# MILAB-IIT-CV/ATDN_vSLAM

Measured on AMD Instinct MI355X. Metric: frame-pairs/sec, KITTI 1241x376 odometry inference at 1/2/4/8 MI355X, higher is better.
Workload: dtype f32 via 3xf16 split MFMA (fp32 accumulate); 1 GPU; KITTI seq-03-shaped 376x1241 uint8 frames (resident in HBM) resized to 376x1232, GMA flow 12 GRU iters + CLVO head -> 6-DoF trajectory (BASELINE configs[1]); streams_per_gpu=2, gru_iters=12, parallelism=pairs sharded x1, one all-gather of 512-d features, replicated LSTM scan

## Files before the change

atdn_vslam_amd/_lib.py:

```python
import ctypes as C
import os

_HERE = os.path.dirname(os.path.abspath(__file__))
LIB_PATH = os.environ.get("ATDN_LIB_PATH") or os.path.join(_HERE, "libatdn_hip.so")

_f32p = C.POINTER(C.c_float)
_i64p = C.POINTER(C.c_int64)
_vp = C.c_void_p

SIGNATURES = {
    "atdn_version": (C.c_int, []),
    "atdn_last_error": (C.c_char_p, []),
    "atdn_gma_create": (C.c_int, [C.POINTER(_vp), C.c_int, C.c_int, C.c_int, C.c_int]),
    "atdn_gma_set_low_latency": (C.c_int, [_vp, C.c_int]),
    "atdn_gma_load": (C.c_int, [_vp, C.c_char_p, _vp, _i64p, C.c_int]),
    "atdn_gma_finalize": (C.c_int, [_vp]),
    "atdn_gma_forward": (C.c_int, [_vp, _vp, _vp, C.c_int, C.c_int, _vp, _vp, _vp, _vp]),
    "atdn_gma_forward_predictions": (C.c_int, [_vp, _vp, _vp, C.c_int, C.c_int, _vp, _vp, _vp]),
    "atdn_gma_forward_sequence": (C.c_int, [_vp, _vp, C.c_int, C.c_int, _vp, _vp, _vp, _vp]),
    "atdn_gma_forward_sequence_continued": (C.c_int, [_vp, _vp, C.c_int, C.c_int, _vp, _vp, _vp, _vp]),
    "atdn_gma_debug_read": (C.c_long, [_vp, C.c_char_p, _vp, C.c_long, _vp]),
    "atdn_gma_profile": (C.c_int, [_vp, C.c_int, C.c_int, C.c_int, _f32p, _vp]),
    "atdn_gma_profile_mode": (C.c_int, [_vp, C.c_int, C.c_int, C.c_int, C.c_int, _f32p, _vp]),
    "atdn_gma_set_range_probe": (C.c_int, [_vp, C.c_int]),
    "atdn_gma_range_rows": (C.c_long, [_vp]),
    "atdn_gma_range_row": (C.c_int, [_vp, C.c_long, C.c_char_p, C.c_int, C.POINTER(C.c_int), C.POINTER(C.c_int), _f32p, _i64p, _i64p]),
    "atdn_range_probe": (C.c_int, [_vp, C.c_int64, C.c_int64, C.c_int64, _f32p, _i64p, _i64p, _vp]),
    "atdn_range_probe_launch": (C.c_int, [_vp, C.c_int64, C.c_int64, C.c_int64, _vp, _vp]),
    "atdn_gma_workspace_bytes": (C.c_size_t, [_vp]),
    "atdn_gma_destroy": (None, [_vp]),
    "atdn_device_bytes_live": (C.c_int64, []),
    "atdn_clvo_create": (C.c_int, [C.POINTER(_vp), C.c_int, C.c_int, C.c_int]),
    "atdn_clvo_load": (C.c_int, [_vp, C.c_char_p, _vp, _i64p, C.c_int]),
    "atdn_clvo_finalize": (C.c_int, [_vp]),
    "atdn_clvo_encode": (C.c_int, [_vp, _vp, C.c_int, _vp, _vp]),
    "atdn_clvo_step": (C.c_int, [_vp, _vp, C.c_int, C.c_int, _vp, _vp, _vp, _vp]),
    "atdn_clvo_last_scan_path": (C.c_int, [_vp]),
    "atdn_clvo_destroy": (None, [_vp]),
    "atdn_vae_create": (C.c_int, [C.POINTER(_vp), C.c_int, C.c_int, C.c_int]),
    "atdn_vae_load": (C.c_int, [_vp, C.c_char_p, _vp, _i64p, C.c_int]),
    "atdn_vae_finalize": (C.c_int, [_vp]),
    "atdn_vae_embedding_shape": (C.c_int, [_vp, C.POINTER(C.c_int), C.POINTER(C.c_int)]),
    "atdn_vae_encode": (C.c_int, [_vp, _vp, C.c_int, _vp, _vp]),
    "atdn_vae_scratch_floats": (C.c_int, [C.c_int, C.c_int, C.POINTER(C.c_long), C.POINTER(C.c_int)]),
    "atdn_vae_debug_stage": (C.c_int, [_vp, _vp, C.c_int, C.c_int, _vp, C.c_long, _vp]),
    "atdn_vae_destroy": (None, [_vp]),
    "atdn_clvo_trainer_create": (C.c_int, [C.POINTER(_vp), C.c_int, C.c_int, C.c_int, C.c_int]),
    "atdn_clvo_trainer_load": (C.c_int, [_vp, C.c_char_p, _vp, _i64p, C.c_int]),
    "atdn_clvo_trainer_finalize": (C.c_int, [_vp]),
    "atdn_clvo_trainer_forward_backward": (C.c_int, [_vp, _vp, _vp, _vp, _vp, _vp, _f32p, _vp]),
    "atdn_clvo_trainer_gradients": (C.c_int, [_vp, C.POINTER(_vp), C.POINTER(C.c_long)]),
    "atdn_clvo_trainer_adamw_step": (C.c_int, [_vp, C.c_float, C.c_float, C.c_float, C.c_int, _vp]),
    "atdn_clvo_trainer_set_loss": (C.c_int, [_vp, C.c_float, C.c_int, C.c_int]),
    "atdn_clvo_trainer_loss_terms": (C.c_int, [_vp, _f32p]),
    "atdn_clvo_loss": (C.c_int, [_vp, _vp, _vp, _vp, C.c_int, C.c_int, C.c_float, C.c_int, C.c_int, _f32p, _vp, _vp, _vp]),
    "atdn_clvo_trainer_read": (C.c_long, [_vp, C.c_char_p, C.c_int, _vp, C.c_long, _vp]),
    "atdn_clvo_trainer_destroy": (None, [_vp]),
    "atdn_pose_transform_f32": (C.c_int, [_vp, _vp, _vp]),
    "atdn_pose_rel2abs": (C.c_int, [_vp, _vp, C.c_int, _vp]),
    "atdn_pose_accumulate_f32": (C.c_int, [_vp, _vp, _vp]),
    "atdn_resize_frames": (C.c_int, [_vp, C.c_int, C.c_int, C.c_int, C.c_int, C.c_int, _vp, _vp]),
    "atdn_resize_frames_mode": (C.c_int, [_vp, C.c_int, C.c_int, C.c_int, C.c_int, C.c_int, C.c_int, _vp, _vp]),
    "atdn_resize_frames_u8": (C.c_int, [_vp, C.c_int, C.c_int, C.c_int, C.c_int, C.c_int, C.c_int, _vp, _vp]),
    "atdn_pad_frames": (C.c_int, [_vp, C.c_int, C.c_int, C.c_int, C.c_int, C.c_int, C.c_int, C.c_int, _vp, _vp]),
    "atdn_ingest_create": (C.c_int, [C.POINTER(_vp), C.c_int, C.c_int, C.c_int, C.c_int, C.c_int, C.c_int]),
    "atdn_ingest_frames_u8": (C.c_int, [_vp, _vp, C.c_int, _vp, _vp]),
    "atdn_ingest_destroy": (None, [_vp]),
    "atdn_flow_pack_f16": (C.c_int, [_vp, C.c_int, C.c_int, C.c_int, C.c_int, C.c_int, _vp, _vp]),
    "atdn_flow_gather_clips": (C.c_int, [_vp, C.c_int, C.c_int, C.c_int, _vp, _vp, C.c_int, C.c_int, _vp, _vp]),
    "atdn_flow_forward_interpolate": (C.c_int, [_vp, C.c_int, C.c_int, C.c_int, _vp, _vp]),
    "atdn_flow_forward_interpolate_host": (C.c_int, [_vp, C.c_int, C.c_int, C.c_int, _vp]),
    "atdn_flow_consistency": (C.c_int, [_vp, _vp, C.c_int, C.c_int, C.c_int, C.c_double, C.c_double, _vp, _vp, _vp]),
    "atdn_flow_consistency_host": (C.c_int, [_vp, _vp, C.c_int, C.c_int, C.c_int, C.c_double, C.c_double, _vp, _vp]),
    "atdn_flow_two_view_depth": (C.c_int, [_vp, _vp, _vp, C.c_int, C.c_int, C.c_int, C.c_double, C.c_double, C.c_double, C.c_double,
                                           C.c_double, C.c_double, C.c_double, _vp, _vp, _vp]),
    "atdn_flow_two_view_depth_host": (C.c_int, [_vp, _vp, _vp, C.c_int, C.c_int, C.c_int, C.c_double, C.c_double, C.c_double,
                                                C.c_double, C.c_double, C.c_double, C.c_double, _vp, _vp]),
    "atdn_depth_backproject": (C.c_int, [_vp, C.c_int, C.c_int, C.c_int, C.c_double, C.c_double, C.c_double, C.c_double, _vp, _vp]),
    "atdn_flow_track_step": (C.c_int, [_vp, _vp, _vp, _vp, C.c_int, C.c_int, C.c_int, _vp, _vp, _vp, C.c_double, C.c_double, C.c_double,
                                       C.c_double, C.c_double, C.c_double, C.c_double, _vp, _vp, _vp]),
    "atdn_flow_track_step_host": (C.c_int, [_vp, _vp, _vp, _vp, C.c_int, C.c_int, C.c_int, _vp, _vp, _vp, C.c_double, C.c_double,
                                            C.c_double, C.c_double, C.c_double, C.c_double, C.c_double, _vp, _vp]),
    "atdn_depth_fuse": (C.c_int, [_vp, _vp, _vp, _vp, C.c_int, C.c_int, C.c_int, C.c_int, C.c_int, C.c_double, C.c_double, C.c_double,
                                  C.c_double, C.c_double, C.c_double, C.c_int, C.c_double, C.c_int, _vp, _vp, _vp, _vp]),
    "atdn_depth_fuse_host": (C.c_int, [_vp, _vp, _vp, _vp, C.c_int, C.c_int, C.c_int, C.c_int, C.c_int, C.c_double, C.c_double,
                                       C.c_double, C.c_double, C.c_double, C.c_double, C.c_int, C.c_double, C.c_int, _vp, _vp, _vp]),
    "atdn_multiview_depth": (C.c_int, [_vp, _vp, _vp, _vp, _vp, C.c_int, C.c_int, C.c_int, C.c_int, C.c_int, C.c_double, C.c_double,
                                       C.c_double, C.c_double, C.c_double, C.c_double, C.c_double, C.c_int, C.c_double, C.c_double,
                                       C.c_int, _vp, _vp, _vp, _vp, _vp]),
    "atdn_multiview_depth_host": (C.c_int, [_vp, _vp, _vp, _vp, _vp, C.c_int, C.c_int, C.c_int, C.c_int, C.c_int, C.c_double,
                                            C.c_double, C.c_double, C.c_double, C.c_double, C.c_double, C.c_double, C.c_int,
                                            C.c_double, C.c_double, C.c_int, _vp, _vp, _vp, _vp]),
    "atdn_bundle_workspace_bytes": (C.c_long, [C.c_int, C.c_int, C.c_int, C.c_int, C.c_int]),
    "atdn_bundle_terms": (C.c_int, [_vp] * 6 + [C.c_int] * 5 + [C.c_double] * 4 + [C.c_int] + [C.c_double] * 3 + [C.c_int] + [_vp] * 4),
    "atdn_bundle_terms_host": (C.c_int, [_vp] * 6 + [C.c_int] * 5 + [C.c_double] * 4 + [C.c_int] + [C.c_double] * 3 + [C.c_int] +
                               [_vp] * 2),
    "atdn_bundle_adjust": (C.c_int, [_vp] * 6 + [C.c_int] * 5 + [C.c_double] * 4 + [C.c_int] * 2 + [C.c_double] * 3 + [C.c_int] +
                           [_vp] * 6),
    "atdn_bundle_adjust_host": (C.c_int, [_vp] * 6 + [C.c_int] * 5 + [C.c_double] * 4 + [C.c_int] * 2 + [C.c_double] * 3 + [C.c_int] +
                                [_vp] * 4),
    "atdn_pnp_workspace_bytes":(C.c_long, [C.c_int, C.c_int, C.c_int]),
    "atdn_pnp_terms": (C.c_int, [_vp, _vp, _vp, _vp, C.c_int, C.c_int, C.c_int, C.c_double, C.c_double, C.c_double, C.c_double,
                                 C.c_double, C.c_double, C.c_double, _vp, _vp, _vp, _vp]),
    "atdn_pnp_terms_host": (C.c_int, [_vp, _vp, _vp, _vp, C.c_int, C.c_int, C.c_int, C.c_double, C.c_double, C.c_double, C.c_double,
                                      C.c_double, C.c_double, C.c_double, _vp, _vp]),
    "atdn_pnp_solve": (C.c_int, [_vp, _vp, _vp, _vp, C.c_int, C.c_int, C.c_int, C.c_double, C.c_double, C.c_double, C.c_double,
                                 C.c_double, C.c_double, C.c_double, C.c_int, _vp, _vp, _vp, _vp, _vp]),
    "atdn_pnp_solve_host": (C.c_int, [_vp, _vp, _vp, _vp, C.c_int, C.c_int, C.c_int, C.c_double, C.c_double, C.c_double, C.c_double,
                                      C.c_double, C.c_double, C.c_double, C.c_int, _vp, _vp, _vp]),
    "atdn_epipolar_workspace_bytes": (C.c_long, [C.c_int, C.c_int, C.c_int]),
    "atdn_epipolar_terms": (C.c_int, [_vp, _vp, _vp, C.c_int, C.c_int, C.c_int, C.c_double, C.c_double, C.c_double, C.c_double,
                                      C.c_double, C.c_double, _vp, _vp, _vp, _vp]),
    "atdn_epipolar_terms_host": (C.c_int, [_vp, _vp, _vp, C.c_int, C.c_int, C.c_int, C.c_double, C.c_double, C.c_double, C.c_double,
                                           C.c_double, C.c_double, _vp, _vp]),
    "atdn_epipolar_solve": (C.c_int, [_vp, _vp, _vp, C.c_int, C.c_int, C.c_int, C.c_double, C.c_double, C.c_double, C.c_double,
                                      C.c_double, C.c_double, C.c_int, _vp, _vp, _vp, _vp, _vp]),
    "atdn_epipolar_solve_host": (C.c_int, [_vp, _vp, _vp, C.c_int, C.c_int, C.c_int, C.c_double, C.c_double, C.c_double, C.c_double,
                                           C.c_double, C.c_double, C.c_int, _vp, _vp, _vp]),
    "atdn_ground_workspace_bytes": (C.c_long, [C.c_int, C.c_int, C.c_int]),
    "atdn_ground_terms": (C.c_int, [_vp] * 3 + [C.c_int] * 5 + [C.c_double] * 8 + [_vp] * 4),
    "atdn_ground_terms_host": (C.c_int, [_vp] * 3 + [C.c_int] * 5 + [C.c_double] * 8 + [_vp] * 2),
    "atdn_ground_solve": (C.c_int, [_vp] * 3 + [C.c_int] * 5 + [C.c_double] * 11 + [C.c_int] * 2 + [_vp] * 5),
    "atdn_ground_solve_host": (C.c_int, [_vp] * 3 + [C.c_int] * 5 + [C.c_double] * 11 + [C.c_int] * 2 + [_vp] * 3),
    "atdn_ground_classify": (C.c_int, [_vp] * 3 + [C.c_int] * 5 + [C.c_double] * 7 + [_vp] * 3),
    "atdn_ground_classify_host": (C.c_int, [_vp] * 3 + [C.c_int] * 5 + [C.c_double] * 7 + [_vp] * 2),
    "atdn_pose_graph_workspace_bytes": (C.c_long, [C.c_int, C.c_int, C.c_int]),
    "atdn_pose_graph_terms": (C.c_int, [_vp, _vp, _vp, _vp, _vp, C.c_int, C.c_int, C.c_int, C.c_double, _vp, _vp, _vp, _vp, _vp]),
    "atdn_pose_graph_terms_host": (C.c_int, [_vp, _vp, _vp, _vp, _vp, C.c_int, C.c_int, C.c_int, C.c_double, _vp, _vp, _vp]),
    "atdn_pose_graph_solve": (C.c_int, [_vp, _vp, _vp, _vp, _vp, _vp, C.c_int, C.c_int, C.c_int, C.c_double, C.c_int, C.c_int,
                                        C.c_double, _vp, _vp, _vp, _vp, _vp, _vp]),
    "atdn_pose_graph_solve_host": (C.c_int, [_vp, _vp, _vp, _vp, _vp, _vp, C.c_int, C.c_int, C.c_int, C.c_double, C.c_int, C.c_int,
                                             C.c_double, _vp, _vp, _vp, _vp]),
    "atdn_map_search": (C.c_int, [_vp, C.c_int, C.c_int, _vp, C.c_int, C.c_int, _vp, _vp, _vp]),
    "atdn_map_gather_images_u8": (C.c_int, [_vp, C.c_int, C.c_long, _vp, C.c_int, _vp, _vp]),
    "atdn_corr_lookup": (C.c_int, [_vp, _vp, _vp, _vp, C.c_int, C.c_int, C.c_int, _vp, _vp, C.c_int, _vp]),
    "atdn_corr_pyramid": (C.c_int, [_vp, _vp, C.c_int, C.c_int, C.c_int, C.c_int, _vp, _vp, _vp, _vp, _vp]),
    "atdn_corr_lookup_bricks": (C.c_int, [_vp, _vp, C.c_int, C.c_int, C.c_int, C.c_int, _vp, _vp, _vp, _vp, _vp, _vp, _vp, _vp,
                                          _vp, _vp]),
    "atdn_conv2d_nhwc": (C.c_int, [_vp, C.c_int, C.c_int, C.c_int, C.c_int, _vp, _vp, C.c_int, C.c_int, C.c_int,
                                   C.c_int, C.c_int, C.c_int, C.c_int, _vp, _vp]),
    "atdn_conv2d_nhwc_sf": (C.c_int, [_vp, C.c_int, C.c_int, C.c_int, C.c_int, _vp, _vp, C.c_int, C.c_int, C.c_int,
                                      C.c_int, C.c_int, C.c_int, _vp, _vp]),
    "atdn_conv2d_nhwc_sf_epi": (C.c_int, [_vp, C.c_int, C.c_int, C.c_int, C.c_int, _vp, _vp, C.c_int, C.c_int, C.c_int,
                                      C.c_int, C.c_int, C.c_int, C.c_int, _vp, _vp]),
}

GMA_STAGES = ("fnet", "corr", "pool", "cnet", "attention", "lookup", "motion_encoder", "aggregate", "gru_zr", "gru_q",
              "flow_head", "mask", "gru_ctx", "attn_logits", "agg_vt", "convc1", "gru_zr_v", "gru_q_v")

_lib = None


def lib():
    global _lib
    if _lib is None:
        if not os.path.exists(LIB_PATH):
            raise RuntimeError(
                "%s is missing: the HIP extension has not been built (python -m atdn_vslam_amd.build). "
                "There is no CPU fallback for the product path." % LIB_PATH)
        import torch
        handle = C.CDLL(LIB_PATH)
        for name, (res, args) in SIGNATURES.items():
            fn = getattr(handle, name)
            fn.restype = res
            fn.argtypes = args
        _lib = handle
    return _lib


def check(rc):
    if rc != 0:
        raise RuntimeError("libatdn_hip: " + lib().atdn_last_error().decode("utf-8", "replace"))


def load_state(load_fn, handle, state):
    import numpy as np
    import torch
    for key, val in state.items():
        if isinstance(val, torch.Tensor):
            if not val.dtype.is_floating_point:
                continue
            arr = val.detach().to("cpu", torch.float32).contiguous().numpy()
        else:
            arr = np.asarray(val)
            if arr.dtype.kind != "f":
                continue
            arr = np.ascontiguousarray(arr, dtype=np.float32)
        shape = (C.c_int64 * max(arr.ndim, 1))(*arr.shape) if arr.ndim else (C.c_int64 * 1)(1)
        check(load_fn(handle, key.encode(), arr.ctypes.data_as(_vp), shape, arr.ndim))
```

atdn_vslam_amd/csrc/capi.hip:

```cpp
#include "../../include/atdn_hip.h"

#include <cmath>
#include <cstring>

#include "clvo.h"
#include "gma.h"
#include "vae.h"
#include "clvo_train.h"
#include "train_kernels.h"
#include "frontend.h"
#include "conv_sf.h"
#include "depth_fusion_host.h"
#include "epilogues_sf.h"
#include "epipolar_host.h"
#include "flow_args.h"
#include "flow_consistency_host.h"
#include "flow_track_host.h"
#include "bundle_host.h"
#include "ground_host.h"
#include "multiview_depth_host.h"
#include "pnp_host.h"
#include "two_view_host.h"
#include "warm_start_host.h"

namespace atdn {
extern template TileChoice conv_dispatch<MODE_TAP, EpiBias<ACT_NONE>>(const ConvShape&, EpiBias<ACT_NONE>, hipStream_t);
extern template TileChoice conv_dispatch<MODE_TAP, EpiBias<ACT_RELU>>(const ConvShape&, EpiBias<ACT_RELU>, hipStream_t);
extern template TileChoice conv_dispatch<MODE_ROW, EpiBias<ACT_NONE>>(const ConvShape&, EpiBias<ACT_NONE>, hipStream_t);
extern template TileChoice conv_dispatch<MODE_ROW, EpiBias<ACT_RELU>>(const ConvShape&, EpiBias<ACT_RELU>, hipStream_t);
extern template TileChoice conv_dispatch<MODE_TAP, EpiScale>(const ConvShape&, EpiScale, hipStream_t);

extern template TileChoice conv_sf_dispatch<EpiBias<ACT_NONE>>(const ConvShape&, float, EpiBias<ACT_NONE>, hipStream_t);
extern template TileChoice conv_sf_dispatch<SfBias<ACT_NONE>>(const ConvShape&, float, SfBias<ACT_NONE>, hipStream_t);

static thread_local std::string g_last_error;
void set_last_error(const std::string& msg) { g_last_error = msg; }
}

using namespace atdn;

struct atdn_gma { GmaNet net; atdn_gma(int H, int W, int B, int prec) : net(H, W, B, prec) {} };
struct atdn_clvo { ClvoNet net; atdn_clvo(int H, int W, int B) : net(H, W, B) {} };
struct atdn_vae { VaeEncoder net; atdn_vae(int H, int W, int B) : net(H, W, B) {} };
struct atdn_ingest { FrameIngest in; atdn_ingest(int a, int b, int c, int d, int n, int aa) : in(a, b, c, d, n, aa) {} };
struct atdn_clvo_trainer { ClvoTrainer net; atdn_clvo_trainer(int H, int W, int B, int T) : net(H, W, B, T) {} };

template <class T>
static void euler_yxz(const T* r, T* R) {
  const T c1 = std::cos(r[0]), c2 = std::cos(r[1]), c3 = std::cos(r[2]);
  const T s1 = std::sin(r[0]), s2 = std::sin(r[1]), s3 = std::sin(r[2]);
  R[0] = c1 * c3 + s1 * s2 * s3; R[1] = c3 * s1 * s2 - c1 * s3; R[2] = c2 * s1;
  R[3] = c2 * s3;                R[4] = c2 * c3;                R[5] = -s2;
  R[6] = c1 * s2 * s3 - c3 * s1; R[7] = c1 * c3 * s2 + s1 * s3; R[8] = c1 * c2;
}
template <class T>
static void make_transform(const T* rot, const T* tr, T* m) {
  T R[9];
  euler_yxz(rot, R);
  for (int i = 0; i < 3; ++i) { for (int j = 0; j < 3; ++j) m[i * 4 + j] = R[i * 3 + j]; m[i * 4 + 3] = tr[i]; }
  m[12] = 0; m[13] = 0; m[14] = 0; m[15] = 1;
}
template <class T>
static void matmul4(const T* a, const T* b, T* c) {
  for (int i = 0; i < 4; ++i)
    for (int j = 0; j < 4; ++j) {
      T s = 0;
      for (int k = 0; k < 4; ++k) s += a[i * 4 + k] * b[k * 4 + j];
      c[i * 4 + j] = s;
    }
}

extern "C" {

int atdn_version(void) { return 100; }
const char* atdn_last_error(void) { return g_last_error.c_str(); }

int atdn_gma_create(atdn_gma** out, int H, int W, int max_batch, int precision) {
  ATDN_API_BEGIN
  ATDN_CHECK(out, "null out pointer");
  *out = new atdn_gma(H, W, max_batch, precision);
  ATDN_API_END
}
int atdn_gma_set_low_latency(atdn_gma* h, int on) {
  ATDN_API_BEGIN
  ATDN_CHECK(h, "null handle");
  h->net.set_low_latency(on != 0);
  ATDN_API_END
}
int atdn_gma_load(atdn_gma* h, const char* key, const float* data, const int64_t* shape, int rank) {
  ATDN_API_BEGIN
  ATDN_CHECK(h && key && data && rank >= 0 && rank <= 4, "bad state-dict entry");
  h->net.state().put(key, data, shape, rank);
  ATDN_API_END
}
int atdn_gma_finalize(atdn_gma* h) {
  ATDN_API_BEGIN
  ATDN_CHECK(h, "null handle");
  h->net.finalize();
  ATDN_API_END
}
int atdn_gma_forward(atdn_gma* h, const float* im1, const float* im2, int B, int iters, const float* flow_init,
                     float* flow_low, float* flow_up, void* stream) {
  ATDN_API_BEGIN
  ATDN_CHECK(h, "null handle");
  h->net.forward(im1, im2, B, iters, flow_init, flow_low, flow_up, (hipStream_t)stream);
  ATDN_API_END
}
int atdn_gma_forward_predictions(atdn_gma* h, const float* im1, const float* im2, int B, int iters, const float* flow_init,
                                 float* flow_predictions, void* stream) {
  ATDN_API_BEGIN
  ATDN_CHECK(h, "null handle");
  h->net.forward_predictions(im1, im2, B, iters, flow_init, flow_predictions, (hipStream_t)stream);
  ATDN_API_END
}
int atdn_gma_forward_sequence(atdn_gma* h, const float* frames, int B, int iters, const float* flow_init,
                              float* flow_low, float* flow_up, void* stream) {
  ATDN_API_BEGIN
  ATDN_CHECK(h, "null handle");
  h->net.forward_sequence(frames, B, iters, flow_init, flow_low, flow_up, (hipStream_t)stream);
  ATDN_API_END
}
int atdn_gma_forward_sequence_continued(atdn_gma* h, const float* frames, int B, int iters, const float* flow_init,
                                        float* flow_low, float* flow_up, void* stream) {
  ATDN_API_BEGIN
  ATDN_CHECK(h, "null handle");
  h->net.forward_sequence(frames, B, iters, flow_init, flow_low, flow_up, (hipStream_t)stream, true);
  ATDN_API_END
}
long atdn_gma_debug_read(atdn_gma* h, const char* name, float* host, long capacity, void* stream) {
  try {
    if (!h || !name || !host) throw Error("null argument");
    const long n = h->net.debug_read(name, host, capacity, (hipStream_t)stream);
    if (n < 0) throw Error(std::string("unknown tensor name: ") + name);
    return n;
  } catch (const std::exception& e) {
    set_last_error(e.what());
    return -1;
  }
}
int atdn_gma_profile(atdn_gma* h, int B, int iters, int reps, float* ms_out, void* stream) {
  ATDN_API_BEGIN
  ATDN_CHECK(h && ms_out, "null argument");
  static_assert(GmaNet::ST_COUNT == ATDN_GMA_STAGES, "stage table out of sync with the header");
  h->net.profile(B, iters, reps, ms_out, (hipStream_t)stream, 0);
  ATDN_API_END
}
int atdn_gma_profile_mode(atdn_gma* h, int B, int iters, int reps, int mode, float* ms_out, void* stream) {
  ATDN_API_BEGIN
  ATDN_CHECK(h && ms_out, "null argument");
  ATDN_CHECK(mode >= 0 && mode <= 2, "mode must be 0 (pair), 1 (sequence) or 2 (continued sequence)");
  h->net.profile(B, iters, reps, ms_out, (hipStream_t)stream, mode);
  ATDN_API_END
}
int atdn_gma_set_range_probe(atdn_gma* h, int on) {
  ATDN_API_BEGIN
  ATDN_CHECK(h, "null handle");
  h->net.set_probe(on != 0);
  ATDN_API_END
}
long atdn_gma_range_rows(atdn_gma* h) {
  if (!h) { set_last_error("null handle"); return -1; }
  return (long)h->net.probe_rows().size();
}
int atdn_gma_range_row(atdn_gma* h, long index, char* name, int name_capacity, int* iteration, int* limited, float* max_abs,
                       int64_t* over, int64_t* nonfinite) {
  ATDN_API_BEGIN
  ATDN_CHECK(h && name && iteration && limited && max_abs && over && nonfinite, "null argument");
  const auto& rows = h->net.probe_rows();
  ATDN_CHECK(index >= 0 && index < (long)rows.size(), "row index out of range");
  const GmaNet::ProbeRow& r = rows[(size_t)index];
  ATDN_CHECK(name_capacity > (int)r.name.size(), "name buffer too small");
  memcpy(name, r.name.c_str(), r.name.size() + 1);
  *iteration = r.iter; *limited = r.limited ? 1 : 0; *max_abs = r.max_abs;
  *over = (int64_t)r.over; *nonfinite = (int64_t)r.nonfinite;
  ATDN_API_END
}
int atdn_range_probe_launch(const float* x, int64_t rows, int64_t cols, int64_t ld, void* slot, void* stream) {
  ATDN_API_BEGIN
  launch_range_probe(x, (long)rows, (long)cols, (long)ld, static_cast<RangeSlot*>(slot), (hipStream_t)stream);
  ATDN_API_END
}
int atdn_range_probe(const float* x, int64_t rows, int64_t cols, int64_t ld, float* max_abs, int64_t* over, int64_t* nonfinite,
                     void* stream) {
  ATDN_API_BEGIN
  ATDN_CHECK(x && max_abs && over && nonfinite, "null argument");
  hipStream_t st = (hipStream_t)stream;
// ... 451 lines not shown
    }
    fbrick[l].alloc((long)B * bp.NB[l] * 256);
    launch_brick_rows(src, src_sb, B, pH[l], pW[l], 256, 256, fbrick[l].p, (long)bp.NB[l] * 256, st);
    pyr[l].alloc((long)B * bp.NPB * kBrickPixelBlock * bp.NB[l]);
    launch_corr_bricks(f1.p, (long)N * 256, fbrick[l].p, (long)bp.NB[l] * 256, B, N, bp.NB[l], 256, 1.0f / sqrtf(256.0f), pyr[l].p, false, st);
    bp.base[l] = pyr[l].p;
    if (rowmajor[l]) launch_unbrick(pyr[l].p, bp.NB[l], N, pH[l], pW[l], n8, rowmajor[l], st);
  }
  if (samples) {
    outsf.alloc(n8 * 352);
    launch_lookup_bricks(bp, coords, n8, outsf.p, st);
    scratch.alloc(n8 * 352);
    launch_from_sf(outsf.p, scratch.p, n8, 352, st);
    ATDN_HIP(hipMemcpy2DAsync(samples, 324 * sizeof(float), scratch.p, 352 * sizeof(float), 324 * sizeof(float), (size_t)n8,
                              hipMemcpyDeviceToDevice, st));
  }
  if (cor1) {
    StateDict sd;
    const int64_t ws[4] = {256, 324, 1, 1}, bs[1] = {256};
    sd.put("c.weight", convc1_weight_host, ws, 4);
    sd.put("c.bias", convc1_bias_host, bs, 1);
    PackedConv L = pack_conv_sf(A, sd, {"c"});
    pack_fragment_major16(A, L);
    A.upload();
    resolve(A, L);
    csf.alloc(n8 * 256);
    launch_lookup_conv(bp, coords, n8, nullptr, L.wf16, L.wscale, L.b, csf.p, false, st);
    launch_from_sf(csf.p, cor1, n8, 256, st);
    ATDN_HIP(hipStreamSynchronize(st));
  }
  ATDN_HIP(hipStreamSynchronize(st));
  ATDN_API_END
}

int atdn_conv2d_nhwc(const float* src, int nimg, int H, int W, int Cin, const float* weight_host,
                     const float* bias_host, int Cout, int KH, int KW, int stride, int padH, int padW, int relu,
                     float* dst, void* stream) {
  ATDN_API_BEGIN
  ATDN_CHECK(src && weight_host && dst && nimg >= 1, "null argument");
  const bool row = (Cin == 4 || Cin == 16);
  ATDN_CHECK(row || Cin % 32 == 0, "Cin must be 4, 16 or a multiple of 32");
  StateDict sd;
  const int64_t ws[4] = {Cout, Cin, KH, KW};
  sd.put("c.weight", weight_host, ws, 4);
  std::vector<float> zb(Cout, 0.f);
  const int64_t bs[1] = {Cout};
  sd.put("c.bias", bias_host ? bias_host : zb.data(), bs, 1);
  WeightArena A;
  PackedConv L = pack_conv(A, sd, {"c"}, row ? MODE_ROW : MODE_TAP, Cin);
  A.upload();
  resolve(A, L);
  ConvShape s;
  s.src0 = src; s.ld0 = Cin; s.sb0 = (long)H * W * Cin; s.C0 = L.C; s.H = H; s.W = W;
  s.KH = KH; s.KW = KW; s.stride = stride; s.padH = padH; s.padW = padW;
  s.w = L.w; s.ldw = L.ldw; s.N = Cout; s.nimg = nimg;
  const int Ho = conv_out(H, KH, stride, padH), Wo = conv_out(W, KW, stride, padW);
  hipStream_t st = (hipStream_t)stream;
  if (row) {
    if (relu) conv_dispatch<MODE_ROW>(s, EpiBias<ACT_RELU>{L.b, dst, (long)Ho * Wo * Cout, Cout, 1.f}, st);
    else conv_dispatch<MODE_ROW>(s, EpiBias<ACT_NONE>{L.b, dst, (long)Ho * Wo * Cout, Cout, 1.f}, st);
  } else {
    if (relu) conv_dispatch<MODE_TAP>(s, EpiBias<ACT_RELU>{L.b, dst, (long)Ho * Wo * Cout, Cout, 1.f}, st);
    else conv_dispatch<MODE_TAP>(s, EpiBias<ACT_NONE>{L.b, dst, (long)Ho * Wo * Cout, Cout, 1.f}, st);
  }
  ATDN_HIP(hipStreamSynchronize(st));
  ATDN_API_END
}

int atdn_resize_frames(const float* src, int planes, int Hin, int Win, int Hout, int Wout, float* dst, void* stream) {
  return atdn_resize_frames_mode(src, planes, Hin, Win, Hout, Wout, ATDN_RESIZE_ANTIALIAS, dst, stream);
}
int atdn_resize_frames_mode(const float* src, int planes, int Hin, int Win, int Hout, int Wout, int antialias, float* dst,
                            void* stream) {
  ATDN_API_BEGIN
  ATDN_CHECK(src && dst && planes >= 1 && Hin >= 1 && Win >= 1 && Hout >= 1 && Wout >= 1, "bad argument");
  ATDN_CHECK(antialias == 0 || antialias == 1, "antialias must be ATDN_RESIZE_BILINEAR or ATDN_RESIZE_ANTIALIAS");
  launch_resize<float>(src, planes, Hin, Win, Hout, Wout, antialias, dst, (hipStream_t)stream);
  ATDN_API_END
}
int atdn_resize_frames_u8(const uint8_t* src, int planes, int Hin, int Win, int Hout, int Wout, int antialias, float* dst,
                          void* stream) {
  ATDN_API_BEGIN
  ATDN_CHECK(src && dst && planes >= 1 && Hin >= 1 && Win >= 1 && Hout >= 1 && Wout >= 1, "bad argument");
  ATDN_CHECK(antialias == 0 || antialias == 1, "antialias must be ATDN_RESIZE_BILINEAR or ATDN_RESIZE_ANTIALIAS");
  launch_resize<unsigned char>(src, planes, Hin, Win, Hout, Wout, antialias, dst, (hipStream_t)stream);
  ATDN_API_END
}
int atdn_pad_frames(const float* src, int planes, int H, int W, int left, int right, int top, int bottom, float* dst,
                    void* stream) {
  ATDN_API_BEGIN
  ATDN_CHECK(src && dst && planes >= 1 && H >= 1 && W >= 1 && left >= 0 && right >= 0 && top >= 0 && bottom >= 0, "bad argument");
  launch_pad_replicate(src, planes, H, W, left, right, top, bottom, dst, (hipStream_t)stream);
  ATDN_API_END
}
int atdn_ingest_create(atdn_ingest** out, int Hin, int Win, int Hout, int Wout, int max_frames, int antialias) {
  ATDN_API_BEGIN
  ATDN_CHECK(out, "null out pointer");
  ATDN_CHECK(antialias == 0 || antialias == 1, "antialias must be ATDN_RESIZE_BILINEAR or ATDN_RESIZE_ANTIALIAS");
  *out = new atdn_ingest(Hin, Win, Hout, Wout, max_frames, antialias);
  ATDN_API_END
}
int atdn_ingest_frames_u8(atdn_ingest* h, const uint8_t* host_frames, int n_frames, float* dst, void* stream) {
  ATDN_API_BEGIN
  ATDN_CHECK(h, "null handle");
  h->in.ingest(host_frames, n_frames, dst, (hipStream_t)stream);
  ATDN_API_END
}
void atdn_ingest_destroy(atdn_ingest* h) { delete h; }

int atdn_conv2d_nhwc_sf_epi(const float* src, int nimg, int H, int W, int Cin, const float* weight_host,
                            const float* bias_host, int Cout, int KH, int KW, int stride, int padH, int padW, int sf_store,
                            float* dst, void* stream) {
  ATDN_API_BEGIN
  ATDN_CHECK(src && weight_host && dst && nimg >= 1 && Cin % 32 == 0, "bad argument (Cin must be a multiple of 32)");
  ATDN_CHECK(sf_store >= 0 && sf_store <= 7 && (sf_store & 6) != 6, "sf_store: bit 0 names the epilogue, bit 1 or bit 2 the tile form");
  const int tile_form = (sf_store & 2) ? 1 : (sf_store & 4) ? 2 : 0;
  sf_store &= 1;
  ATDN_CHECK(!sf_store || Cout % 32 == 0, "the split-f16 store needs Cout % 32 == 0");
  StateDict sd;
  const int64_t ws[4] = {Cout, Cin, KH, KW};
  sd.put("c.weight", weight_host, ws, 4);
  std::vector<float> zb(Cout, 0.f);
  const int64_t bs[1] = {Cout};
  sd.put("c.bias", bias_host ? bias_host : zb.data(), bs, 1);
  WeightArena A;
  PackedConv L = pack_conv_sf(A, sd, {"c"});
  A.upload();
  resolve(A, L);
  hipStream_t st = (hipStream_t)stream;
  DeviceBuf tmp, osf;
  const long rows = (long)nimg * H * W;
  tmp.alloc(rows * Cin);
  launch_to_sf(src, tmp.p, rows, Cin, st);
  ConvShape s;
  s.src0 = tmp.p; s.ld0 = Cin; s.sb0 = (long)H * W * Cin; s.C0 = L.C; s.H = H; s.W = W;
  s.KH = KH; s.KW = KW; s.stride = stride; s.padH = padH; s.padW = padW;
  s.w = L.w; s.ldw = L.ldw; s.N = Cout; s.nimg = nimg;
  const int Ho = conv_out(H, KH, stride, padH), Wo = conv_out(W, KW, stride, padW);
  s.wfrag16 = L.wf16;
  s.tile_form = tile_form;
  if (sf_store) {
    const long orows = (long)nimg * Ho * Wo;
    osf.alloc(orows * Cout);
    conv_sf_dispatch(s, L.wscale, SfBias<ACT_NONE>{L.b, osf.p, (long)Ho * Wo * Cout, Cout}, st);
    launch_from_sf(osf.p, dst, orows, Cout, st);
    ATDN_HIP(hipStreamSynchronize(st));
  } else {
    conv_sf_dispatch(s, L.wscale, EpiBias<ACT_NONE>{L.b, dst, (long)Ho * Wo * Cout, Cout, 1.f}, st);
    ATDN_HIP(hipStreamSynchronize(st));
  }
  ATDN_API_END
}

int atdn_conv2d_nhwc_sf(const float* src, int nimg, int H, int W, int Cin, const float* weight_host,
                        const float* bias_host, int Cout, int KH, int KW, int stride, int padH, int padW, float* dst,
                        void* stream) {
  return atdn_conv2d_nhwc_sf_epi(src, nimg, H, W, Cin, weight_host, bias_host, Cout, KH, KW, stride, padH, padW, 0, dst, stream);
}

}
```

atdn_vslam_amd/csrc/conv_mfma.h:

```cpp
#pragma once
#include "common.h"

namespace atdn {

typedef float f32x16 __attribute__((ext_vector_type(16)));

enum { MODE_TAP = 0, MODE_ROW = 1 };

struct ConvGeom {
  const float* src0;
  const float* src1;
  long sb0, sb1;
  int ld0, ld1;
  int C0, C1;
  int H, W, Ho, Wo;
  int KH, KW, stride, padH, padW;
  int cpk;
  int nchunks;
  int log2C;
  const float* w;
  long wb;
  int ldw;
  int N;
  int tiles_per_img, nimg, ntile_n;
// ... 62 lines not shown
        const float4 v = *reinterpret_cast<const float4*>(sp + (long)(ok ? iy * g.W + ix : 0) * ld + co + 4 * s);
        ra[i] = v;
        aok[i] = ok;
      }
      cc += 32;
      if (cc == ctot) { cc = 0; if (++kx == g.KW) { kx = 0; ++ky; } }
    } else {
      const int f = kx * 32 + 4 * s;
      const int dx = f >> g.log2C, c = f & (g.C0 - 1);
#pragma unroll
      for (int i = 0; i < RA; ++i) {
        const int iy = iy0[i] + ky, ix = ix0[i] + dx;
        const bool ok = ((unsigned)iy < (unsigned)g.H) & ((unsigned)ix < (unsigned)g.W);
        const float4 v = *reinterpret_cast<const float4*>(s0 + (long)(ok ? iy * g.W + ix : 0) * g.ld0 + c);
        ra[i] = v;
        aok[i] = ok;
      }
      if (++kx == g.cpk) { kx = 0; ++ky; }
    }
#pragma unroll
    for (int j = 0; j < RB; ++j) {
      const float4 v = *reinterpret_cast<const float4*>(wrow[j] + q * 32);
      rb[j] = v;
    }
  };

  const int lane = tid & 63, wave = tid >> 6;
  const int wm = wave / WGN, wn = wave % WGN;
  const int r = lane & 31, h = lane >> 5;
  f32x16 acc[TM][TN];
#pragma unroll
  for (int i = 0; i < TM; ++i)
#pragma unroll
    for (int j = 0; j < TN; ++j)
#pragma unroll
      for (int e = 0; e < 16; ++e) acc[i][j][e] = 0.f;

  const float* a_rd = As + (wm * TM * 32 + r) * LDS_LD + 4 * h;
  const float* b_rd = Bs + (wn * TN * 32 + r) * LDS_LD + 4 * h;

  fetch(0);
  for (int q = 0; q < g.nchunks; ++q) {
    __syncthreads();
#pragma unroll
    for (int i = 0; i < RA; ++i)
      *reinterpret_cast<float4*>(As + (r0 + 32 * i) * LDS_LD + 4 * s) = keep_if(aok[i], ra[i]);
#pragma unroll
    for (int j = 0; j < RB; ++j)
      *reinterpret_cast<float4*>(Bs + (r0 + 32 * j) * LDS_LD + 4 * s) = keep_if(wok[j], rb[j]);
    __syncthreads();
    if (q + 1 < g.nchunks) fetch(q + 1);
#pragma unroll
    for (int kc = 0; kc < 4; ++kc) {
      float4 a[TM], b[TN];
#pragma unroll
      for (int i = 0; i < TM; ++i) a[i] = *reinterpret_cast<const float4*>(a_rd + i * 32 * LDS_LD + kc * 8);
#pragma unroll
      for (int j = 0; j < TN; ++j) b[j] = *reinterpret_cast<const float4*>(b_rd + j * 32 * LDS_LD + kc * 8);
#pragma unroll
      for (int i = 0; i < TM; ++i)
#pragma unroll
        for (int j = 0; j < TN; ++j) {
          acc[i][j] = __builtin_amdgcn_mfma_f32_32x32x2f32(a[i].x, b[j].x, acc[i][j], 0, 0, 0);
          acc[i][j] = __builtin_amdgcn_mfma_f32_32x32x2f32(a[i].y, b[j].y, acc[i][j], 0, 0, 0);
          acc[i][j] = __builtin_amdgcn_mfma_f32_32x32x2f32(a[i].z, b[j].z, acc[i][j], 0, 0, 0);
          acc[i][j] = __builtin_amdgcn_mfma_f32_32x32x2f32(a[i].w, b[j].w, acc[i][j], 0, 0, 0);
        }
    }
  }

  typename EpiCol<Epi>::type colj[TN];
  float biasj[TN];
#pragma unroll
  for (int j = 0; j < TN; ++j) {
    const int n = min(n0 + (wn * TN + j) * 32 + r, g.N - 1);
    biasj[j] = 0.f;
    if constexpr (Epi::kStats) biasj[j] = ep.bias[n];
    if constexpr (epi_bias_arg<Epi>::value) colj[j] = ep.col(n);
  }
#pragma unroll
  for (int i = 0; i < TM; ++i) {
    const int mbase = pix0 + (wm * TM + i) * 32;
#pragma unroll
    for (int j = 0; j < TN; ++j) {
      const int n = n0 + (wn * TN + j) * 32 + r;
      const bool nok = n < g.N;
      if constexpr (Epi::kStats) {
        const float bias = nok ? biasj[j] : 0.f;
        float v[16];
        float sum = 0.f;
        int cnt = 0;
#pragma unroll
        for (int e = 0; e < 16; ++e) {
          const int m = mbase + (e & 3) + 8 * (e >> 2) + 4 * h;
          v[e] = acc[i][j][e] + bias;
          if (m < HoWo) { sum += v[e]; ++cnt; }
        }
        sum += __shfl_xor(sum, 32);
        cnt += __shfl_xor(cnt, 32);
        const float mean = sum / (float)(cnt > 0 ? cnt : 1);
        float m2 = 0.f;
#pragma unroll
        for (int e = 0; e < 16; ++e) {
          const int m = mbase + (e & 3) + 8 * (e >> 2) + 4 * h;
          if (m < HoWo) { const float d = v[e] - mean; m2 += d * d; }
        }
        m2 += __shfl_xor(m2, 32);
        if (h == 0 && nok) {
          const int grp = mbase >> 5;
          const long o = ((long)img * ep.groups_per_img + grp) * g.N + n;
          ep.part_sum[o] = sum;
          ep.part_m2[o] = m2;
        }
      }
      if (nok) {
        if constexpr (Epi::kPrefetch) {
          typename Epi::Aux aux[16];
#pragma unroll
          for (int e = 0; e < 16; ++e) aux[e] = ep.load(img, min(mbase + (e & 3) + 8 * (e >> 2) + 4 * h, HoWo - 1), n);
#pragma unroll
          for (int e = 0; e < 16; ++e) {
            const int m = mbase + (e & 3) + 8 * (e >> 2) + 4 * h;
            if (m < HoWo) ep.apply(img, m, n, acc[i][j][e], aux[e]);
          }
        } else if constexpr (epi_bias_arg<Epi>::value) {
#pragma unroll
          for (int e = 0; e < 16; ++e) {
            const int m = mbase + (e & 3) + 8 * (e >> 2) + 4 * h;
            if (m < HoWo) ep.store_c(img, m, n, acc[i][j][e], colj[j]);
          }
        } else {
#pragma unroll
          for (int e = 0; e < 16; ++e) {
            const int m = mbase + (e & 3) + 8 * (e >> 2) + 4 * h;
            if (m < HoWo) ep(img, m, n, acc[i][j][e]);
          }
        }
      }
    }
  }
}

struct ConvShape {
  const float* src0 = nullptr; const float* src1 = nullptr;
  long sb0 = 0, sb1 = 0;
  int ld0 = 0, ld1 = 0, C0 = 0, C1 = 0;
  int H = 1, W = 1;
  int KH = 1, KW = 1, stride = 1, padH = 0, padW = 0;
  const float* w = nullptr; long wb = 0; int ldw = 0;
  const float* wfrag16 = nullptr;
  int N = 0;
  int nimg = 1;
  const float* in_mean = nullptr; const float* in_rstd = nullptr;
  int tile_form = 0;
};

inline int conv_out(int in, int k, int stride, int pad) { return (in + 2 * pad - k) / stride + 1; }

template <int MODE>
inline ConvGeom make_geom(const ConvShape& s, int BM, int BN) {
  ConvGeom g{};
  g.src0 = s.src0; g.src1 = s.src1; g.sb0 = s.sb0; g.sb1 = s.sb1; g.ld0 = s.ld0; g.ld1 = s.ld1;
  g.C0 = s.C0; g.C1 = s.C1; g.H = s.H; g.W = s.W;
  g.KH = s.KH; g.KW = s.KW; g.stride = s.stride; g.padH = s.padH; g.padW = s.padW;
  g.Ho = conv_out(s.H, s.KH, s.stride, s.padH);
  g.Wo = conv_out(s.W, s.KW, s.stride, s.padW);
  if (MODE == MODE_TAP) {
    ATDN_CHECK(s.C0 % 32 == 0 && s.C1 % 32 == 0 && s.C0 > 0, "TAP mode needs channel counts that are multiples of 32");
    ATDN_CHECK(s.ld0 % 4 == 0 && (s.C1 == 0 || (s.src1 && s.ld1 % 4 == 0)), "TAP mode needs 16-byte aligned pixels");
    g.cpk = s.KW * ((s.C0 + s.C1) / 32);
    g.log2C = 0;
  } else {
    ATDN_CHECK(s.C1 == 0 && s.src1 == nullptr, "ROW mode takes one source");
    ATDN_CHECK(s.C0 >= 4 && (s.C0 & (s.C0 - 1)) == 0 && s.ld0 == s.C0, "ROW mode needs dense power-of-two channels");
    g.cpk = cdiv(s.KW * s.C0, 32);
    int l = 0; while ((1 << l) < s.C0) ++l;
    g.log2C = l;
  }
  g.nchunks = s.KH * g.cpk;
  g.w = s.w; g.wb = s.wb; g.ldw = s.ldw; g.N = s.N;
  ATDN_CHECK(s.ldw % 4 == 0 && s.ldw >= g.nchunks * 32, "weight rows must hold the padded K and be 16-byte aligned");
  ATDN_CHECK(((uintptr_t)s.src0 % 16) == 0 && ((uintptr_t)s.w % 16) == 0 && s.sb0 % 4 == 0 && s.wb % 4 == 0,
             "operands must be 16-byte aligned");
  ATDN_CHECK(g.Ho > 0 && g.Wo > 0 && s.N > 0 && s.nimg > 0, "empty convolution");
  g.nimg = s.nimg;
  g.tiles_per_img = cdiv(g.Ho * g.Wo, BM);
  g.ntile_n = cdiv(s.N, BN);
  return g;
}

inline int packed_k(int mode, int KH, int KW, int C) {
  return mode == MODE_TAP ? KH * KW * C : KH * round_up(KW * C, 32);
}

template <int MODE, int TM, int TN, int WGM, int WGN, class Epi>
inline void launch_conv(const ConvShape& s, const Epi& ep, hipStream_t st) {
  constexpr int BM = 32 * TM * WGM, BN = 32 * TN * WGN;
  ConvGeom g = make_geom<MODE>(s, BM, BN);
  const int nblk = g.nimg * g.tiles_per_img * g.ntile_n;
  hipLaunchKernelGGL((conv_mfma_kernel<MODE, TM, TN, WGM, WGN, Epi>), dim3(nblk), dim3(256), 0, st, g, ep);
  ATDN_HIP(hipGetLastError());
}

}
```

atdn_vslam_amd/csrc/conv_sf.h:

```cpp
#pragma once
#include <type_traits>
#include "conv_dispatch.h"
#include "sf.h"

namespace atdn {

template <int TM, int TN, int WGM, int WGN, class Epi, bool FAST = false>
__global__ __launch_bounds__(256) void conv_sf_kernel(const ConvGeom g, const float wscale, const Epi ep) {
  constexpr int BM = 32 * TM * WGM, BN = 32 * TN * WGN;
  constexpr int RA = BM / 32, RB = BN / 32;
  constexpr int LDS_LD = 40;
  __shared__ __attribute__((aligned(16))) float lds[(BM + BN) * LDS_LD];
  float* As = lds;
  float* Bs = lds + BM * LDS_LD;

  const int tid = threadIdx.x;
  const int nblk = g.nimg * g.tiles_per_img * g.ntile_n;
  const int id = xcd_remap(blockIdx.x, nblk);
  const int tile_n = id % g.ntile_n;
  const int tmg = id / g.ntile_n;
  const int img = tmg / g.tiles_per_img;
  const int pix0 = (tmg % g.tiles_per_img) * BM;
  const int n0 = tile_n * BN;
  const int HoWo = g.Ho * g.Wo;
// ... 74 lines not shown
  for (int d = 0; d < PF; ++d) fetch(min(d, last), d);
  const int nq = (g.nchunks + PF - 1) / PF * PF;
  for (int q0 = 0; q0 < nq; q0 += PF) {
#pragma unroll
   for (int d = 0; d < PF; ++d) {
    const int q = q0 + d;
    const bool live = PF == 1 || q <= last;
    __syncthreads();
#pragma unroll
    for (int i = 0; i < RA; ++i)
      *reinterpret_cast<float4*>(As + (r0 + 32 * i) * LDS_LD + 4 * s) = keep_if(aok[d][i] && live, ra[d][i]);
#pragma unroll
    for (int j = 0; j < RB; ++j)
      *reinterpret_cast<float4*>(Bs + (r0 + 32 * j) * LDS_LD + 4 * s) = keep_if(wok[j], rb[d][j]);
    __syncthreads();
    fetch(min(q + PF, last), d);
    f16x8 ah[TM][2], al[TM][2], bh[TN][2], bl[TN][2];
#pragma unroll
    for (int i = 0; i < TM; ++i)
#pragma unroll
      for (int hb = 0; hb < 2; ++hb) {
        ah[i][hb] = *reinterpret_cast<const f16x8*>(a_rd + (i * 32 + 16 * hb) * ROWB);
        if constexpr (!FAST) al[i][hb] = *reinterpret_cast<const f16x8*>(a_rd + (i * 32 + 16 * hb) * ROWB + 64);
      }
#pragma unroll
    for (int j = 0; j < TN; ++j)
#pragma unroll
      for (int cb = 0; cb < 2; ++cb) {
        bh[j][cb] = *reinterpret_cast<const f16x8*>(b_rd + (j * 32 + 16 * cb) * ROWB);
        if constexpr (!FAST) bl[j][cb] = *reinterpret_cast<const f16x8*>(b_rd + (j * 32 + 16 * cb) * ROWB + 64);
      }
#pragma unroll
    for (int i = 0; i < TM; ++i)
#pragma unroll
      for (int j = 0; j < TN; ++j)
#pragma unroll
        for (int hb = 0; hb < 2; ++hb)
#pragma unroll
          for (int cb = 0; cb < 2; ++cb) {
            f32x4v c = acc[i][j].b[hb][cb];
            if constexpr (!FAST) {
              c = __builtin_amdgcn_mfma_f32_16x16x32_f16(al[i][hb], bh[j][cb], c, 0, 0, 0);
              c = __builtin_amdgcn_mfma_f32_16x16x32_f16(ah[i][hb], bl[j][cb], c, 0, 0, 0);
            }
            c = __builtin_amdgcn_mfma_f32_16x16x32_f16(ah[i][hb], bh[j][cb], c, 0, 0, 0);
            acc[i][j].b[hb][cb] = c;
          }
   }
  }

  constexpr int NSET = 2, NPX = 8;
  auto col_of = [&](int cs) { return 16 * cs + (lane & 15); };
  auto row_of = [&](int e) { return 16 * (e >> 2) + 4 * (lane >> 4) + (e & 3); };
  auto val_of = [&](int i, int j, int cs, int e) __attribute__((always_inline)) { return acc[i][j].b[e >> 2][cs][e & 3]; };
  typename EpiCol<Epi>::type colj[TN][NSET];
  float biasj[TN][NSET];
#pragma unroll
  for (int j = 0; j < TN; ++j)
#pragma unroll
    for (int cs = 0; cs < NSET; ++cs) {
      const int n = min(n0 + (wn * TN + j) * 32 + col_of(cs), g.N - 1);
      biasj[j][cs] = 0.f;
      if constexpr (Epi::kStats) biasj[j][cs] = ep.bias[n];
      if constexpr (epi_bias_arg<Epi>::value) colj[j][cs] = ep.col(n);
    }
#pragma unroll
  for (int i = 0; i < TM; ++i) {
    const int mbase = pix0 + (wm * TM + i) * 32;
#pragma unroll
    for (int j = 0; j < TN; ++j)
#pragma unroll
      for (int cs = 0; cs < NSET; ++cs) {
        const int n = n0 + (wn * TN + j) * 32 + col_of(cs);
        const bool nok = n < g.N;
        if constexpr (Epi::kStats) {
          const float bias = nok ? biasj[j][cs] : 0.f;
          float v[NPX];
          float sum = 0.f;
          int cnt = 0;
#pragma unroll
          for (int e = 0; e < NPX; ++e) {
            const int m = mbase + row_of(e);
            v[e] = val_of(i, j, cs, e) * wscale + bias;
            if (m < HoWo) { sum += v[e]; ++cnt; }
          }
          sum += __shfl_xor(sum, 16);
          cnt += __shfl_xor(cnt, 16);
          sum += __shfl_xor(sum, 32);
          cnt += __shfl_xor(cnt, 32);
          const float mean = sum / (float)(cnt > 0 ? cnt : 1);
          float m2 = 0.f;
#pragma unroll
          for (int e = 0; e < NPX; ++e) {
            const int m = mbase + row_of(e);
            if (m < HoWo) { const float d = v[e] - mean; m2 += d * d; }
          }
          m2 += __shfl_xor(m2, 16);
          m2 += __shfl_xor(m2, 32);
          if ((lane >> 4) == 0 && nok) {
            const int grp = mbase >> 5;
            const long o = ((long)img * ep.groups_per_img + grp) * g.N + n;
            ep.part_sum[o] = sum;
            ep.part_m2[o] = m2;
          }
        }
        if (nok) {
          if constexpr (Epi::kPrefetch) {
            typename Epi::Aux aux[NPX];
#pragma unroll
            for (int e = 0; e < NPX; ++e) aux[e] = ep.load(img, min(mbase + row_of(e), HoWo - 1), n);
#pragma unroll
            for (int e = 0; e < NPX; ++e) {
              const int m = mbase + row_of(e);
              if (m < HoWo) ep.apply(img, m, n, val_of(i, j, cs, e) * wscale, aux[e]);
            }
          } else if constexpr (epi_bias_arg<Epi>::value) {
#pragma unroll
            for (int e = 0; e < NPX; ++e) {
              const int m = mbase + row_of(e);
              if (m < HoWo) ep.store_c(img, m, n, val_of(i, j, cs, e) * wscale, colj[j][cs]);
            }
          } else {
#pragma unroll
            for (int e = 0; e < NPX; ++e) {
              const int m = mbase + row_of(e);
              if (m < HoWo) ep(img, m, n, val_of(i, j, cs, e) * wscale);
            }
          }
        }
      }
  }
}

template <int TM, int TN, int WGM, int WGN, class Epi, bool FAST = false>
inline void launch_conv_sf(const ConvShape& s, float wscale, const Epi& ep, hipStream_t st) {
  constexpr int BM = 32 * TM * WGM, BN = 32 * TN * WGN;
  ConvGeom g = make_geom<MODE_TAP>(s, BM, BN);
  const int nblk = g.nimg * g.tiles_per_img * g.ntile_n;
  hipLaunchKernelGGL((conv_sf_kernel<TM, TN, WGM, WGN, Epi, FAST>), dim3(nblk), dim3(256), 0, st, g, wscale, ep);
  ATDN_HIP(hipGetLastError());
}

bool& sf_fast_mode();

template <class F>
inline auto with_fast(bool fast, F&& f) {
  return fast ? f(std::true_type{}) : f(std::false_type{});
}

template <class Epi>
TileChoice conv_sf_dispatch(const ConvShape& s, float wscale, Epi ep, hipStream_t st);
template <class Epi>
void conv_sf_dispatch_pair(const ConvShape& s0, float wscale0, Epi ep0, const ConvShape& s1, float wscale1, Epi ep1, hipStream_t st);

}
```

atdn_vslam_amd/csrc/conv_sf6.h:

```cpp
#pragma once
#include <type_traits>
#include "conv_sf.h"

namespace atdn {

struct Conv2Geom {
  const float* src0; const float* src1;
  long sb0, sb1;
  int ld0, ld1, C0, C1;
  int H, W, Ho, Wo;
  int padH, padW;
  int tiles_x, tiles_y;
  int nimg, ntile_n;
  const float* w; int N;
  float wscale;
  const float* in_mean; const float* in_rstd;
};

inline bool conv_halo_eligible(const ConvShape& s) {
  if (s.stride != 1 || s.wb != 0) return false;
  return (s.KH == 3 && s.KW == 3) || (s.KH == 1 && s.KW == 5) || (s.KH == 5 && s.KW == 1);
}

template <class E, class = void> struct epi_gen6 : std::integral_constant<int, 0> {};
template <class E> struct epi_gen6<E, std::void_t<decltype(E::kGen6)>> : std::integral_constant<int, E::kGen6> {};
template <class E, class = void> struct EpiAux4 { struct type {}; };
template <class E> struct EpiAux4<E, std::void_t<typename E::Aux4>> { using type = typename E::Aux4; };
template <class E, class = void> struct epi_flowhead : std::false_type {};
template <class E> struct epi_flowhead<E, std::void_t<decltype(E::kFlowHead)>> : std::bool_constant<E::kFlowHead> {};
template <class E, class = void> struct epi_ring3 : std::false_type {};
template <class E> struct epi_ring3<E, std::void_t<decltype(E::kRing3)>> : std::bool_constant<E::kRing3> {};
template <class E, class = void> struct epi_rawacc : std::false_type {};
template <class E> struct epi_rawacc<E, std::void_t<decltype(E::kRawAcc)>> : std::bool_constant<E::kRawAcc> {};
template <class E, class = void> struct epi_vec4 : std::false_type {};
template <class E> struct epi_vec4<E, std::void_t<decltype(E::kVec4)>> : std::bool_constant<E::kVec4> {};

typedef float f32x4v __attribute__((ext_vector_type(4)));
struct SfAcc { f32x4v b[2][2]; };

#ifdef ATDN_CONV_STAMP
#define ATDN_CONV_STAMP_SLOTS 4096
extern __device__ unsigned long long atdn_conv_stamps_dev[4][ATDN_CONV_STAMP_SLOTS][12];
template <class E> struct conv_stamp_kind : std::integral_constant<int, -1> {};
#endif

template <int TH, int TW, int BN, int WM, int WN, int KH, int KW, class Epi, bool FAST = false, bool NORM = false, int ABL = 0,
          bool RUN = false>
__device__ __forceinline__ void conv_sf6_body(const Conv2Geom& g, const Epi& ep, const int bidx) {
  static_assert(ABL == 0 || !NORM, "ablation builds exist for the plain patch loader");
  static_assert(!RUN || (((KH == 1 && KW == 5) || (KH == 5 && KW == 1)) && TH == 8 && BN == 128 && WM == 1 && WN == 4 && !NORM &&
                         ABL == 0 && !Epi::kStats && !epi_flowhead<Epi>::value),
                "run tiles: separable passes on the 8 x 16 x 128 block, plain loader, epilogues without statistics");
  static_assert(TW == 16, "the 16x16x32 loop is built for 16-pixel tile rows");
  constexpr int NIMG = 2;
  constexpr int NW = WM * WN, NT = NW * 64;
  constexpr int TM = TH * TW / 32 / WM, TN = BN / 32 / WN;
  static_assert(TM * WM * 32 == TH * TW && TN * WN * 32 == BN, "wave grid must tile the block");
  static_assert(32 % TW == 0 || TW % 32 == 0, "a 32-pixel MFMA row tile must cover whole tile rows");
  constexpr int NTAP = KH * KW;
  constexpr int RSTEP = NT / 8;
  constexpr int RSLOTS = 160;
  constexpr int PROWS = RUN ? RSLOTS : (TH + KH - 1) * (TW + KW - 1);
  constexpr int PW = TW + KW - 1;
  constexpr int NP = (PROWS + RSTEP - 1) / RSTEP;
  constexpr int ROWB = 160;
  constexpr int RS = PW * ROWB;
  constexpr bool SWAP = epi_vec4<Epi>::value;
  constexpr int PSZ = RUN ? RSLOTS * ROWB : (TH + KH - 1) * RS;
  __shared__ __attribute__((aligned(256))) char Pbytes[NIMG * PSZ];

  const int tid = threadIdx.x;
  const int tiles_img = g.tiles_x * g.tiles_y;
  const int nblk = g.nimg * tiles_img * g.ntile_n;
  const int id = xcd_remap(bidx, nblk);
  const int tile_n = id % g.ntile_n;
  const int tmg = id / g.ntile_n;
  const int img = tmg / tiles_img;
  const int tloc = tmg - img * tiles_img;
  const int ty0 = (tloc / g.tiles_x) * TH, tx0 = (tloc % g.tiles_x) * TW;
  const int n0 = tile_n * BN;
  const int lane = tid & 63, wave = tid >> 6;
  const int rL = KH == 1 ? g.W : g.H, rHW = g.H * g.W;
  const int rm0 = tloc * (TH * TW);
  const int rrun0 = RUN ? rm0 / rL : 0, rpos0 = rm0 - rrun0 * rL;
  const int rb1 = rL - rpos0, rb2 = rb1 + rL, rb3 = rb2 + rL;
  auto out_pixel = [&](int p) {
    if constexpr (RUN) {
      const int k = (p >= rb1 ? 1 : 0) + (p >= rb2 ? 1 : 0) + (p >= rb3 ? 1 : 0);
      const int m = rm0 + p;
      if (m >= rHW) return -1;
      return KH == 1 ? m : (rpos0 + p - k * rL) * g.W + rrun0 + k;
    } else {
      const int oy = ty0 + p / TW, ox = tx0 + p % TW;
      return (oy < g.Ho && ox < g.Wo) ? oy * g.Wo + ox : -1;
    }
  };
#ifdef ATDN_CONV_STAMP
  constexpr int kStamp = conv_stamp_kind<Epi>::value;
  unsigned long long st_r0 = 0, st_t0 = 0, st_t1 = 0, st_t2 = 0, st_bar = 0;
  unsigned long long st_e_slab = 0, st_e_wait = 0, st_e_apply = 0;
  if constexpr (kStamp >= 0) { st_r0 = __builtin_amdgcn_s_memrealtime(); st_t0 = __builtin_amdgcn_s_memtime(); }
#endif

  const int jrow = (tid >> 3) & 7;
  const int s = tid & 7, r0 = !NORM ? tid >> 3 : ((tid >> 6) << 3) + 2 * (jrow & 1) + ((jrow >> 1) & 1) + 4 * (jrow >> 2);
  static_assert(PSZ / 16 <= 4096, "LDS offset field");
  unsigned pmeta[NP];
#pragma unroll
  for (int k = 0; k < NP; ++k) {
    const int prow = r0 + RSTEP * k;
    unsigned off = 0;
    if constexpr (RUN) {
      static_assert(PROWS == NP * RSTEP, "every loader step writes slots of the image");
      const int kk = (prow >= 2 + rb1 ? 1 : 0) + (prow >= 10 + rb2 ? 1 : 0) + (prow >= 18 + rb3 ? 1 : 0);
      const bool gap = kk > 0 && prow < 2 + rb1 + (kk - 1) * rL + 8 * kk;
      const int p = prow - 2 - 8 * kk;
      const int pos = rpos0 + p - kk * rL;
      if (!gap && p < 130 && (unsigned)pos < (unsigned)rL && rm0 + p < rHW) off = (unsigned)(KH == 1 ? rm0 + p : pos * g.W + rrun0 + kk) + 1u;
      pmeta[k] = (off << 12) | (unsigned)((prow * ROWB + 16 * s) >> 4);
      continue;
    }
    const int py = prow / PW, px = prow - py * PW;
    if (prow < PROWS) {
      const int iy = ty0 - g.padH + py, ix = tx0 - g.padW + px;
      if ((unsigned)iy < (unsigned)g.H && (unsigned)ix < (unsigned)g.W) off = (unsigned)(iy * g.W + ix) + 1u;
    }
    pmeta[k] = (off << 12) | (unsigned)((py * RS + px * ROWB + 16 * s) >> 4);
    if (prow >= PROWS) pmeta[k] = pmeta[0];
  }
  const float* s0 = g.src0 + (long)img * g.sb0;
  const float* s1 = g.src1 ? g.src1 + (long)img * g.sb1 : nullptr;
  const int nck = (g.C0 + g.C1) >> 5;

  float4 pr[NP];
  auto fetch_patch = [&](int c) {
    const int cc = c << 5;
    const float* sp; int ld, co;
    if (cc < g.C0) { sp = s0; ld = g.ld0; co = cc; } else { sp = s1; ld = g.ld1; co = cc - g.C0; }
#pragma unroll
    for (int k = 0; k < NP; ++k)
      pr[k] = *reinterpret_cast<const float4*>(sp + (long)((pmeta[k] >> 12) ? (pmeta[k] >> 12) - 1 : 0) * ld + co + 4 * s);
  };
  auto store_patch = [&](int buf) {
#pragma unroll
    for (int k = 0; k < NP; ++k)
      *reinterpret_cast<float4*>(Pbytes + buf * PSZ + ((pmeta[k] & 0xFFFu) << 4)) = keep_if((pmeta[k] >> 12) != 0, pr[k]);
  };
  float4 nmu = make_float4(0.f, 0.f, 0.f, 0.f), nrs = make_float4(1.f, 1.f, 1.f, 1.f);
  auto fetch_norm = [&](int c) {
    nmu = *reinterpret_cast<const float4*>(g.in_mean + (long)img * g.C0 + (c << 5) + 4 * s);
    nrs = *reinterpret_cast<const float4*>(g.in_rstd + (long)img * g.C0 + (c << 5) + 4 * s);
  };
  bool norm_sat = false;
  auto store_row_norm = [&](int buf, int k, float4 mu, float4 rs) {
    const float hi = (pmeta[k] >> 12) != 0 ? 65504.f : 0.f;
    float4 v = pr[k];
    v.x = (v.x - mu.x) * rs.x; v.y = (v.y - mu.y) * rs.y; v.z = (v.z - mu.z) * rs.z; v.w = (v.w - mu.w) * rs.w;
    const float m = fmaxf(fmaxf(v.x, v.y), fmaxf(v.z, v.w));
    norm_sat |= !(m <= 65504.f);
    v.x = __builtin_amdgcn_fmed3f(v.x, 0.f, hi); v.y = __builtin_amdgcn_fmed3f(v.y, 0.f, hi);
    v.z = __builtin_amdgcn_fmed3f(v.z, 0.f, hi); v.w = __builtin_amdgcn_fmed3f(v.w, 0.f, hi);
    const unsigned h0 = sf_cvt_pk_(v.x, v.y), h1 = sf_cvt_pk_(v.z, v.w);
    const unsigned l0 = sf_residual_pk_(h0, v.x, v.y), l1 = sf_residual_pk_(h1, v.z, v.w);
    char* px = Pbytes + buf * PSZ + (((pmeta[k] & 0xFFFu) - (unsigned)s) << 4);
    *reinterpret_cast<uint2*>(px + 8 * s) = make_uint2(h0, h1);
    *reinterpret_cast<uint2*>(px + 64 + 8 * s) = make_uint2(l0, l1);
  };

  const int wm = wave / WN, wn = wave % WN;
  SfAcc acc[TM][TN];
#pragma unroll
  for (int i = 0; i < TM; ++i)
#pragma unroll
    for (int j = 0; j < TN; ++j) {
#pragma unroll
      for (int e = 0; e < 16; ++e) acc[i][j].b[e >> 3][(e >> 2) & 1][e & 3] = 0.f;
    }
  {
    const int n16 = lane & 15, g16 = lane >> 4;
    int a_off[RUN ? 2 * TM : TM];
#pragma unroll
    for (int i = 0; i < TM; ++i) {
      if constexpr (RUN) {
#pragma unroll
        for (int hh = 0; hh < 2; ++hh) {
          const int p = ((wm * TM + i) * 2 + hh) * 16 + n16;
          const int k = (p >= rb1 ? 1 : 0) + (p >= rb2 ? 1 : 0) + (p >= rb3 ? 1 : 0);
          a_off[hh * TM + i] = (p + 8 * k) * ROWB + 16 * g16;
        }
      } else {
        a_off[i] = ((wm * TM + i) * 2) * RS + n16 * ROWB + 16 * g16;
      }
    }
    const char* Pb = Pbytes;
    const int nblk16 = (g.N + 15) >> 4;
    const float* wrow[TN][2];
#pragma unroll
    for (int j = 0; j < TN; ++j)
#pragma unroll
      for (int cb = 0; cb < 2; ++cb)
        wrow[j][cb] = g.w + (long)min(((n0 >> 4) + (wn * TN + j) * 2 + cb), nblk16 - 1) * (NTAP * nck) * 512 + lane * 4;
    constexpr int RT = (NTAP % 3 == 0 || epi_ring3<Epi>::value) ? 3 : 2;
    constexpr int CU = (NTAP % RT == 0) ? 1 : RT;
    constexpr int NS = CU * NTAP;
    static_assert(NS % RT == 0, "ring size must divide the K steps of an unrolled iteration");
    struct WFrag { f16x8 hi[TN][2], lo[TN][2]; };
    WFrag wr[RT];
    auto load_w = [&](WFrag& f, int c0, int st, int cb) __attribute__((always_inline)) {
      const int cc = min(c0 + st / NTAP, nck - 1);
      const int q = (st % NTAP) * nck + cc;
#pragma unroll
      for (int j = 0; j < TN; ++j) {
        f.hi[j][cb] = *reinterpret_cast<const f16x8*>(wrow[j][cb] + (long)q * 512);
        if constexpr (!FAST) f.lo[j][cb] = *reinterpret_cast<const f16x8*>(wrow[j][cb] + (long)q * 512 + 256);
      }
    };
    fetch_patch(0);
    if constexpr (NORM) fetch_norm(0);
#pragma unroll
    for (int st = 0; st < RT - 1; ++st) { load_w(wr[st], 0, st, 0); load_w(wr[st], 0, st, 1); }
    if constexpr ((ABL & 1) != 0) { load_w(wr[RT - 1], 0, RT - 1, 0); load_w(wr[RT - 1], 0, RT - 1, 1); }
    if constexpr (NORM) {
#pragma unroll
      for (int k = 0; k < NP; ++k) store_row_norm(0, k, nmu, nrs);
    } else {
      store_patch(0);
    }
    __syncthreads();
#ifdef ATDN_CONV_STAMP
    if constexpr (kStamp >= 0) st_t1 = __builtin_amdgcn_s_memtime();
#endif
    f16x8 ah[2][TM], al[2][TM];
    auto read_a = [&](int half, int tap) __attribute__((always_inline)) {
      const char* arow = RUN ? Pb + tap * ROWB : Pb + (tap / KW + half) * RS + (tap % KW) * ROWB;
#pragma unroll
      for (int i = 0; i < TM; ++i) {
        const int ao = a_off[RUN ? half * TM + i : i];
        ah[half][i] = *reinterpret_cast<const f16x8*>(arow + ao);
        if constexpr (!FAST) al[half][i] = *reinterpret_cast<const f16x8*>(arow + ao + 64);
      }
    };
    auto mfma_half = [&](int half, const WFrag& w) __attribute__((always_inline)) {
#pragma unroll
      for (int i = 0; i < TM; ++i)
#pragma unroll
        for (int j = 0; j < TN; ++j)
#pragma unroll
          for (int cb = 0; cb < 2; ++cb) {
            f32x4v c = acc[i][j].b[half][cb];
            if constexpr (SWAP) {
              if constexpr (!FAST) {
                c = __builtin_amdgcn_mfma_f32_16x16x32_f16(w.hi[j][cb], al[half][i], c, 0, 0, 0);
                c = __builtin_amdgcn_mfma_f32_16x16x32_f16(w.lo[j][cb], ah[half][i], c, 0, 0, 0);
              }
              c = __builtin_amdgcn_mfma_f32_16x16x32_f16(w.hi[j][cb], ah[half][i], c, 0, 0, 0);
            } else {
              if constexpr (!FAST) {
                c = __builtin_amdgcn_mfma_f32_16x16x32_f16(al[half][i], w.hi[j][cb], c, 0, 0, 0);
                c = __builtin_amdgcn_mfma_f32_16x16x32_f16(ah[half][i], w.lo[j][cb], c, 0, 0, 0);
              }
              c = __builtin_amdgcn_mfma_f32_16x16x32_f16(ah[half][i], w.hi[j][cb], c, 0, 0, 0);
            }
            acc[i][j].b[half][cb] = c;
          }
    };
    constexpr int NMF = (FAST ? 1 : 3) * TM * TN * 2;
    constexpr int NH = 2 * NTAP;
    static_assert(!NORM || NH - 1 - NP >= 1, "normalise-on-load spreads its NP patch rows over the half-steps of a chunk");
    read_a(0, 0);
    if constexpr (KH != 3 || !Epi::kStats) __builtin_amdgcn_s_setprio(2);
    for (int c0 = 0; c0 < nck; c0 += CU) {
#pragma unroll
      for (int cu = 0; cu < CU; ++cu) {
        const int c = c0 + cu;
        const bool live = CU == 1 || c < nck;
        const int cn = min(c + 1, nck - 1);
#pragma unroll
        for (int hs = 0; hs < NH; ++hs) {
          const int tap = hs >> 1, half = hs & 1;
          const int st = cu * NTAP + tap;
          __builtin_amdgcn_sched_barrier(0);
          if (!(ABL & 2) && hs == 0) { fetch_patch(cn); if constexpr (NORM) fetch_norm(cn); }
          if (!(ABL & 1)) {
            if (RT == 2) { if (half == 0) { load_w(wr[(st + 1) % RT], c0, st + 1, 0); load_w(wr[(st + 1) % RT], c0, st + 1, 1); } }
            else load_w(wr[(st + RT - 1) % RT], c0, st + RT - 1, half);
          }
          if (!(ABL & 4) && hs + 1 < NH) read_a((hs + 1) & 1, (hs + 1) >> 1);
          if constexpr (NORM) {
            if (hs >= NH - 1 - NP && hs <= NH - 2) store_row_norm((c + 1) & 1, hs - (NH - 1 - NP), nmu, nrs);
          } else {
            if (!(ABL & 2) && hs == NH - 2) store_patch((c + 1) & 1);
          }
          if (live) mfma_half(half, wr[st % RT]);
          {
            constexpr int nds = 2 * TM;
            const int nvm = (RT == 2 ? (half == 0 ? 4 * TN : 0) : 2 * TN) + (hs == 0 ? NP : 0);
            const int ndw = NORM ? ((hs >= NH - 1 - NP && hs <= NH - 2) ? 2 : 0) : ((hs == NH - 2) ? NP : 0);
#pragma unroll
            for (int k = 0; k < NMF; ++k) {
              __builtin_amdgcn_sched_group_barrier(0x008, 1, 0);
              if (hs + 1 < NH && k < nds) __builtin_amdgcn_sched_group_barrier(0x100, 1, 0);
              else if (k - ((hs + 1 < NH) ? nds : 0) < nvm) __builtin_amdgcn_sched_group_barrier(0x020, 1, 0);
              else if (k - ((hs + 1 < NH) ? nds : 0) - nvm < ndw) __builtin_amdgcn_sched_group_barrier(0x200, 1, 0);
            }
          }
        }
        if (!(ABL & 2)) {
#ifdef ATDN_CONV_STAMP
          unsigned long long st_b0 = 0;
          if constexpr (kStamp >= 0) { asm volatile("s_waitcnt lgkmcnt(0)" ::: "memory"); st_b0 = __builtin_amdgcn_s_memtime(); }
#endif
          asm volatile("s_waitcnt lgkmcnt(0)\n\ts_barrier" ::: "memory");
#ifdef ATDN_CONV_STAMP
          if constexpr (kStamp >= 0) st_bar += __builtin_amdgcn_s_memtime() - st_b0;
#endif
          Pb = Pbytes + ((c + 1) & 1) * PSZ;
        }
        if (!(ABL & 4)) read_a(0, 0);
      }
    }
  }

#ifdef ATDN_CONV_STAMP
  if constexpr (kStamp >= 0) st_t2 = __builtin_amdgcn_s_memtime();
  auto stamp_out = [&]() __attribute__((always_inline)) {
    if constexpr (kStamp >= 0) {
      asm volatile("s_waitcnt vmcnt(0) lgkmcnt(0)" ::: "memory");
      const unsigned long long t3 = __builtin_amdgcn_s_memtime(), r1 = __builtin_amdgcn_s_memrealtime();
      const unsigned hw = __builtin_amdgcn_s_getreg((31 << 11) | 4), xcc = __builtin_amdgcn_s_getreg((31 << 11) | 20);
      if (wave == 0 && lane == 0 && bidx < ATDN_CONV_STAMP_SLOTS) {
        unsigned long long* o = atdn_conv_stamps_dev[kStamp * 2 + (KH == 5 ? 1 : 0)][bidx];
        o[0] = st_r0; o[1] = r1; o[2] = st_t1 - st_t0; o[3] = st_t2 - st_t1; o[4] = st_bar; o[5] = t3 - st_t2;
        o[6] = ((unsigned long long)xcc << 32) | hw; o[7] = t3 - st_t0;
        o[8] = st_e_slab; o[9] = st_e_wait; o[10] = st_e_apply; o[11] = 0;
      }
    }
  };
#endif
  if constexpr (KH != 3 || !Epi::kStats) __builtin_amdgcn_s_setprio(0);
  if constexpr (NORM) sf_report(norm_sat);
  if constexpr ((ABL & 8) != 0) {
    float tot = 0.f;
#pragma unroll
    for (int i = 0; i < TM; ++i)
#pragma unroll
      for (int j = 0; j < TN; ++j)
#pragma unroll
        for (int e = 0; e < 16; ++e) tot += acc[i][j].b[e >> 3][(e >> 2) & 1][e & 3];
    if (tot == 1.2345e-30f) ep(img, 0, 0, tot);
    return;
  }
  if constexpr (SWAP) {
    static_assert(NW * 32 * LDS_LD * 4 <= NIMG * PSZ, "transpose slabs must fit in the patch images");
    __syncthreads();
    float* tb = reinterpret_cast<float*>(Pbytes) + wave * (32 * LDS_LD);
    const int trow = lane >> 3, tcol = (lane & 7) * 4;
    auto tile_pixel = [&](int i, int q) {
      const int p = (wm * TM + i) * 32 + 8 * q + trow;
      if constexpr ((ABL & 16) != 0) return p;
      return out_pixel(p);
    };
    constexpr bool RAW = epi_rawacc<Epi>::value && !epi_flowhead<Epi>::value;
    auto slab_write = [&](const SfAcc& a) __attribute__((always_inline)) {
      const float sc = RAW ? 1.0f : g.wscale;
#pragma unroll
      for (int hh = 0; hh < 2; ++hh)
#pragma unroll
        for (int cb = 0; cb < 2; ++cb)
          *reinterpret_cast<float4*>(tb + (16 * hh + (lane & 15)) * LDS_LD + 16 * cb + 4 * (lane >> 4)) =
              RAW ? make_float4(a.b[hh][cb][0], a.b[hh][cb][1], a.b[hh][cb][2], a.b[hh][cb][3])
                  : make_float4(a.b[hh][cb][0] * sc, a.b[hh][cb][1] * sc, a.b[hh][cb][2] * sc, a.b[hh][cb][3] * sc);
    };
    if constexpr (epi_flowhead<Epi>::value) {
      static_assert(!epi_flowhead<Epi>::value || (WM == 1 && TN == 1 && TW == 16), "one block holds all output channels of its pixels");
      constexpr int RP = 20;
      static_assert(32 * RP <= 32 * LDS_LD, "the exchange rows live inside the wave's slab");
      {
        const int n16 = lane & 15, g16 = lane >> 4;
        const int c8 = n0 + wn * 32 + 8 * g16;
        const float4 bq0 = *reinterpret_cast<const float4*>(ep.bias + c8), bq1 = *reinterpret_cast<const float4*>(ep.bias + c8 + 4);
        const float b8[8] = {bq0.x, bq0.y, bq0.z, bq0.w, bq1.x, bq1.y, bq1.z, bq1.w};
        f16x8 w2h[2], w2l[2];
#pragma unroll
        for (int rbk = 0; rbk < 2; ++rbk) {
          const int u = 16 * rbk + n16;
          const float* wr = ep.w2 + (long)min(u, 17) * g.N + c8;
          const float4 wa = *reinterpret_cast<const float4*>(wr), wb = *reinterpret_cast<const float4*>(wr + 4);
          const float w8[8] = {wa.x, wa.y, wa.z, wa.w, wb.x, wb.y, wb.z, wb.w};
#pragma unroll
          for (int e = 0; e < 8; ++e) {
            const float w = u < 18 ? w8[e] * ep.w2mul : 0.f;
            w2h[rbk][e] = (_Float16)w;
            w2l[rbk][e] = (_Float16)(w - (float)w2h[rbk][e]);
          }
        }
        bool sat = false;
#pragma unroll
        for (int i = 0; i < TM; ++i) {
          slab_write(acc[i][0]);
          asm volatile("s_waitcnt lgkmcnt(0)" ::: "memory");
          __builtin_amdgcn_wave_barrier();
          f16x8 xh[2], xl[2];
#pragma unroll
          for (int pb = 0; pb < 2; ++pb) {
            const float* src = tb + (16 * pb + n16) * LDS_LD + 8 * g16;
            const float4 xa = *reinterpret_cast<const float4*>(src), xb = *reinterpret_cast<const float4*>(src + 4);
            const float x8[8] = {xa.x, xa.y, xa.z, xa.w, xb.x, xb.y, xb.z, xb.w};
#pragma unroll
            for (int e = 0; e < 8; ++e) {
              const SfPair sp = sf_split_flag(fmaxf(x8[e] + b8[e], 0.f), sat);
              xh[pb][e] = sp.hi; xl[pb][e] = sp.lo;
            }
          }
          asm volatile("s_waitcnt lgkmcnt(0)" ::: "memory");
          __builtin_amdgcn_wave_barrier();
#pragma unroll
          for (int pb = 0; pb < 2; ++pb) {
            f32x4v d0 = {0.f, 0.f, 0.f, 0.f}, d1 = {0.f, 0.f, 0.f, 0.f};
            if constexpr (!FAST) {
              d0 = __builtin_amdgcn_mfma_f32_16x16x32_f16(w2h[0], xl[pb], d0, 0, 0, 0);
              d0 = __builtin_amdgcn_mfma_f32_16x16x32_f16(w2l[0], xh[pb], d0, 0, 0, 0);
              d1 = __builtin_amdgcn_mfma_f32_16x16x32_f16(w2h[1], xl[pb], d1, 0, 0, 0);
              d1 = __builtin_amdgcn_mfma_f32_16x16x32_f16(w2l[1], xh[pb], d1, 0, 0, 0);
            }
            d0 = __builtin_amdgcn_mfma_f32_16x16x32_f16(w2h[0], xh[pb], d0, 0, 0, 0);
            d1 = __builtin_amdgcn_mfma_f32_16x16x32_f16(w2h[1], xh[pb], d1, 0, 0, 0);
            float* rp = tb + (16 * pb + n16) * RP;
            *reinterpret_cast<float4*>(rp + 4 * g16) = make_float4(d0[0] * ep.w2inv, d0[1] * ep.w2inv, d0[2] * ep.w2inv, d0[3] * ep.w2inv);
            if (g16 == 0) *reinterpret_cast<float2*>(rp + 16) = make_float2(d1[0] * ep.w2inv, d1[1] * ep.w2inv);
          }
          __syncthreads();
          for (int idx = tid; idx < 32 * 18; idx += NT) {
            const int px = idx / 18, u = idx - px * 18;
            const float* rq = reinterpret_cast<const float*>(Pbytes) + px * RP + u;
            float sum = 0.f;
#pragma unroll
            for (int w = 0; w < NW; ++w) sum += rq[w * (32 * LDS_LD)];
            const int p = i * 32 + px;
            const int oy = ty0 + p / TW, ox = tx0 + p % TW;
            if (oy < g.Ho && ox < g.Wo)
              ep.G[(long)(n0 / (NW * 32)) * ep.gstride + ((long)img * ep.npix + (long)oy * g.Wo + ox) * 18 + u] = sum;
          }
          __syncthreads();
        }
        sf_report(sat);
        return;
      }
    }
    struct NoAux {};
    using AuxT = typename std::conditional<Epi::kPrefetch, typename EpiAux4<Epi>::type, NoAux>::type;
    constexpr bool PIPE = Epi::kPrefetch && sizeof(AuxT) <= 2 * sizeof(float4);
    AuxT aux_next[PIPE ? 4 : 1];
    bool clamped = false;
    if constexpr (PIPE) {
      const int nb0 = n0 + (wn * TN) * 32 + tcol;
#pragma unroll
// ... 49 lines not shown
            asm volatile("s_waitcnt lgkmcnt(0)" ::: "memory");
            st_e_wait += st_c - st_b; st_b = st_c;
          }
#endif
#endif
#pragma unroll
          for (int q = 0; q < 4; ++q)
            if (mq[q] >= 0 && nb < g.N) {
              if constexpr (RAW) ep.apply4(img, mq[q], nb, v[q], aux[q], bj, clamped, g.wscale);
              else ep.apply4(img, mq[q], nb, v[q], aux[q], bj, clamped);
            }
#ifdef ATDN_CONV_STAMP
          if constexpr (kStamp >= 0) { asm volatile("s_waitcnt lgkmcnt(0)" ::: "memory"); st_e_apply += __builtin_amdgcn_s_memtime() - st_b; }
#endif
        } else {
#pragma unroll
          for (int q = 0; q < 4; ++q) {
            if (mq[q] < 0) continue;
            if (nb + 4 <= g.N) {
              if constexpr (RAW) ep.store4((ABL & 16) ? 0 : img, mq[q], nb, v[q], bj, clamped, g.wscale);
              else ep.store4((ABL & 16) ? 0 : img, mq[q], nb, v[q], bj, clamped);
            } else {
              const float sc = RAW ? g.wscale : 1.0f;
              const float e4[4] = {v[q].x * sc, v[q].y * sc, v[q].z * sc, v[q].w * sc};
#pragma unroll
              for (int e = 0; e < 4; ++e)
                if (nb + e < g.N) ep(img, mq[q], nb + e, e4[e]);
            }
          }
        }
      }
    }
    sf_report(clamped);
#ifdef ATDN_CONV_STAMP
    stamp_out();
#endif
    return;
  }
  constexpr int NSET = 2, NPX = 8;
  auto col_of = [&](int cs) { return 16 * cs + (lane & 15); };
  auto pix_of = [&](int e) { return 16 * (e >> 2) + 4 * (lane >> 4) + (e & 3); };
  auto val_of = [&](const SfAcc& a, int cs, int e) __attribute__((always_inline)) { return a.b[e >> 2][cs][e & 3]; };
  typename EpiCol<Epi>::type colj[TN][NSET];
  float biasj[TN][NSET];
#pragma unroll
  for (int j = 0; j < TN; ++j)
#pragma unroll
    for (int cs = 0; cs < NSET; ++cs) {
      const int n = min(n0 + (wn * TN + j) * 32 + col_of(cs), g.N - 1);
      biasj[j][cs] = 0.f;
      if constexpr (Epi::kStats) biasj[j][cs] = ep.bias[n];
      if constexpr (epi_bias_arg<Epi>::value) colj[j][cs] = ep.col(n);
    }
#pragma unroll
  for (int i = 0; i < TM; ++i) {
    const int pbase = (wm * TM + i) * 32;
    int mm[NPX];
#pragma unroll
    for (int e = 0; e < NPX; ++e) {
      mm[e] = out_pixel(pbase + pix_of(e));
    }
    int cnt = 0;
    unsigned mo[NPX];
    if constexpr (Epi::kStats) {
#pragma unroll
      for (int e = 0; e < NPX; ++e) {
        cnt += mm[e] >= 0 ? 1 : 0;
        mo[e] = (unsigned)max(mm[e], 0) * (unsigned)ep.ld;
      }
      cnt += __shfl_xor(cnt, 16);
      cnt += __shfl_xor(cnt, 32);
      cnt = __builtin_amdgcn_readfirstlane(cnt);
    }
    const bool full = cnt == 32;
    const float inv_cnt = 1.0f / (float)(cnt > 0 ? cnt : 1);
#pragma unroll
    for (int j = 0; j < TN; ++j)
#pragma unroll
      for (int cs = 0; cs < NSET; ++cs) {
        const int n = n0 + (wn * TN + j) * 32 + col_of(cs);
        const bool nok = n < g.N;
        if constexpr (Epi::kStats) {
          const float bias = nok ? biasj[j][cs] : 0.f;
          float v[NPX];
#pragma unroll
          for (int e = 0; e < NPX; ++e) v[e] = __builtin_fmaf(val_of(acc[i][j], cs, e), g.wscale, bias);
          float sum, m2;
          if (full) {
            sum = ((v[0] + v[1]) + (v[2] + v[3])) + ((v[4] + v[5]) + (v[6] + v[7]));
          } else {
            sum = 0.f;
#pragma unroll
            for (int e = 0; e < NPX; ++e) sum += mm[e] >= 0 ? v[e] : 0.f;
          }
          sum += __shfl_xor(sum, 16);
          sum += __shfl_xor(sum, 32);
          const float mean = sum * inv_cnt;
          if (full) {
            float d[NPX];
#pragma unroll
            for (int e = 0; e < NPX; ++e) d[e] = v[e] - mean;
            m2 = __builtin_fmaf(d[1], d[1], d[0] * d[0]);
#pragma unroll
            for (int e = 2; e < NPX; ++e) m2 = __builtin_fmaf(d[e], d[e], m2);
          } else {
            m2 = 0.f;
#pragma unroll
            for (int e = 0; e < NPX; ++e) { const float dd = mm[e] >= 0 ? v[e] - mean : 0.f; m2 = __builtin_fmaf(dd, dd, m2); }
          }
          m2 += __shfl_xor(m2, 16);
          m2 += __shfl_xor(m2, 32);
          const int grp = tloc * (TH * TW / 32) + wm * TM + i;
          if ((lane >> 4) == 0 && nok) {
            const long o = ((long)img * ep.groups_per_img + grp) * g.N + n;
            ep.part_sum[o] = sum;
            ep.part_m2[o] = m2;
          }
          if (lane == 0 && n == 0) ep.part_cnt[(long)img * ep.groups_per_img + grp] = (float)cnt;
          if (nok) {
            char* ob = reinterpret_cast<char*>(ep.dst + (long)img * ep.ob);
#pragma unroll
            for (int e = 0; e < NPX; ++e)
              if (full || mm[e] >= 0) *reinterpret_cast<float*>(ob + 4u * (mo[e] + (unsigned)n)) = v[e];
          }
          continue;
        }
        if (nok) {
          if constexpr (Epi::kPrefetch) {
            typename Epi::Aux aux[NPX];
#pragma unroll
            for (int e = 0; e < NPX; ++e) aux[e] = ep.load(img, max(mm[e], 0), n);
#pragma unroll
            for (int e = 0; e < NPX; ++e)
              if (mm[e] >= 0) ep.apply(img, mm[e], n, val_of(acc[i][j], cs, e) * g.wscale, aux[e]);
          } else if constexpr (epi_bias_arg<Epi>::value) {
#pragma unroll
            for (int e = 0; e < NPX; ++e)
              if (mm[e] >= 0) ep.store_c(img, mm[e], n, val_of(acc[i][j], cs, e) * g.wscale, colj[j][cs]);
          } else {
#pragma unroll
            for (int e = 0; e < NPX; ++e)
              if (mm[e] >= 0) ep(img, mm[e], n, val_of(acc[i][j], cs, e) * g.wscale);
          }
        }
      }
  }
}

template <int TH, int TW, int BN, int WM, int WN, int KH, int KW, class Epi, bool FAST = false, bool NORM = false, int ABL = 0>
__global__ __launch_bounds__(WM * WN * 64, 1) void conv_sf6_kernel(const Conv2Geom g, const Epi ep) {
  conv_sf6_body<TH, TW, BN, WM, WN, KH, KW, Epi, FAST, NORM, ABL>(g, ep, (int)blockIdx.x);
}

template <int KH, int KW, class Epi, bool FAST = false>
__global__ __launch_bounds__(256, 1) void conv_sf6_run_kernel(const Conv2Geom g, const Epi ep) {
  conv_sf6_body<8, 16, 128, 1, 4, KH, KW, Epi, FAST, false, 0, true>(g, ep, (int)blockIdx.x);
}

__device__ __forceinline__ Conv2Geom conv2_geom_pick(const Conv2Geom& a, const Conv2Geom& b, bool s) {
  Conv2Geom g;
  g.src0 = s ? b.src0 : a.src0; g.src1 = s ? b.src1 : a.src1; g.sb0 = s ? b.sb0 : a.sb0; g.sb1 = s ? b.sb1 : a.sb1;
  g.ld0 = s ? b.ld0 : a.ld0; g.ld1 = s ? b.ld1 : a.ld1; g.C0 = s ? b.C0 : a.C0; g.C1 = s ? b.C1 : a.C1;
  g.H = s ? b.H : a.H; g.W = s ? b.W : a.W; g.Ho = s ? b.Ho : a.Ho; g.Wo = s ? b.Wo : a.Wo;
  g.padH = s ? b.padH : a.padH; g.padW = s ? b.padW : a.padW; g.tiles_x = s ? b.tiles_x : a.tiles_x; g.tiles_y = s ? b.tiles_y : a.tiles_y;
  g.nimg = s ? b.nimg : a.nimg; g.ntile_n = s ? b.ntile_n : a.ntile_n;
  g.w = s ? b.w : a.w; g.N = s ? b.N : a.N; g.wscale = s ? b.wscale : a.wscale;
  g.in_mean = nullptr; g.in_rstd = nullptr;
  return g;
}
template <int TH, int TW, int BN, int WM, int WN, int KH, int KW, class Epi, bool FAST = false>
__global__ __launch_bounds__(WM * WN * 64, 1) void conv_sf6_pair_kernel(const Conv2Geom g0, const Conv2Geom g1, const Epi ep0,
                                                                        const Epi ep1, const int nblk0, const int start1) {
  const int b = (int)blockIdx.x;
  if (b >= nblk0 && b < start1) return;
  const bool second = b >= start1;
  const Conv2Geom g = conv2_geom_pick(g0, g1, second);
  const Epi ep = Epi::pick(ep0, ep1, second);
  conv_sf6_body<TH, TW, BN, WM, WN, KH, KW, Epi, FAST, false, 0>(g, ep, second ? b - start1 : b);
}

template <int TH, int BN, int WM, int WN, int KH, int KW, class Epi, bool FAST = false, bool NORM = false, int ABL = 0>
inline Conv2Geom conv_sf6_geom(const ConvShape& s, float wscale) {
  constexpr int TW = 16;
  ATDN_CHECK(s.KH == KH && s.KW == KW && s.stride == 1, "kernel shape does not match the instantiation");
  Conv2Geom g{};
  g.src0 = s.src0; g.src1 = s.src1; g.sb0 = s.sb0; g.sb1 = s.sb1; g.ld0 = s.ld0; g.ld1 = s.ld1;
  g.C0 = s.C0; g.C1 = s.C1; g.H = s.H; g.W = s.W;
  g.padH = s.padH; g.padW = s.padW;
  g.Ho = conv_out(s.H, s.KH, 1, s.padH); g.Wo = conv_out(s.W, s.KW, 1, s.padW);
  ATDN_CHECK(s.C0 % 32 == 0 && s.C1 % 32 == 0 && s.C0 > 0 && s.ld0 % 4 == 0, "TAP-mode channel constraints");
  ATDN_CHECK(s.ldw % 4 == 0 && s.ldw >= s.KH * s.KW * (s.C0 + s.C1), "weight rows too short");
  ATDN_CHECK(!epi_vec4<Epi>::value || !Epi::kPrefetch || s.N % 4 == 0, "channel-vector epilogue with operand loads needs N % 4 == 0");
  ATDN_CHECK((long)s.H * s.W < (1L << 20) - 1, "image too large for the packed patch descriptor");
  ATDN_CHECK((long)g.Ho * g.Wo * 1024L * 4L <= (1L << 32) && s.ld0 <= 1024 && s.ld1 <= 1024 && s.N <= 1024,
             "per-image slice of 4 GB or more: the 32-bit epilogue offsets would wrap");
  g.tiles_x = cdiv(g.Wo, TW); g.tiles_y = cdiv(g.Ho, TH);
  g.nimg = s.nimg; g.ntile_n = cdiv(s.N, BN);
  g.w = s.wfrag16; g.N = s.N; g.wscale = wscale;
  g.in_mean = s.in_mean; g.in_rstd = s.in_rstd;
  ATDN_CHECK(NORM == (s.in_mean != nullptr) && (!NORM || (s.in_rstd && s.C1 == 0 && s.ld0 == s.C0)),
             "normalise-on-load: one dense fp32 source with its mean / rstd");
  ATDN_CHECK(g.w != nullptr, "missing weight copy for this kernel");
  return g;
}

template <int TH, int BN, int WM, int WN, int KH, int KW, class Epi, bool FAST = false, bool NORM = false, int ABL = 0>
inline void launch_conv_sf6(const ConvShape& s, float wscale, Epi ep, hipStream_t st) {
  constexpr int TW = 16;
  const Conv2Geom g = conv_sf6_geom<TH, BN, WM, WN, KH, KW, Epi, FAST, NORM, ABL>(s, wscale);
  set_groups(ep, g.tiles_x * g.tiles_y * (TH * TW / 32));
  const int nblk = g.nimg * g.tiles_x * g.tiles_y * g.ntile_n;
  hipLaunchKernelGGL((conv_sf6_kernel<TH, TW, BN, WM, WN, KH, KW, Epi, FAST, NORM, ABL>), dim3(nblk), dim3(WM * WN * 64), 0, st, g, ep);
  ATDN_HIP(hipGetLastError());
}

template <int KH, int KW>
inline bool conv_sf6_run_eligible(const ConvShape& s) {
  if (KH * KW != 5 || s.KH != KH || s.KW != KW || s.stride != 1 || s.in_mean) return false;
  if (s.padH != KH / 2 || s.padW != KW / 2) return false;
  const int L = KH == 1 ? s.W : s.H;
  return (L + 126) / L <= 3;
}

template <int KH, int KW, class Epi, bool FAST>
inline void launch_conv_sf6_run(const ConvShape& s, float wscale, Epi ep, hipStream_t st) {
  Conv2Geom g = conv_sf6_geom<8, 128, 1, 4, KH, KW, Epi, FAST, false, 0>(s, wscale);
  ATDN_CHECK((conv_sf6_run_eligible<KH, KW>(s)) && g.Ho == g.H && g.Wo == g.W, "shape not served by the run-tile kernel");
  g.tiles_x = cdiv(g.H * g.W, 128); g.tiles_y = 1;
  const int nblk = g.nimg * g.tiles_x * g.ntile_n;
  hipLaunchKernelGGL((conv_sf6_run_kernel<KH, KW, Epi, FAST>), dim3(nblk), dim3(256), 0, st, g, ep);
  ATDN_HIP(hipGetLastError());
}

template <int TH, int BN, int WM, int WN, int KH, int KW, class Epi, bool FAST>
inline void launch_conv_sf6_pair(const ConvShape& s0, float wscale0, Epi ep0, const ConvShape& s1, float wscale1, Epi ep1,
                                 hipStream_t st) {
  constexpr int TW = 16;
  static_assert(!Epi::kStats, "the pair launch serves plain-store epilogues");
  const Conv2Geom g0 = conv_sf6_geom<TH, BN, WM, WN, KH, KW, Epi, FAST, false, 0>(s0, wscale0);
  const Conv2Geom g1 = conv_sf6_geom<TH, BN, WM, WN, KH, KW, Epi, FAST, false, 0>(s1, wscale1);
  const int nblk0 = g0.nimg * g0.tiles_x * g0.tiles_y * g0.ntile_n;
  const int start1 = (nblk0 + 7) / 8 * 8;
  const int nblk1 = g1.nimg * g1.tiles_x * g1.tiles_y * g1.ntile_n;
  hipLaunchKernelGGL((conv_sf6_pair_kernel<TH, TW, BN, WM, WN, KH, KW, Epi, FAST>), dim3(start1 + nblk1), dim3(WM * WN * 64), 0, st,
                     g0, g1, ep0, ep1, nblk0, start1);
  ATDN_HIP(hipGetLastError());
}


inline bool conv_sf6_operands_ok(const ConvShape& s) {
  return s.wfrag16 && s.stride == 1 && s.C0 % 32 == 0 && s.C1 % 32 == 0 && s.C0 > 0 && s.ld0 % 4 == 0;
}

struct Sf6Plan { int th, bn; bool run; };

template <int KH, int KW, class Epi>
inline Sf6Plan conv_sf6_plan(const ConvShape& s, bool fast) {
  constexpr bool k3 = KH == 3;
  constexpr bool plain = !Epi::kStats && !epi_flowhead<Epi>::value;
  constexpr Sf6Plan none{0, 0, false};
  const int Ho = conv_out(s.H, s.KH, 1, s.padH), Wo = conv_out(s.W, s.KW, 1, s.padW);
  const long tiles = (long)s.nimg * cdiv(Wo, 16) * cdiv(Ho, 8);
  int bn = 64;
  if (s.N <= 32 && k3) bn = 32;
  else if (s.N == 96 && k3) bn = 96;
  else {
    int best = cdiv(s.N, 64) * 64;
    for (int c : {128, 256})
      if (cdiv(s.N, c) * c <= best) { best = cdiv(s.N, c) * c; bn = c; }
  }
  while (bn > 64 && bn != 96 && tiles * cdiv(s.N, bn) < 300) bn /= 2;
  if (!k3) bn = std::min(bn, 128);
  const bool fits12 = k3 && (bn == 64 || bn == 96) && cdiv(Ho, 12) * 12 * 100 <= cdiv(Ho, 8) * 8 * 103;
  if (s.in_mean) {
    if (!Epi::kStats || !k3 || fast || bn == 32 || bn == 256) return none;
    return {fits12 ? 12 : 8, bn, false};
  }
  const bool run_ok = !k3 && plain && conv_sf6_run_eligible<KH, KW>(s);
  if (!k3 && plain && s.tile_form == 1) return {8, 128, false};
  if (run_ok && s.tile_form == 2) return {8, 128, true};
  if (plain && bn == 64 && tiles * cdiv(s.N, 64) < 300) return {4, 64, false};
  const long tiles12 = (long)s.nimg * cdiv(Wo, 16) * cdiv(Ho, 12);
  if (fits12 && (Epi::kStats || tiles12 * cdiv(s.N, bn) >= 512)) return {12, bn, false};
  if (run_ok && bn == 128) return {8, 128, true};
  return {8, bn, false};
}

template <int TH, int BN, int WM, int WN, int KH, int KW, class Epi, bool FAST>
inline void conv_sf6_launch_tile(const ConvShape& s, float wscale, const Epi& ep, hipStream_t st) {
  if (s.in_mean) {
    if constexpr (Epi::kStats && KH == 3 && !FAST && TH >= 8 && (BN == 64 || BN == 96 || BN == 128))
      return launch_conv_sf6<TH, BN, WM, WN, KH, KW, Epi, false, true>(s, wscale, ep, st);
    ATDN_CHECK(false, "no normalise-on-load kernel for this tile");
  }
  launch_conv_sf6<TH, BN, WM, WN, KH, KW, Epi, FAST, false>(s, wscale, ep, st);
}

template <int KH, int KW, class Epi, bool FAST>
inline void conv_sf6_launch(const Sf6Plan& p, const ConvShape& s, float wscale, const Epi& ep, hipStream_t st) {
  constexpr bool k3 = KH == 3;
  constexpr bool plain = !Epi::kStats && !epi_flowhead<Epi>::value;
  const int th = p.th, bn = p.bn;
  if (p.run) {
    if constexpr (!k3 && plain) return launch_conv_sf6_run<KH, KW, Epi, FAST>(s, wscale, ep, st);
  } else if (th == 4 && bn == 64) {
    if constexpr (plain) return conv_sf6_launch_tile<4, 64, 2, 2, KH, KW, Epi, FAST>(s, wscale, ep, st);
  } else if (th == 8 && bn == 64) {
    return conv_sf6_launch_tile<8, 64, 2, 2, KH, KW, Epi, FAST>(s, wscale, ep, st);
  } else if (th == 8 && bn == 128) {
    return conv_sf6_launch_tile<8, 128, 1, 4, KH, KW, Epi, FAST>(s, wscale, ep, st);
  } else if constexpr (k3) {
    if (th == 8 && bn == 32) return conv_sf6_launch_tile<8, 32, 4, 1, KH, KW, Epi, FAST>(s, wscale, ep, st);
    if (th == 8 && bn == 96) return conv_sf6_launch_tile<8, 96, 2, 3, KH, KW, Epi, FAST>(s, wscale, ep, st);
    if (th == 8 && bn == 256) return conv_sf6_launch_tile<8, 256, 1, 8, KH, KW, Epi, FAST>(s, wscale, ep, st);
    if (th == 12 && bn == 64) return conv_sf6_launch_tile<12, 64, 2, 2, KH, KW, Epi, FAST>(s, wscale, ep, st);
    if (th == 12 && bn == 96) return conv_sf6_launch_tile<12, 96, 2, 3, KH, KW, Epi, FAST>(s, wscale, ep, st);
  }
  ATDN_CHECK(false, "tile plan without a kernel for this epilogue");
}

template <class Epi>
inline bool conv_sf6_try_pair(const ConvShape& s0, float wscale0, const Epi& ep0, const ConvShape& s1, float wscale1, const Epi& ep1,
                              hipStream_t st, bool fast) {
  if constexpr ((epi_gen6<Epi>::value & 1) == 0 || Epi::kStats || epi_flowhead<Epi>::value) {
    return false;
  } else {
    auto picks_12x64 = [&](const ConvShape& s) {
      if (!conv_halo_eligible(s) || s.KH != 3 || s.KW != 3 || !conv_sf6_operands_ok(s) || s.in_mean) return false;
      if (epi_vec4<Epi>::value && (s.N % 4) != 0) return false;
      const Sf6Plan p = conv_sf6_plan<3, 3, Epi>(s, fast);
      return p.th == 12 && p.bn == 64 && !p.run;
    };
    if (!picks_12x64(s0) || !picks_12x64(s1)) return false;
    with_fast(fast, [&](auto f) {
      launch_conv_sf6_pair<12, 64, 2, 2, 3, 3, Epi, decltype(f)::value>(s0, wscale0, ep0, s1, wscale1, ep1, st);
    });
    return true;
  }
}

template <int KH, int KW, class Epi>
inline bool conv_sf6_try_taps(const ConvShape& s, float wscale, const Epi& ep, hipStream_t st, int* bn_out, int* th_out, bool fast) {
  const Sf6Plan p = conv_sf6_plan<KH, KW, Epi>(s, fast);
  if (p.th == 0) return false;
  *bn_out = p.bn; *th_out = p.th;
  with_fast(fast, [&](auto f) { conv_sf6_launch<KH, KW, Epi, decltype(f)::value>(p, s, wscale, ep, st); });
  return true;
}

template <class Epi>
inline bool conv_sf6_try(const ConvShape& s, float wscale, const Epi& ep, hipStream_t st, int* bn_out, int* th_out, bool fast) {
  constexpr int kinds = epi_gen6<Epi>::value;
  if (kinds == 0 || !conv_sf6_operands_ok(s)) return false;
  if (epi_vec4<Epi>::value && Epi::kPrefetch && (s.N % 4) != 0) return false;
  if (epi_vec4<Epi>::value && s.N < 4) return false;
  if constexpr ((kinds & 1) != 0) {
    if (s.KH == 3 && s.KW == 3) return conv_sf6_try_taps<3, 3>(s, wscale, ep, st, bn_out, th_out, fast);
  }
  if constexpr ((kinds & 2) != 0) {
    if (s.KH == 1 && s.KW == 5) return conv_sf6_try_taps<1, 5>(s, wscale, ep, st, bn_out, th_out, fast);
    if (s.KH == 5 && s.KW == 1) return conv_sf6_try_taps<5, 1>(s, wscale, ep, st, bn_out, th_out, fast);
  }
  return false;
}

}
```

atdn_vslam_amd/csrc/conv_sf_dispatch_impl.h:

```cpp
#pragma once
#include "conv_dispatch_impl.h"
#include "conv_sf.h"
#include "conv_sf6.h"
#include "epilogues_sf.h"

namespace atdn {

template <class Epi>
TileChoice conv_sf_dispatch(const ConvShape& s, float wscale, Epi ep, hipStream_t st) {
  const int Ho = conv_out(s.H, s.KH, s.stride, s.padH), Wo = conv_out(s.W, s.KW, s.stride, s.padW);
  if (conv_halo_eligible(s)) {
    int bn = 0, th = 8;
    if (conv_sf6_try(s, wscale, ep, st, &bn, &th, sf_fast_mode())) return TileChoice{th * 16, bn, cdiv(Wo, 16) * cdiv(Ho, th) * (th / 2), true};
  }
  ATDN_CHECK(s.in_mean == nullptr, "normalise-on-load is served by the halo-patch statistics kernels only");
  TileChoice t = choose_tile(s.nimg, Ho * Wo, s.N);
  t.groups_per_img = cdiv(Ho * Wo, t.BM) * (t.BM / 32);
  set_groups(ep, t.groups_per_img);
  with_fast(sf_fast_mode(), [&](auto f) {
    constexpr bool FAST = decltype(f)::value;
    if (t.BM == 128 && t.BN == 128) launch_conv_sf<2, 2, 2, 2, Epi, FAST>(s, wscale, ep, st);
    else if (t.BM == 128 && t.BN == 64) launch_conv_sf<2, 1, 2, 2, Epi, FAST>(s, wscale, ep, st);
    else if (t.BM == 128 && t.BN == 96) launch_conv_sf<1, 3, 4, 1, Epi, FAST>(s, wscale, ep, st);
    else if (t.BM == 128 && t.BN == 32) launch_conv_sf<1, 1, 4, 1, Epi, FAST>(s, wscale, ep, st);
    else launch_conv_sf<1, 1, 2, 2, Epi, FAST>(s, wscale, ep, st);
  });
  return t;
}

template <class Epi>
void conv_sf_dispatch_pair(const ConvShape& s0, float wscale0, Epi ep0, const ConvShape& s1, float wscale1, Epi ep1, hipStream_t st) {
  if (conv_sf6_try_pair(s0, wscale0, ep0, s1, wscale1, ep1, st, sf_fast_mode())) return;
  conv_sf_dispatch(s0, wscale0, ep0, st);
  conv_sf_dispatch(s1, wscale1, ep1, st);
}

#define ATDN_INSTANTIATE_CONV_SF(EPI) \
  template TileChoice conv_sf_dispatch<EPI>(const ConvShape&, float, EPI, hipStream_t);
#define ATDN_INSTANTIATE_CONV_SF_PAIR(EPI) \
  template void conv_sf_dispatch_pair<EPI>(const ConvShape&, float, EPI, const ConvShape&, float, EPI, hipStream_t);

}
```

atdn_vslam_amd/csrc/conv_sf_inst_b.hip:

```cpp
#include "conv_sf_dispatch_impl.h"
namespace atdn {
ATDN_INSTANTIATE_CONV_SF(EpiBiasStats)
ATDN_INSTANTIATE_CONV_SF(SfBiasReluAddRelu)
ATDN_INSTANTIATE_CONV_SF(SfContextSplit)
}
```

atdn_vslam_amd/csrc/gma.hip:

```cpp
#include "gma.h"
#include "small_convs.h"
#include "conv_sf.h"
#include "epilogues_sf.h"

namespace atdn { const float* zero_line(); }

namespace atdn {

extern template TileChoice conv_dispatch<MODE_TAP, EpiBias<ACT_NONE>>(const ConvShape&, EpiBias<ACT_NONE>, hipStream_t);
extern template TileChoice conv_dispatch<MODE_TAP, EpiBias<ACT_RELU>>(const ConvShape&, EpiBias<ACT_RELU>, hipStream_t);
extern template TileChoice conv_dispatch<MODE_ROW, EpiBias<ACT_RELU>>(const ConvShape&, EpiBias<ACT_RELU>, hipStream_t);
extern template TileChoice conv_dispatch<MODE_TAP, EpiBiasStats>(const ConvShape&, EpiBiasStats, hipStream_t);
extern template TileChoice conv_dispatch<MODE_ROW, EpiBiasStats>(const ConvShape&, EpiBiasStats, hipStream_t);
extern template TileChoice conv_dispatch<MODE_TAP, EpiBiasReluAddRelu>(const ConvShape&, EpiBiasReluAddRelu, hipStream_t);
extern template TileChoice conv_dispatch<MODE_TAP, EpiContextSplit>(const ConvShape&, EpiContextSplit, hipStream_t);
extern template TileChoice conv_dispatch<MODE_TAP, EpiScale>(const ConvShape&, EpiScale, hipStream_t);
extern template TileChoice conv_dispatch<MODE_TAP, EpiQK>(const ConvShape&, EpiQK, hipStream_t);
extern template TileChoice conv_dispatch<MODE_TAP, EpiStoreT>(const ConvShape&, EpiStoreT, hipStream_t);
extern template TileChoice conv_dispatch<MODE_TAP, EpiAggregate>(const ConvShape&, EpiAggregate, hipStream_t);
extern template TileChoice conv_dispatch<MODE_TAP, EpiGruZR>(const ConvShape&, EpiGruZR, hipStream_t);
extern template TileChoice conv_dispatch<MODE_TAP, EpiGruQ>(const ConvShape&, EpiGruQ, hipStream_t);
extern template TileChoice conv_dispatch<MODE_TAP, EpiFlowDelta>(const ConvShape&, EpiFlowDelta, hipStream_t);

extern template TileChoice conv_dispatch<MODE_ROW, SfBias<ACT_RELU>>(const ConvShape&, SfBias<ACT_RELU>, hipStream_t);
// ... 390 lines not shown
        pr(bi, ".downsample.out", true, R, ohw, co);
        conv_dispatch<MODE_TAP>(s2, EpiBiasReluAddRelu{Bk.c2.b, R, ohw * co, co, P, ohw * co, co}, st);
      } else {
        conv_dispatch<MODE_TAP>(s2, EpiBiasReluAddRelu{Bk.c2.b, P, ohw * co, co, R, ohw * co, co}, st);
        std::swap(P, R);
      }
    }
    pr(bi, "", true, P, ohw, co);
    h = oh; w = ow; c = co;
  }
  *out_buf = P; *outH = h; *outW = w;
}

void GmaNet::iteration(int B, hipStream_t st) {
  const long n8 = (long)B * N;
  PyramidLevels pl;
  for (int l = 0; l < 4; ++l) { pl.base[l] = pyr_[l].p; pl.H[l] = pyrH_[l]; pl.W[l] = pyrW_[l]; }
  launch_lookup(pl, coords1_.p, n8, corrfeat_.p, CORR_LD, st);
  mark(ST_LOOKUP, st);
  auto pr = [&](const char* name, bool limited, const float* p, long rows, long cols, long ld) {
    if (probe_) probe(name, limited, p, rows, cols, ld, st);
  };
  pr("corr_lookup", true, corrfeat_.p, n8, 324, CORR_LD);

  ConvShape s = conv_shape(convc1_, corrfeat_.p, CORR_LD, (long)N * CORR_LD, B, H8, W8, 1, 0, 0);
  conv_dispatch<MODE_TAP>(s, EpiBias<ACT_RELU>{convc1_.b, cor1_.p, (long)N * 256, 256, 1.f}, st);
  mark(ST_CONVC1, st);
  pr("encoder.convc1", true, cor1_.p, n8, 256, 256);
  s = conv_shape(convc2_, cor1_.p, 256, (long)N * 256, B, H8, W8, 1, 1, 1);
  conv_dispatch<MODE_TAP>(s, EpiBias<ACT_RELU>{convc2_.b, corflo_.p, (long)N * 256, 256, 1.f}, st);
  pr("encoder.convc2", true, corflo_.p, n8, convc2_.N, 256);
  s = conv_shape(convf1_, flow4_.p, 4, (long)N * 4, B, H8, W8, 1, 3, 3);
  conv_dispatch<MODE_ROW>(s, EpiBias<ACT_RELU>{convf1_.b, flo1_.p, (long)N * 128, 128, 1.f}, st);
  pr("encoder.convf1", true, flo1_.p, n8, 128, 128);
  s = conv_shape(convf2_, flo1_.p, 128, (long)N * 128, B, H8, W8, 1, 1, 1);
  conv_dispatch<MODE_TAP>(s, EpiBias<ACT_RELU>{convf2_.b, corflo_.p + 192, (long)N * 256, 256, 1.f}, st);
  pr("encoder.convf2", true, corflo_.p + 192, n8, convf2_.N, 256);
  s = conv_shape(convm_, corflo_.p, 256, (long)N * 256, B, H8, W8, 1, 1, 1);
  float* mf = x_.p + 128;
  conv_dispatch<MODE_TAP>(s, EpiBias<ACT_RELU>{convm_.b, mf, (long)N * XLD, XLD, 1.f}, st);
  mark(ST_MOTION, st);
  pr("encoder.conv", true, mf, n8, convm_.N, XLD);

  s = conv_shape(to_v_, mf, XLD, (long)N * XLD, B, H8, W8, 1, 0, 0);
  conv_dispatch<MODE_TAP>(s, EpiStoreT{vT_.p, (long)128 * ldN, ldN}, st);
  mark(ST_AGG_VT, st);
  pr("aggregator.to_v", true, vT_.p, (long)B * 128, N, ldN);
  ConvShape a;
  a.src0 = attn_.p; a.ld0 = ldN; a.sb0 = (long)N * ldN; a.C0 = ldN; a.H = 1; a.W = N;
  a.w = vT_.p; a.wb = (long)128 * ldN; a.ldw = ldN; a.N = 128; a.nimg = B;
  conv_dispatch<MODE_TAP>(a, EpiAggregate{gamma_, mf, (long)N * XLD, XLD, x_.p + 256, (long)N * XLD, XLD}, st);
  mark(ST_AGG, st);
  pr("aggregator.out", true, x_.p + 256, n8, 128, XLD);

  for (int p = 0; p < 2; ++p) {
    const float* hin = h_[p].p;
    float* hout = h_[p ^ 1].p;
    const int ph = p ? 2 : 0, pw = p ? 0 : 2;
    ConvShape g = conv_shape(gru_zr_[p], hin, 128, (long)N * 128, B, H8, W8, 1, ph, pw);
    g.C0 = 128; g.src1 = x_.p; g.ld1 = XLD; g.sb1 = (long)N * XLD; g.C1 = XLD;
    conv_dispatch<MODE_TAP>(g, EpiGruZR{gru_zr_[p].b, hin, z_.p, rh_.p, (long)N * 128}, st);
    mark(p ? ST_GRU_ZR_V : ST_GRU_ZR, st);
    pr(p ? "gru.z2" : "gru.z1", false, z_.p, n8, 128, 128);
    pr(p ? "gru.rh2" : "gru.rh1", true, rh_.p, n8, 128, 128);
    g.src0 = rh_.p; g.w = gru_q_[p].w; g.ldw = gru_q_[p].ldw; g.N = gru_q_[p].N;
    conv_dispatch<MODE_TAP>(g, EpiGruQ{gru_q_[p].b, hin, z_.p, hout, (long)N * 128}, st);
    mark(p ? ST_GRU_Q_V : ST_GRU_Q, st);
    pr(p ? "gru.h2" : "gru.h1", true, hout, n8, 128, 128);
  }

  s = conv_shape(fh1_, h_[0].p, 128, (long)N * 128, B, H8, W8, 1, 1, 1);
  conv_dispatch<MODE_TAP>(s, EpiBias<ACT_RELU>{fh1_.b, fh_.p, (long)N * 256, 256, 1.f}, st);
  pr("flow_head.conv1", true, fh_.p, n8, 256, 256);
  s = conv_shape(fh2_, fh_.p, 256, (long)N * 256, B, H8, W8, 1, 1, 1);
  conv_dispatch<MODE_TAP>(s, EpiFlowDelta{fh2_.b, coords1_.p, flow4_.p, x_.p + 254, XLD, (long)N * XLD, W8, (long)N}, st);
  mark(ST_FLOWHEAD, st);
  pr("flow", true, flow4_.p, n8, 2, 4);
  pr("coords1", false, coords1_.p, n8, 2, 2);
}

void GmaNet::run_body(int B, int iters, hipStream_t st) {
  float* f; int fh, fw;
  run_encoder(fnet_, true, 2 * B, st, &f, &fh, &fw);
  ATDN_CHECK(fh == H8 && fw == W8, "encoder geometry mismatch");
  ConvShape s = conv_shape(fnet_.head, f, 128, (long)N * 128, 2 * B, H8, W8, 1, 0, 0);
  conv_dispatch<MODE_TAP>(s, EpiBias<ACT_NONE>{fnet_.head.b, fmap_.p, (long)N * 256, 256, 1.f}, st);
  mark(ST_FNET, st);
  auto pr = [&](const char* name, bool limited, const float* p, long rows, long cols, long ld) {
    if (probe_) probe(name, limited, p, rows, cols, ld, st);
  };
  pr("fnet.conv2", true, fmap_.p, 2L * B * N, 256, 256);

  ConvShape c;
  c.src0 = fmap_.p; c.ld0 = 256; c.sb0 = (long)N * 256; c.C0 = 256; c.H = 1; c.W = N;
  c.w = fmap_.p + (long)B * N * 256; c.wb = (long)N * 256; c.ldw = 256; c.N = N; c.nimg = B;
  conv_dispatch<MODE_TAP>(c, EpiScale{1.0f / sqrtf(256.0f), pyr_[0].p, (long)N * N, N}, st);
  mark(ST_CORR, st);
  pr("corr.0", false, pyr_[0].p, (long)B * N, N, N);
  for (int l = 1; l < 4; ++l) {
    launch_avgpool(pyr_[l - 1].p, pyrH_[l - 1], pyrW_[l - 1], pyr_[l].p, (long)B * N, st);
    if (probe_) probe("corr." + std::to_string(l), false, pyr_[l].p, (long)B * N, (long)pyrH_[l] * pyrW_[l], (long)pyrH_[l] * pyrW_[l], st);
  }
  mark(ST_POOL, st);

  run_encoder(cnet_, false, B, st, &f, &fh, &fw);
  s = conv_shape(cnet_.head, f, 128, (long)N * 128, B, H8, W8, 1, 0, 0);
  conv_dispatch<MODE_TAP>(s, EpiContextSplit{cnet_.head.b, h_[0].p, (long)N * 128, x_.p, (long)N * XLD, XLD}, st);
  mark(ST_CNET, st);
  pr("net0", true, h_[0].p, (long)B * N, 128, 128);
  pr("inp", true, x_.p, (long)B * N, 128, XLD);

  s = conv_shape(to_qk_, x_.p, XLD, (long)N * XLD, B, H8, W8, 1, 0, 0);
  conv_dispatch<MODE_TAP>(s, EpiQK{1.0f / sqrtf(128.0f), 128, qk_.p, (long)N * 256, 256}, st);
  pr("att.qk", true, qk_.p, (long)B * N, 256, 256);
  ConvShape q;
  q.src0 = qk_.p; q.ld0 = 256; q.sb0 = (long)N * 256; q.C0 = 128; q.H = 1; q.W = N;
  q.w = qk_.p + 128; q.wb = (long)N * 256; q.ldw = 256; q.N = N; q.nimg = B;
  conv_dispatch<MODE_TAP>(q, EpiScale{1.0f, attn_.p, (long)N * ldN, ldN}, st);
  mark(ST_ATTN_LOGITS, st);
  pr("att.logits", false, attn_.p, (long)B * N, N, ldN);
  launch_softmax_rows(attn_.p, (long)B * N, N, ldN, st);
  mark(ST_ATTN, st);
  pr("att.attn", false, attn_.p, (long)B * N, N, ldN);

  for (int it = 0; it < iters; ++it) {
    probe_it_ = it;
    iteration(B, st);
    if (preds_out_) {
      mask_head(B, st);
      launch_upsample(mask_.p, flow4_.p, B, H8, W8, nullptr, preds_out_ + it * preds_stride_, st);
      pr("flow_up", false, preds_out_ + it * preds_stride_, 1, preds_stride_, preds_stride_);
    }
  }
  probe_it_ = -1;
  if (!preds_out_) mask_head(B, st);
  mark(ST_MASK, st);
}

void GmaNet::mask_head(int B, hipStream_t st) {
  ConvShape s = conv_shape(mask0_, h_[0].p, 128, (long)N * 128, B, H8, W8, 1, 1, 1);
  conv_dispatch<MODE_TAP>(s, EpiBias<ACT_RELU>{mask0_.b, fh_.p, (long)N * 256, 256, 1.f}, st);
  if (probe_) probe("mask.0", true, fh_.p, (long)B * N, 256, 256, st);
  s = conv_shape(mask2_, fh_.p, 256, (long)N * 256, B, H8, W8, 1, 0, 0);
  conv_dispatch<MODE_TAP>(s, EpiBias<ACT_NONE>{mask2_.b, mask_.p, (long)N * 576, 576, 0.25f}, st);
  if (probe_) probe("mask", false, mask_.p, (long)B * N, 576, 576, st);
}

void GmaNet::run_encoder_sf(const EncoderWeights& E, bool instance, int nimg, hipStream_t st, float** out_buf, int first_img,
                            DeviceBuf* bufs, float* final_dst) {
  const float* images = img4_.p + (long)first_img * H * W * 4;
  int h = conv_out(H, 7, 2, 3), w = conv_out(W, 7, 2, 3);
  DeviceBuf* eb = bufs ? bufs : enc_;
  float* X = eb[0].p; float* R = eb[1].p; float* Y = eb[2].p; float* O = eb[3].p;
  auto stats_sf = [&](const PackedConv& L, const float* src, int ld, int ih, int iw, int stride, int pad, float* dst,
                      int slot, int in_slot = -1) {
    ConvShape s = conv_shape(L, src, ld, (long)ih * iw * ld, nimg, ih, iw, stride, pad, pad);
    if (in_slot >= 0) { s.in_mean = mean_[in_slot].p; s.in_rstd = rstd_[in_slot].p; }
    const int oh = conv_out(ih, L.KH, stride, pad), ow = conv_out(iw, L.KW, stride, pad);
    EpiBiasStats ep{L.b, dst, (long)oh * ow * L.N, L.N, psum_.p, pm2_.p, 0, pcnt_.p};
    TileChoice t = conv_sf_dispatch(s, L.wscale, ep, st);
    const int groups = t.groups_per_img;
    ATDN_CHECK((long)nimg * groups * L.N <= psum_.n && (long)nimg * groups <= pcnt_.n, "statistics scratch too small");
    if (t.counted)
      launch_in_finalize_cnt(psum_.p, pm2_.p, pcnt_.p, nimg, groups, oh * ow, L.N, 1e-5f, mean_[slot].p,
                             rstd_[slot].p, reinterpret_cast<double*>(fin_.p), st);
    else
      launch_in_finalize_cnt(psum_.p, pm2_.p, nullptr, nimg, groups, oh * ow, L.N, 1e-5f, mean_[slot].p, rstd_[slot].p,
                             reinterpret_cast<double*>(fin_.p), st);
  };
  const bool stem_raw = instance && norm_on_load_;
  if (stem_raw) {
    const int groups = stem_sf_groups(h, w);
    ATDN_CHECK((long)nimg * groups * 64 <= psum_.n && (long)nimg * groups <= pcnt_.n, "statistics scratch too small");
    launch_stem_sf(3, images, nimg, H, W, E.stem.wf, E.stem.wscale, E.stem.b, X, psum_.p, pm2_.p, pcnt_.p, nullptr, nullptr, st);
    launch_in_finalize_cnt(psum_.p, pm2_.p, pcnt_.p, nimg, groups, h * w, 64, 1e-5f, mean_[2].p, rstd_[2].p,
                           reinterpret_cast<double*>(fin_.p), st);
  } else if (instance) {
    const int groups = stem_sf_groups(h, w);
    ATDN_CHECK((long)nimg * groups * 64 <= psum_.n && (long)nimg * groups <= pcnt_.n, "statistics scratch too small");
    launch_stem_sf(1, images, nimg, H, W, E.stem.wf, E.stem.wscale, E.stem.b, nullptr, psum_.p, pm2_.p, pcnt_.p, nullptr,
                   nullptr, st);
    launch_in_finalize_cnt(psum_.p, pm2_.p, pcnt_.p, nimg, groups, h * w, 64, 1e-5f, mean_[0].p, rstd_[0].p,
                           reinterpret_cast<double*>(fin_.p), st);
    launch_stem_sf(2, images, nimg, H, W, E.stem.wf, E.stem.wscale, E.stem.b, X, nullptr, nullptr, nullptr, mean_[0].p,
                   rstd_[0].p, st);
  } else {
    launch_stem_sf(0, images, nimg, H, W, E.stem.wf, E.stem.wscale, E.stem.b, X, nullptr, nullptr, nullptr, nullptr,
                   nullptr, st);
  }
  int c = 64;
  for (int bi = 0; bi < 6; ++bi) {
    const auto& Bk = E.blk[bi];
    const int stride = Bk.has_ds ? 2 : 1;
    const int co = Bk.c1.N;
    const int oh = conv_out(h, 3, stride, 1), ow = conv_out(w, 3, stride, 1);
    const long ohw = (long)oh * ow;
    if (bi == 5 && final_dst) O = final_dst;
    if (instance && norm_on_load_) {
      const bool raw_in = stem_raw && bi == 0;
      ATDN_CHECK(!raw_in || !Bk.has_ds, "the block behind the stem has no downsample branch");
      stats_sf(Bk.c1, X, c, h, w, stride, 1, R, 0, raw_in ? 2 : -1);
      stats_sf(Bk.c2, R, co, oh, ow, 1, 1, Y, 1, 0);
      if (Bk.has_ds) {
        stats_sf(Bk.ds, X, c, h, w, 2, 0, R, 0);
        launch_in_apply_sf(Y, O, mean_[1].p, rstd_[1].p, nullptr, R, mean_[0].p, rstd_[0].p, nimg, ohw, co, st);
      } else if (raw_in) {
        launch_in_apply_sf(Y, O, mean_[1].p, rstd_[1].p, nullptr, X, mean_[2].p, rstd_[2].p, nimg, ohw, co, st, true);
      } else {
        launch_in_apply_sf(Y, O, mean_[1].p, rstd_[1].p, X, nullptr, nullptr, nullptr, nimg, ohw, co, st);
      }
    } else if (instance) {
      stats_sf(Bk.c1, X, c, h, w, stride, 1, R, 0);
      launch_in_apply_sf(R, Y, mean_[0].p, rstd_[0].p, nullptr, nullptr, nullptr, nullptr, nimg, ohw, co, st);
      stats_sf(Bk.c2, Y, co, oh, ow, 1, 1, R, 0);
      if (Bk.has_ds) {
        stats_sf(Bk.ds, X, c, h, w, 2, 0, Y, 1);
        launch_in_apply_sf(R, O, mean_[0].p, rstd_[0].p, nullptr, Y, mean_[1].p, rstd_[1].p, nimg, ohw, co, st);
      } else {
        launch_in_apply_sf(R, O, mean_[0].p, rstd_[0].p, X, nullptr, nullptr, nullptr, nimg, ohw, co, st);
      }
    } else {
      const float* res = X;
      if (Bk.has_ds) {
        ConvShape sd = conv_shape(Bk.ds, X, c, (long)h * w * c, nimg, h, w, 2, 0, 0);
        conv_sf_dispatch(sd, Bk.ds.wscale, SfBias<ACT_NONE>{Bk.ds.b, R, ohw * co, co}, st);
        res = R;
      }
      ConvShape s1 = conv_shape(Bk.c1, X, c, (long)h * w * c, nimg, h, w, stride, 1, 1);
      conv_sf_dispatch(s1, Bk.c1.wscale, SfBias<ACT_RELU>{Bk.c1.b, Y, ohw * co, co}, st);
      ConvShape s2 = conv_shape(Bk.c2, Y, co, ohw * co, nimg, oh, ow, 1, 1, 1);
      conv_sf_dispatch(s2, Bk.c2.wscale, SfBiasReluAddRelu{Bk.c2.b, res, ohw * co, co, O, ohw * co, co}, st);
    }
    std::swap(X, O);
    h = oh; w = ow; c = co;
  }
  ATDN_CHECK(h == H8 && w == W8, "encoder geometry mismatch");
  *out_buf = X;
}

void GmaNet::iteration_sf(int B, hipStream_t st) {
  const long n8 = (long)B * N;
  ConvShape s;
  if (par_) fork(st, par_stream_);
  launch_lookup_conv(brick_pyramid(), coords1_.p, n8, coords_used_.p, convc1_.wf16, convc1_.wscale, convc1_.b, cor1_.p,
                     sf_fast_mode(), st);
  mark(ST_LOOKUP, st);
  s = conv_shape(convc2_, cor1_.p, 256, (long)N * 256, B, H8, W8, 1, 1, 1);
  const ConvShape sf2 = conv_shape(convf2_, flo1_.p, 128, (long)N * 128, B, H8, W8, 1, 1, 1);
  if (par_) {
    launch_flow_conv7_sf(flow4_.p, B, H8, W8, arena_.dev(convf1_sf_off_), convf1_wscale_, convf1_.b, flo1_.p, sf_fast_mode(), par_stream_);
    conv_sf_dispatch(sf2, convf2_.wscale, SfBias<ACT_RELU>{convf2_.b, corflo_.p + 192, (long)N * 256, 256}, par_stream_);
    conv_sf_dispatch(s, convc2_.wscale, SfBias<ACT_RELU>{convc2_.b, corflo_.p, (long)N * 256, 256}, st);
    fork(par_stream_, st);
  } else {
    launch_flow_conv7_sf(flow4_.p, B, H8, W8, arena_.dev(convf1_sf_off_), convf1_wscale_, convf1_.b, flo1_.p, sf_fast_mode(), st);
    conv_sf_dispatch_pair(s, convc2_.wscale, SfBias<ACT_RELU>{convc2_.b, corflo_.p, (long)N * 256, 256},
                          sf2, convf2_.wscale, SfBias<ACT_RELU>{convf2_.b, corflo_.p + 192, (long)N * 256, 256}, st);
  }
  s = conv_shape(convm_, corflo_.p, 256, (long)N * 256, B, H8, W8, 1, 1, 1);
  float* mf = x_.p + 128;
  conv_sf_dispatch(s, convm_.wscale, SfBias<ACT_RELU>{convm_.b, mf, (long)N * XLD, XLD}, st);
  mark(ST_MOTION, st);

  launch_attn_v(attn_.p, rinv_.p, attn_geom(B, N, ldN), nullptr, nullptr, mf, x_.p + 256, (long)N * XLD, XLD,
                sf_fast_mode(), st, attn_part_.p);
  mark(ST_AGG, st);

  for (int p = 0; p < 2; ++p) {
    const float* hin = h_[p].p;
    float* hout = h_[p ^ 1].p;
    const int ph = p ? 2 : 0, pw = p ? 0 : 2;
    ConvShape g = conv_shape(gru_zr_[p], hin, 128, (long)N * 128, B, H8, W8, 1, ph, pw);
    g.C0 = 128; g.src1 = x_.p + 128; g.ld1 = XLD; g.sb1 = (long)N * XLD; g.C1 = 256;
    conv_sf_dispatch(g, gru_zr_[p].wscale,
                     SfGruZR{gru_zr_[p].b, hin, z_.p, rh_.p, (long)N * 128, pre_zr_[p].p, (long)N * 256}, st);
    mark(p ? ST_GRU_ZR_V : ST_GRU_ZR, st);
    g.src0 = rh_.p; g.w = gru_q_[p].w; g.wfrag16 = gru_q_[p].wf16; g.ldw = gru_q_[p].ldw; g.N = gru_q_[p].N;
    conv_sf_dispatch(g, gru_q_[p].wscale, SfGruQ{gru_q_[p].b, hin, z_.p, hout, (long)N * 128, pre_q_[p].p}, st);
    mark(p ? ST_GRU_Q_V : ST_GRU_Q, st);
  }

  s = conv_shape(fh1_, h_[0].p, 128, (long)N * 128, B, H8, W8, 1, 1, 1);
  const SfFlowDelta fd{fh2_.b, coords1_.p, flow4_.p, x_.p, XLD, (long)N * XLD, 254, W8, (long)N};
  const long fh_gs = (long)maxB * N * 18;
  launch_flow_head_fused(s, fh1_.wscale, SfFlowHeadPartial{fh1_.b, arena_.dev(fh2_w32_off_), fhG_.p, (long)N, fh2_mul_, 1.0f / fh2_mul_, fh_gs}, st);
  launch_flow_gather(fhG_.p, fh_gs, B, H8, W8, fd, st);
  mark(ST_FLOWHEAD, st);
}

void GmaNet::run_body_sf(int B, int iters, hipStream_t st) {
  float* f;
  const int nfeat = seq_ == 0 ? 2 * B : seq_ == 1 ? B + 1 : B;
  hipStream_t sB = par_ ? par_stream_ : st;
  if (par_) fork(st, sB);
  run_encoder_sf(fnet_, true, nfeat, st, &f, seq_ == 2 ? 1 : 0, nullptr, fpre_.p + (seq_ == 2 ? (long)N * 128 : 0));
  ConvShape s = conv_shape(fhead_fold_, fpre_.p, 128, (long)N * 128, B, H8, W8, 1, 0, 0);
  conv_sf_dispatch(s, fhead_fold_.wscale, SfBias<ACT_NONE>{fhead_fold_.b, fsrc_.p, (long)N * 160, 160}, st);
  mark(ST_FNET, st);

  const float* target = fpre_.p + (long)(seq_ ? 1 : B) * N * 128;
  for (int l = 0; l < 4; ++l) {
    const float* plain = target;
    long plain_sb = (long)N * 128;
    if (l > 0) {
      const float* prev = l == 1 ? target : fplain_[l - 2].p;
      const long prev_sb = l == 1 ? (long)N * 128 : (long)pyrH_[l - 1] * pyrW_[l - 1] * 128;
      plain_sb = (long)pyrH_[l] * pyrW_[l] * 128;
      launch_pool_features_sf(prev, B, pyrH_[l - 1], pyrW_[l - 1], 128, prev_sb, fplain_[l - 1].p, plain_sb, st);
      plain = fplain_[l - 1].p;
    }
    launch_brick_rows(plain, plain_sb, B, pyrH_[l], pyrW_[l], 128, 160, fbrick_[l].p, (long)brickNB_[l] * 160, st);
    launch_corr_bricks(fsrc_.p, (long)N * 160, fbrick_[l].p, (long)brickNB_[l] * 160, B, N, brickNB_[l], 160,
                       corr_mul_ / sqrtf(256.0f), pyr_[l].p, sf_fast_mode(), st);
    if (l == 0) mark(ST_CORR, st);
  }
  mark(ST_POOL, st);

  run_encoder_sf(cnet_, false, B, sB, &f, 0, par_ ? enc2_ : nullptr);
  s = conv_shape(cnet_.head, f, 128, (long)N * 128, B, H8, W8, 1, 0, 0);
  conv_sf_dispatch(s, cnet_.head.wscale,
                   SfContextSplit{cnet_.head.b, h_[0].p, (long)N * 128, x_.p, (long)N * XLD, XLD}, sB);
  mark(ST_CNET, st);

  s = conv_shape(to_qk_, x_.p, XLD, (long)N * XLD, B, H8, W8, 1, 0, 0);
  conv_sf_dispatch(s, to_qk_.wscale, SfQK{1.0f / sqrtf(128.0f), 128, qk_.p, (long)N * 256, 256}, sB);
  {
    const AttnGeom ag = attn_geom(B, N, ldN);
    launch_qk_rowmax(qk_.p, ag, rowmax_.p, sB);
    mark(ST_ATTN_LOGITS, st);
    launch_qk_softmax(qk_.p, ag, rowmax_.p, attn_.p, rinv_.p, sf_fast_mode(), sB);
  }
  mark(ST_ATTN, st);

  for (int p = 0; p < 2; ++p) {
    const int ph = p ? 2 : 0, pw = p ? 0 : 2;
    ConvShape g = conv_shape(gru_zr_ctx_[p], x_.p, XLD, (long)N * XLD, B, H8, W8, 1, ph, pw);
    conv_sf_dispatch(g, gru_zr_ctx_[p].wscale, EpiBias<ACT_NONE>{nullptr, pre_zr_[p].p, (long)N * 256, 256, 1.f}, sB);
    g = conv_shape(gru_q_ctx_[p], x_.p, XLD, (long)N * XLD, B, H8, W8, 1, ph, pw);
    conv_sf_dispatch(g, gru_q_ctx_[p].wscale, EpiBias<ACT_NONE>{nullptr, pre_q_[p].p, (long)N * 128, 128, 1.f}, sB);
  }
  mark(ST_GRU_CTX, st);
  if (par_) fork(sB, st);

  for (int it = 0; it < iters; ++it) {
    iteration_sf(B, st);
    if (preds_out_) {
      mask_head_sf(B, st);
      launch_upsample(mask_.p, flow4_.p, B, H8, W8, nullptr, preds_out_ + it * preds_stride_, st);
    }
  }
  if (!preds_out_) mask_head_sf(B, st);
  mark(ST_MASK, st);
}

void GmaNet::mask_head_sf(int B, hipStream_t st) {
  ConvShape s = conv_shape(mask0_, h_[0].p, 128, (long)N * 128, B, H8, W8, 1, 1, 1);
  conv_sf_dispatch(s, mask0_.wscale, SfBias<ACT_RELU>{mask0_.b, fh_.p, (long)N * 256, 256}, st);
  s = conv_shape(mask2_, fh_.p, 256, (long)N * 256, B, H8, W8, 1, 0, 0);
  conv_sf_dispatch(s, mask2_.wscale, EpiBias<ACT_NONE>{mask2_.b, mask_.p, (long)N * 576, 576, 0.25f}, st);
}
// ... 207 lines not shown
```

atdn_vslam_amd/csrc/kernels.hip:

```cpp
#include "kernels.h"
#include "sf.h"

namespace atdn {

bool& sf_fast_mode() {
  static thread_local bool fast = false;
  return fast;
}

__device__ __forceinline__ float wave_sum(float v) {
#pragma unroll
  for (int o = 32; o > 0; o >>= 1) v += __shfl_xor(v, o);
  return v;
}
__device__ __forceinline__ float wave_max(float v) {
#pragma unroll
  for (int o = 32; o > 0; o >>= 1) v = fmaxf(v, __shfl_xor(v, o));
  return v;
}
template <bool MAX>
__device__ __forceinline__ float block_reduce(float v, float* sm) {
  v = MAX ? wave_max(v) : wave_sum(v);
  __syncthreads();
  if ((threadIdx.x & 63) == 0) sm[threadIdx.x >> 6] = v;
// ... 348 lines not shown
  for (int b = 0; b < B; ++b) {
    float acc = 0.f;
    const float4* w = reinterpret_cast<const float4*>(W0 + (long)n * K0);
    const float4* x = reinterpret_cast<const float4*>(x0 + (long)b * ldx0);
    for (int k = lane; k < K0 / 4; k += 64) {
      const float4 a = w[k], v = x[k];
      acc += a.x * v.x + a.y * v.y + a.z * v.z + a.w * v.w;
    }
    if (W1) {
      const float4* w1 = reinterpret_cast<const float4*>(W1 + (long)n * K1);
      const float4* x1v = reinterpret_cast<const float4*>(x1 + (long)b * ldx1);
      for (int k = lane; k < K1 / 4; k += 64) {
        const float4 a = w1[k], v = x1v[k];
        acc += a.x * v.x + a.y * v.y + a.z * v.z + a.w * v.w;
      }
    }
    acc = wave_sum(acc);
    if (lane == 0) {
      float v = acc + (b0 ? b0[n] : 0.f) + (b1 ? b1[n] : 0.f);
      if (act == 1) v = mishf_(v);
      y[(long)b * ldy + n] = v;
    }
  }
}
void launch_linear(const float* W0, const float* x0, int K0, int ldx0, const float* W1, const float* x1, int K1,
                   int ldx1, const float* b0, const float* b1, int act, float* y, int ldy, int N, int B,
                   hipStream_t st) {
  ATDN_CHECK(K0 % 4 == 0 && K1 % 4 == 0 && ldx0 % 4 == 0 && ldx1 % 4 == 0, "linear: K and ld must be multiples of 4");
  hipLaunchKernelGGL(linear_kernel, dim3(cdiv(N, 4)), dim3(256), 0, st, W0, x0, K0, ldx0, W1, x1, K1, ldx1, b0, b1, act,
                     y, ldy, N, B);
  ATDN_HIP(hipGetLastError());
}

__global__ __launch_bounds__(256) void lstm_pipe_kernel(const LstmPipeArgs a) {
  __shared__ float gate[4];
  const int Hd = a.Hd, lane = threadIdx.x & 63, wv = threadIdx.x >> 6;
  auto dot = [&](const float* __restrict__ wrow, const float* __restrict__ x) {
    float acc = 0.f;
    for (int k = lane; k < Hd / 4; k += 64) {
      const float4 w = reinterpret_cast<const float4*>(wrow)[k];
      const float4 v = reinterpret_cast<const float4*>(x)[k];
      acc += w.x * v.x + w.y * v.y + w.z * v.z + w.w * v.w;
    }
    return wave_sum(acc);
  };
  int blk = blockIdx.x;
  if (blk < Hd) {
    if (!a.do1) return;
    const int j = blk;
    for (int b = 0; b < a.B; ++b) {
      const float acc = dot(a.Whh1 + ((long)wv * Hd + j) * Hd, a.h1_in + (long)b * Hd);
      if (lane == 0) gate[wv] = a.pre1[(long)b * 4 * Hd + wv * Hd + j] + (acc + a.bhh1[wv * Hd + j]);
      __syncthreads();
      if (threadIdx.x == 0) {
        const float cn = sigmoidf_(gate[1]) * a.c1[(long)b * Hd + j] + sigmoidf_(gate[0]) * tanhf(gate[2]);
        a.c1[(long)b * Hd + j] = cn;
        a.h1_out[(long)b * Hd + j] = sigmoidf_(gate[3]) * tanhf(cn);
      }
      __syncthreads();
    }
    return;
  }
  blk -= Hd;
  if (blk < Hd / 4) {
    if (!a.do_lin) return;
    const int j = blk * 4 + wv;
    for (int b = 0; b < a.B; ++b) {
      const float acc = dot(a.Wlin + (long)j * Hd, a.lin_in + (long)b * Hd);
      if (lane == 0) a.lin_out[(long)b * Hd + j] = mishf_(acc + a.blin[j]);
    }
    return;
  }
  blk -= Hd / 4;
  if (!a.do2) return;
  const int j = blk;
  for (int b = 0; b < a.B; ++b) {
    const float ax = dot(a.Wih2 + ((long)wv * Hd + j) * Hd, a.x2_in + (long)b * Hd);
    const float ah = dot(a.Whh2 + ((long)wv * Hd + j) * Hd, a.h2_in + (long)b * Hd);
    if (lane == 0) gate[wv] = (ax + a.bih2[wv * Hd + j]) + (ah + a.bhh2[wv * Hd + j]);
    __syncthreads();
    if (threadIdx.x == 0) {
      const float cn = sigmoidf_(gate[1]) * a.c2[(long)b * Hd + j] + sigmoidf_(gate[0]) * tanhf(gate[2]);
      a.c2[(long)b * Hd + j] = cn;
      a.h2_out[(long)b * Hd + j] = sigmoidf_(gate[3]) * tanhf(cn);
    }
    __syncthreads();
  }
}
void launch_lstm_pipe(const LstmPipeArgs& a, hipStream_t st) {
  ATDN_CHECK(a.Hd % 16 == 0 && a.B >= 1, "lstm_pipe: bad arguments");
  hipLaunchKernelGGL(lstm_pipe_kernel, dim3(2 * a.Hd + a.Hd / 4), dim3(256), 0, st, a);
  ATDN_HIP(hipGetLastError());
}

__global__ __launch_bounds__(256) void mlp_heads_kernel(const float* __restrict__ h2, MlpHead rot, MlpHead tr,
                                                        float* __restrict__ rot_out, float* __restrict__ tr_out) {
  __shared__ float x[512];
  __shared__ float a1[2][128];
  __shared__ float a2[2][64];
  const int b = blockIdx.x, t = threadIdx.x;
  x[t] = h2[(long)b * 512 + t];
  x[t + 256] = h2[(long)b * 512 + 256 + t];
  __syncthreads();
  const int hd = t >> 7, u = t & 127;
  const MlpHead& H = hd ? tr : rot;
  {
    const float* w = H.w0 + (long)u * 512;
    float acc = 0.f;
    for (int k = 0; k < 512; ++k) acc += w[k] * x[k];
    a1[hd][u] = mishf_(acc + H.b0[u]);
  }
  __syncthreads();
  if (u < 64) {
    const float* w = H.w1 + (long)u * 128;
    float acc = 0.f;
    for (int k = 0; k < 128; ++k) acc += w[k] * a1[hd][k];
    a2[hd][u] = mishf_(acc + H.b1[u]);
  }
  __syncthreads();
  if (u < 3) {
    const float* w = H.w2 + (long)u * 64;
    float acc = 0.f;
    for (int k = 0; k < 64; ++k) acc += w[k] * a2[hd][k];
    (hd ? tr_out : rot_out)[(long)b * 3 + u] = acc;
  }
}
void launch_mlp_heads(const float* h2, int B, MlpHead rot, MlpHead tr, float* rot_out, float* tr_out, hipStream_t st) {
  hipLaunchKernelGGL(mlp_heads_kernel, dim3(B), dim3(256), 0, st, h2, rot, tr, rot_out, tr_out);
  ATDN_HIP(hipGetLastError());
}

const float* zero_line() {
  static float* z = nullptr;
  if (!z) {
    ATDN_HIP(hipMalloc(&z, 256));
    ATDN_HIP(hipMemset(z, 0, 256));
    ATDN_HIP(hipDeviceSynchronize());
  }
  return z;
}

__global__ void fill_kernel(float* p, long n, float v) {
  for (long i = (long)blockIdx.x * blockDim.x + threadIdx.x; i < n; i += (long)gridDim.x * blockDim.x) p[i] = v;
}
void launch_fill(float* p, long n, float v, hipStream_t st) {
  if (n <= 0) return;
  hipLaunchKernelGGL(fill_kernel, dim3((unsigned)std::min<long>(cdivl(n, 256), 4096)), dim3(256), 0, st, p, n, v);
  ATDN_HIP(hipGetLastError());
}

}

#include "sf.h"
#include <mutex>
#include <vector>
namespace atdn {

namespace {
std::vector<void (*)(unsigned int*)>& sf_counter_setters() { static std::vector<void (*)(unsigned int*)> v; return v; }
std::mutex g_sf_counter_mutex;
struct SfCounterDev { int dev; unsigned int* ptr; };
std::vector<SfCounterDev> g_sf_counters;
unsigned int* sf_counter_for_current_device(bool create) {
  int dev = 0;
  ATDN_HIP(hipGetDevice(&dev));
  for (auto& c : g_sf_counters) if (c.dev == dev) return c.ptr;
  if (!create) return nullptr;
  unsigned int* p = nullptr;
  ATDN_HIP(hipMalloc(&p, 2 * sizeof(unsigned int)));
  ATDN_HIP(hipMemset(p, 0, 2 * sizeof(unsigned int)));
  for (auto set : sf_counter_setters()) {
    set(p);
    ATDN_HIP(hipGetLastError());
  }
  ATDN_HIP(hipDeviceSynchronize());
  g_sf_counters.push_back({dev, p});
  return p;
}
}
void sf_counter_register(void (*setter)(unsigned int*)) { sf_counter_setters().push_back(setter); }
void sf_counter_attach() {
  std::lock_guard<std::mutex> lock(g_sf_counter_mutex);
  (void)sf_counter_for_current_device(true);
}
__global__ void sf_counter_exchange_kernel(unsigned int* counter, unsigned int* out) { *out = atomicExch(counter, 0u); }
unsigned int sf_counter_read_reset(hipStream_t st) {
  std::lock_guard<std::mutex> lock(g_sf_counter_mutex);
  unsigned int* p = sf_counter_for_current_device(true);
  unsigned int* slot = p + 1;
  unsigned int v = 0;
  hipLaunchKernelGGL(sf_counter_exchange_kernel, dim3(1), dim3(1), 0, st, p, slot);
  ATDN_HIP(hipGetLastError());
  ATDN_HIP(hipMemcpyAsync(&v, slot, sizeof(v), hipMemcpyDeviceToHost, st));
  ATDN_HIP(hipStreamSynchronize(st));
  return v;
}

__device__ __forceinline__ void sf_store4(float* dst, long i4, float4 v) {
  const long grp = i4 >> 3;
  const int sl = (int)(i4 & 7);
  _Float16* g = reinterpret_cast<_Float16*>(dst + grp * 32) + sl * 4;
  const SfPair a = sf_split(v.x), b = sf_split(v.y), c = sf_split(v.z), d = sf_split(v.w);
  typedef _Float16 h4 __attribute__((ext_vector_type(4)));
  h4 hi = {a.hi, b.hi, c.hi, d.hi};
  h4 lo = {a.lo, b.lo, c.lo, d.lo};
  *reinterpret_cast<h4*>(g) = hi;
  *reinterpret_cast<h4*>(g + 32) = lo;
}
__device__ __forceinline__ float4 sf_load4(const float* src, long i4) {
  const long grp = i4 >> 3;
  const int sl = (int)(i4 & 7);
  const _Float16* g = reinterpret_cast<const _Float16*>(src + grp * 32) + sl * 4;
  typedef _Float16 h4 __attribute__((ext_vector_type(4)));
  const h4 hi = *reinterpret_cast<const h4*>(g);
  const h4 lo = *reinterpret_cast<const h4*>(g + 32);
  return make_float4((float)hi[0] + (float)lo[0], (float)hi[1] + (float)lo[1], (float)hi[2] + (float)lo[2],
                     (float)hi[3] + (float)lo[3]);
}

__global__ void to_sf_kernel(const float4* __restrict__ src, float* __restrict__ dst, long total4) {
  for (long i = (long)blockIdx.x * blockDim.x + threadIdx.x; i < total4; i += (long)gridDim.x * blockDim.x)
    sf_store4(dst, i, src[i]);
}
void launch_to_sf(const float* src, float* dst, long rows, int C, hipStream_t st) {
  ATDN_CHECK(C % 32 == 0, "sf tensors need C % 32 == 0");
  const long total4 = rows * C / 4;
  hipLaunchKernelGGL(to_sf_kernel, dim3((unsigned)std::min<long>(cdivl(total4, 256), 4096)), dim3(256), 0, st,
                     reinterpret_cast<const float4*>(src), dst, total4);
  ATDN_HIP(hipGetLastError());
}
__global__ void from_sf_kernel(const float* __restrict__ src, float4* __restrict__ dst, long total4) {
  for (long i = (long)blockIdx.x * blockDim.x + threadIdx.x; i < total4; i += (long)gridDim.x * blockDim.x)
    dst[i] = sf_load4(src, i);
}
void launch_from_sf(const float* src, float* dst, long rows, int C, hipStream_t st) {
  ATDN_CHECK(C % 32 == 0, "sf tensors need C % 32 == 0");
  const long total4 = rows * C / 4;
  hipLaunchKernelGGL(from_sf_kernel, dim3((unsigned)std::min<long>(cdivl(total4, 256), 4096)), dim3(256), 0, st, src,
                     reinterpret_cast<float4*>(dst), total4);
  ATDN_HIP(hipGetLastError());
}

__global__ __launch_bounds__(128) void mfg_reconstruct_kernel(float* __restrict__ x, int ld, int cmf, int cagg,
                                                              const float* __restrict__ wv, const float* __restrict__ gamma,
                                                              const float* __restrict__ coords_used, int N, int W8, int cflow) {
  __shared__ float a[128];
  const long pix = blockIdx.x;
  float* row = x + pix * ld;
  const int c = threadIdx.x;
  a[c] = row[cagg + c];
  __syncthreads();
  float s = 0.f;
  for (int k = 0; k < 128; ++k) s = fmaf(wv[c * 128 + k], a[k], s);
  float m = row[cmf + c];
  const int n = cmf + c - cflow;
  if (coords_used && (n == 0 || n == 1)) {
    const int p = (int)(pix % N);
    const float f = coords_used[pix * 2 + n] - (n == 0 ? (float)(p % W8) : (float)(p / W8));
    const _Float16 hi = (_Float16)f;
    m = (float)hi + (float)(_Float16)(f - (float)hi);
  }
  row[cagg + c] = m + gamma[0] * s;
}

void launch_mfg_reconstruct(float* x, long rows, int ld, int cmf, int cagg, const float* wv, const float* gamma,
                            const float* coords_used, int N, int W8, int cflow, hipStream_t st) {
  if (rows <= 0) return;
  hipLaunchKernelGGL(mfg_reconstruct_kernel, dim3((unsigned)rows), dim3(128), 0, st, x, ld, cmf, cagg, wv, gamma, coords_used, N, W8, cflow);
  ATDN_HIP(hipGetLastError());
}

__global__ __launch_bounds__(256) void linear_rows_kernel(const float* __restrict__ in, int Cin, const float* __restrict__ w,
                                                          const float* __restrict__ b, int Cout, float* __restrict__ out) {
  __shared__ float a[256];
  const long r = blockIdx.x;
  for (int c = threadIdx.x; c < Cin; c += blockDim.x) a[c] = in[r * Cin + c];
  __syncthreads();
  for (int o = threadIdx.x; o < Cout; o += blockDim.x) {
    float s = b ? b[o] : 0.f;
    for (int k = 0; k < Cin; ++k) s = fmaf(w[(long)o * Cin + k], a[k], s);
    out[r * Cout + o] = s;
  }
}

void launch_linear_rows(const float* in, long rows, int Cin, const float* w, const float* b, int Cout, float* out, hipStream_t st) {
  ATDN_CHECK(Cin >= 1 && Cin <= 256 && Cout >= 1, "linear_rows: bad geometry");
  if (rows <= 0) return;
  hipLaunchKernelGGL(linear_rows_kernel, dim3((unsigned)rows), dim3(256), 0, st, in, Cin, w, b, Cout, out);
  ATDN_HIP(hipGetLastError());
}

__global__ void in_apply_sf_kernel(const float4* __restrict__ x, float* __restrict__ y, const float* __restrict__ mean,
                                   const float* __restrict__ rstd, const float* __restrict__ res,
                                   const float4* __restrict__ res_raw, const float* __restrict__ rmean,
                                   const float* __restrict__ rrstd, int res_relu, long per_img4, int C, long total4) {
  for (long i = (long)blockIdx.x * blockDim.x + threadIdx.x; i < total4; i += (long)gridDim.x * blockDim.x) {
    const long img = i / per_img4;
    const int c = (int)((i * 4) % C);
    const float* mu = mean + img * C + c;
    const float* rs = rstd + img * C + c;
    float4 v = x[i];
    v.x = fmaxf((v.x - mu[0]) * rs[0], 0.f);
    v.y = fmaxf((v.y - mu[1]) * rs[1], 0.f);
    v.z = fmaxf((v.z - mu[2]) * rs[2], 0.f);
    v.w = fmaxf((v.w - mu[3]) * rs[3], 0.f);
    if (res || res_raw) {
      float4 r;
      if (res) {
        r = sf_load4(res, i);
      } else {
        r = res_raw[i];
        const float* m2 = rmean + img * C + c;
        const float* r2 = rrstd + img * C + c;
        r.x = (r.x - m2[0]) * r2[0]; r.y = (r.y - m2[1]) * r2[1];
        r.z = (r.z - m2[2]) * r2[2]; r.w = (r.w - m2[3]) * r2[3];
        if (res_relu) {
          r.x = fmaxf(r.x, 0.f); r.y = fmaxf(r.y, 0.f); r.z = fmaxf(r.z, 0.f); r.w = fmaxf(r.w, 0.f);
        }
      }
      v.x = fmaxf(r.x + v.x, 0.f); v.y = fmaxf(r.y + v.y, 0.f);
      v.z = fmaxf(r.z + v.z, 0.f); v.w = fmaxf(r.w + v.w, 0.f);
    }
    sf_store4(y, i, v);
  }
}
void launch_in_apply_sf(const float* x, float* y, const float* mean, const float* rstd, const float* res,
                        const float* res_raw, const float* rmean, const float* rrstd, int nimg, long HW, int C,
                        hipStream_t st, bool res_relu) {
  ATDN_CHECK(C % 32 == 0, "sf tensors need C % 32 == 0");
  const long per_img4 = HW * C / 4, total4 = per_img4 * nimg;
  const int grid = (int)std::min<long>(cdivl(total4, 256), 256 * 16);
  hipLaunchKernelGGL(in_apply_sf_kernel, dim3(grid), dim3(256), 0, st, reinterpret_cast<const float4*>(x), y, mean,
                     rstd, res, reinterpret_cast<const float4*>(res_raw), rmean, rrstd, res_relu ? 1 : 0, per_img4, C, total4);
  ATDN_HIP(hipGetLastError());
}

__global__ void pool_features_sf_kernel(const float* __restrict__ src, int H, int W, int C, long sb, float* __restrict__ dst,
                                        long db, long total) {
  const long i = (long)blockIdx.x * blockDim.x + threadIdx.x;
  if (i >= total) return;
  const int Ho = H / 2, Wo = W / 2, c4 = C / 4;
  const int cq = (int)(i % c4);
  const long pq = i / c4;
  const int po = (int)(pq % ((long)Ho * Wo));
  const long img = pq / ((long)Ho * Wo);
  const int y = po / Wo, x = po - y * Wo;
  const float* s = src + img * sb;
  const long p00 = ((long)(2 * y) * W + 2 * x) * C;
  const float4 a = sf_load4(s, p00, 4 * cq), b = sf_load4(s, p00 + C, 4 * cq);
  const float4 c = sf_load4(s, p00 + (long)W * C, 4 * cq), d = sf_load4(s, p00 + (long)W * C + C, 4 * cq);
  const float4 o = make_float4((((a.x + b.x) + c.x) + d.x) * 0.25f, (((a.y + b.y) + c.y) + d.y) * 0.25f,
                               (((a.z + b.z) + c.z) + d.z) * 0.25f, (((a.w + b.w) + c.w) + d.w) * 0.25f);
  sf_store4(dst + img * db, (long)po * C, 4 * cq, o);
}
void launch_pool_features_sf(const float* src, int nimg, int H, int W, int C, long sb, float* dst, long db, hipStream_t st) {
  ATDN_CHECK(C % 32 == 0, "sf tensors need C % 32 == 0");
  const long total = (long)nimg * (H / 2) * (W / 2) * (C / 4);
  hipLaunchKernelGGL(pool_features_sf_kernel, dim3((unsigned)cdivl(total, 256)), dim3(256), 0, st, src, H, W, C, sb, dst, db, total);
  ATDN_HIP(hipGetLastError());
}

__global__ void init_coords_sf_kernel(const float* __restrict__ flow_init, int B, int H8, int W8,
                                      float* __restrict__ coords1, float* __restrict__ flow4, float* __restrict__ x,
                                      int ldx, int cflow) {
  const long N = (long)H8 * W8;
  const long i = (long)blockIdx.x * blockDim.x + threadIdx.x;
  if (i >= B * N) return;
  const long img = i / N;
  const int m = (int)(i - img * N);
  const float x0 = (float)(m % W8), y0 = (float)(m / W8);
  float fx = 0.f, fy = 0.f;
  if (flow_init) { fx = flow_init[(img * 2 + 0) * N + m]; fy = flow_init[(img * 2 + 1) * N + m]; }
  const float cx = x0 + fx, cy = y0 + fy;
  coords1[i * 2 + 0] = cx;
  coords1[i * 2 + 1] = cy;
  const float flx = cx - x0, fly = cy - y0;
  reinterpret_cast<float4*>(flow4)[i] = make_float4(flx, fly, 0.f, 0.f);
  sf_store(x, i * ldx, cflow, flx);
  sf_store(x, i * ldx, cflow + 1, fly);
}
void launch_init_coords_sf(const float* flow_init, int B, int H8, int W8, float* coords1, float* flow4, float* x,
                           int ldx, int cflow, hipStream_t st) {
  const long n = (long)B * H8 * W8;
  hipLaunchKernelGGL(init_coords_sf_kernel, dim3((unsigned)cdivl(n, 256)), dim3(256), 0, st, flow_init, B, H8, W8,
                     coords1, flow4, x, ldx, cflow);
  ATDN_HIP(hipGetLastError());
}

}
```

include/atdn_hip.h:

```cpp
#ifndef ATDN_HIP_H
#define ATDN_HIP_H

#include <stddef.h>
#include <stdint.h>

#ifdef __cplusplus
extern "C" {
#endif

typedef struct atdn_gma atdn_gma;
typedef struct atdn_clvo atdn_clvo;
typedef struct atdn_vae atdn_vae;
typedef struct atdn_clvo_trainer atdn_clvo_trainer;

int atdn_version(void);
const char* atdn_last_error(void);


#define ATDN_PRECISION_F32 0
#define ATDN_PRECISION_SPLIT_F16 1
#define ATDN_PRECISION_F16 2
int atdn_gma_create(atdn_gma** out, int H, int W, int max_batch, int precision);

int atdn_gma_set_low_latency(atdn_gma* h, int on);
// ... 114 lines not shown
                                  float* depth, int* counts);

int atdn_depth_backproject(const float* depth, int B, int H, int W, double fx, double fy, double cx, double cy, float* points,
                           void* stream);

int atdn_flow_track_step(const float* flow, const unsigned char* mask, const float* acc_in, const unsigned char* alive_in, int B,
                         int H, int W, float* acc_out, unsigned char* alive_out, const float* pose, double fx, double fy, double cx,
                         double cy, double max_epipolar, double min_sin2, double max_depth, float* depth, int* counts, void* stream);
int atdn_flow_track_step_host(const float* flow, const unsigned char* mask, const float* acc_in, const unsigned char* alive_in,
                              int B, int H, int W, float* acc_out, unsigned char* alive_out, const float* pose, double fx,
                              double fy, double cx, double cy, double max_epipolar, double min_sin2, double max_depth, float* depth,
                              int* counts);

int atdn_depth_fuse(const float* bank, const float* poses, const int* targets, const int* sources, int N, int B, int S, int H, int W,
                    double fx, double fy, double cx, double cy, double max_reproj, double max_rel_depth, int min_views, double min_z,
                    int average, float* fused, unsigned char* views, int* counts, void* stream);
int atdn_depth_fuse_host(const float* bank, const float* poses, const int* targets, const int* sources, int N, int B, int S, int H,
                         int W, double fx, double fy, double cx, double cy, double max_reproj, double max_rel_depth, int min_views,
                         double min_z, int average, float* fused, unsigned char* views, int* counts);

#define ATDN_MULTIVIEW_MAX_VIEWS 16
int atdn_multiview_depth(const float* acc_bank, const unsigned char* alive_bank, const float* poses, const int* slots,
                         const float* depth_init, int N, int B, int S, int H, int W, double fx, double fy, double cx, double cy,
                         double scale_px, double inlier_px, double min_z, int min_views, double max_rel_sigma, double max_depth,
                         int iters, float* depth, float* info, unsigned char* views, int* counts, void* stream);
int atdn_multiview_depth_host(const float* acc_bank, const unsigned char* alive_bank, const float* poses, const int* slots,
                              const float* depth_init, int N, int B, int S, int H, int W, double fx, double fy, double cx, double cy,
                              double scale_px, double inlier_px, double min_z, int min_views, double max_rel_sigma, double max_depth,
                              int iters, float* depth, float* info, unsigned char* views, int* counts);

long atdn_bundle_workspace_bytes(int B, int S, int H, int W, int stride);
int atdn_bundle_terms(const float* acc_bank, const unsigned char* alive_bank, const float* poses, const int* slots,
                      const float* depth, const unsigned char* mask, int N, int B, int S, int H, int W, double fx, double fy,
                      double cx, double cy, int stride, double scale_px, double inlier_px, double min_z, int min_views, double* sums,
                      int* counts, void* workspace, void* stream);
int atdn_bundle_adjust(const float* acc_bank, const unsigned char* alive_bank, const float* poses, const int* slots,
                       const float* depth_init, const unsigned char* mask, int N, int B, int S, int H, int W, double fx, double fy,
                       double cx, double cy, int stride, int iters, double scale_px, double inlier_px, double min_z, int min_views,
                       float* poses_out, float* depth, double* cost, int* counts, void* workspace, void* stream);
int atdn_bundle_terms_host(const float* acc_bank, const unsigned char* alive_bank, const float* poses, const int* slots,
                           const float* depth, const unsigned char* mask, int N, int B, int S, int H, int W, double fx, double fy,
                           double cx, double cy, int stride, double scale_px, double inlier_px, double min_z, int min_views,
                           double* sums, int* counts);
int atdn_bundle_adjust_host(const float* acc_bank, const unsigned char* alive_bank, const float* poses, const int* slots,
                            const float* depth_init, const unsigned char* mask, int N, int B, int S, int H, int W, double fx,
                            double fy, double cx, double cy, int stride, int iters, double scale_px, double inlier_px, double min_z,
                            int min_views, float* poses_out, float* depth, double* cost, int* counts);


long atdn_pnp_workspace_bytes(int B, int H, int W);

int atdn_pnp_terms(const float* depth, const float* flow, const unsigned char* mask, const float* pose, int B, int H, int W,
                   double fx, double fy, double cx, double cy, double scale_px, double inlier_px, double min_z, double* sums,
                   int* counts, void* workspace, void* stream);
int atdn_pnp_terms_host(const float* depth, const float* flow, const unsigned char* mask, const float* pose, int B, int H, int W,
                        double fx, double fy, double cx, double cy, double scale_px, double inlier_px, double min_z, double* sums,
                        int* counts);

int atdn_pnp_solve(const float* depth, const float* flow, const unsigned char* mask, const float* pose_init, int B, int H, int W,
                   double fx, double fy, double cx, double cy, double scale_px, double inlier_px, double min_z, int iters,
                   float* pose_out, double* cost, int* counts, void* workspace, void* stream);
int atdn_pnp_solve_host(const float* depth, const float* flow, const unsigned char* mask, const float* pose_init, int B, int H,
                        int W, double fx, double fy, double cx, double cy, double scale_px, double inlier_px, double min_z, int iters,
                        float* pose_out, double* cost, int* counts);


long atdn_epipolar_workspace_bytes(int B, int H, int W);

int atdn_epipolar_terms(const float* flow, const unsigned char* mask, const float* pose, int B, int H, int W, double fx, double fy,
                        double cx, double cy, double scale_px, double inlier_px, double* sums, int* counts, void* workspace,
                        void* stream);
int atdn_epipolar_terms_host(const float* flow, const unsigned char* mask, const float* pose, int B, int H, int W, double fx,
                             double fy, double cx, double cy, double scale_px, double inlier_px, double* sums, int* counts);

int atdn_epipolar_solve(const float* flow, const unsigned char* mask, const float* pose_init, int B, int H, int W, double fx,
                        double fy, double cx, double cy, double scale_px, double inlier_px, int iters, float* pose_out, double* cost,
                        int* counts, void* workspace, void* stream);
int atdn_epipolar_solve_host(const float* flow, const unsigned char* mask, const float* pose_init, int B, int H, int W, double fx,
                             double fy, double cx, double cy, double scale_px, double inlier_px, int iters, float* pose_out,
                             double* cost, int* counts);


long atdn_ground_workspace_bytes(int B, int H, int W);

int atdn_ground_terms(const float* depth, const unsigned char* mask, const double* q, int B, int H, int W, int y0, int y1, double fx,
                      double fy, double cx, double cy, double scale_rel, double inlier_rel, double min_z, double max_depth,
                      double* sums, int* counts, void* workspace, void* stream);
int atdn_ground_terms_host(const float* depth, const unsigned char* mask, const double* q, int B, int H, int W, int y0, int y1,
                           double fx, double fy, double cx, double cy, double scale_rel, double inlier_rel, double min_z,
                           double max_depth, double* sums, int* counts);

int atdn_ground_solve(const float* depth, const unsigned char* mask, const double* q_init, int B, int H, int W, int y0, int y1,
                      double fx, double fy, double cx, double cy, double nx, double ny, double nz, double scale_rel,
                      double inlier_rel, double min_z, double max_depth, int min_votes, int iters, double* q, double* sums,
                      int* counts, void* workspace, void* stream);
int atdn_ground_solve_host(const float* depth, const unsigned char* mask, const double* q_init, int B, int H, int W, int y0, int y1,
                           double fx, double fy, double cx, double cy, double nx, double ny, double nz, double scale_rel,
                           double inlier_rel, double min_z, double max_depth, int min_votes, int iters, double* q, double* sums,
                           int* counts);

int atdn_ground_classify(const float* depth, const unsigned char* mask, const double* q, int B, int H, int W, int y0, int y1,
                         double fx, double fy, double cx, double cy, double inlier_rel, double min_z, double max_depth,
                         float* residual, unsigned char* on_ground, void* stream);
int atdn_ground_classify_host(const float* depth, const unsigned char* mask, const double* q, int B, int H, int W, int y0, int y1,
                              double fx, double fy, double cx, double cy, double inlier_rel, double min_z, double max_depth,
                              float* residual, unsigned char* on_ground);


long atdn_pose_graph_workspace_bytes(int B, int N, int E);

int atdn_pose_graph_terms(const float* poses, const int* edge_index, const float* edge_pose, const double* edge_weight,
                          const unsigned char* edge_robust, int B, int N, int E, double robust_scale, double* cost,
                          double* edge_chi2, int* counts, void* workspace, void* stream);
int atdn_pose_graph_terms_host(const float* poses, const int* edge_index, const float* edge_pose, const double* edge_weight,
                               const unsigned char* edge_robust, int B, int N, int E, double robust_scale, double* cost,
                               double* edge_chi2, int* counts);

int atdn_pose_graph_solve(const float* poses, const int* edge_index, const float* edge_pose, const double* edge_weight,
                          const unsigned char* edge_robust, const unsigned char* fixed, int B, int N, int E, double robust_scale,
                          int iters, int cg_iters, double cg_tol, float* poses_out, double* cost, double* edge_chi2, int* counts,
                          void* workspace, void* stream);
int atdn_pose_graph_solve_host(const float* poses, const int* edge_index, const float* edge_pose, const double* edge_weight,
                               const unsigned char* edge_robust, const unsigned char* fixed, int B, int N, int E,
                               double robust_scale, int iters, int cg_iters, double cg_tol, float* poses_out, double* cost,
                               double* edge_chi2, int* counts);


int atdn_map_search(const float* bank, int K, int D, const float* queries, int Q, int topk, float* dist, int* idx, void* stream);

int atdn_map_gather_images_u8(const uint8_t* bank, int K, long plane_bytes, const int* index_host, int n, float* out, void* stream);


int atdn_corr_lookup(const float* pyr0, const float* pyr1, const float* pyr2, const float* pyr3, int B, int H8,
                     int W8, const float* coords, float* out, int ldo, void* stream);

int atdn_corr_pyramid(const float* fmap1, const float* fmap2, int B, int H8, int W8, int C, float* pyr0, float* pyr1,
                      float* pyr2, float* pyr3, void* stream);

int atdn_corr_lookup_bricks(const float* fmap1, const float* fmap2, int B, int H8, int W8, int C, const float* coords,
                            float* pyr0, float* pyr1, float* pyr2, float* pyr3, float* samples,
                            const float* convc1_weight_host, const float* convc1_bias_host, float* cor1, void* stream);

int atdn_conv2d_nhwc(const float* src, int nimg, int H, int W, int Cin, const float* weight_host,
                     const float* bias_host, int Cout, int KH, int KW, int stride, int padH, int padW, int relu,
                     float* dst, void* stream);

int atdn_conv2d_nhwc_sf(const float* src, int nimg, int H, int W, int Cin, const float* weight_host,
                        const float* bias_host, int Cout, int KH, int KW, int stride, int padH, int padW, float* dst,
                        void* stream);
int atdn_conv2d_nhwc_sf_epi(const float* src, int nimg, int H, int W, int Cin, const float* weight_host,
                            const float* bias_host, int Cout, int KH, int KW, int stride, int padH, int padW, int sf_store,
                            float* dst, void* stream);

#ifdef __cplusplus
}
#endif
#endif
```

Before: 447.5 frame-pairs/s.

## Fold instance-norm residual apply into next block's conv patch loader

In the GMA encoder, the norm+shortcut+relu apply pass after the first block of a layer is folded into the next 3x3 convolution's normalise-on-load patch loader. The loader reads the raw conv output and the raw shortcut, computes the residual, and both stages it in LDS and writes the owned pixels back to the output buffer. This removes one elementwise pass over the activations, with its launch and round trip through HBM. In exchange the kernel issues more vector loads and stores and needs extra scheduling groups and registers, and it applies only to certain widths and tile plans. A C API entry point is added to test the fused path.

```diff
diff --git a/atdn_vslam_amd/_lib.py b/atdn_vslam_amd/_lib.py
--- a/atdn_vslam_amd/_lib.py
+++ b/atdn_vslam_amd/_lib.py
@@ -143,6 +143,8 @@
                                       C.c_int, C.c_int, C.c_int, _vp, _vp]),
     "atdn_conv2d_nhwc_sf_epi": (C.c_int, [_vp, C.c_int, C.c_int, C.c_int, C.c_int, _vp, _vp, C.c_int, C.c_int, C.c_int,
                                       C.c_int, C.c_int, C.c_int, C.c_int, _vp, _vp]),
+    "atdn_conv3x3_stats_residual": (C.c_int, [_vp, _vp, _vp, _vp, _vp, _vp, C.c_int, C.c_int, C.c_int, C.c_int, C.c_int, _vp, _vp,
+                                              C.c_int, C.c_int, _vp, _vp, _vp, _vp, _vp, C.c_long, C.POINTER(C.c_int), _vp]),
 }
 
 GMA_STAGES = ("fnet", "corr", "pool", "cnet", "attention", "lookup", "motion_encoder", "aggregate", "gru_zr", "gru_q",
diff --git a/atdn_vslam_amd/csrc/capi.hip b/atdn_vslam_amd/csrc/capi.hip
--- a/atdn_vslam_amd/csrc/capi.hip
+++ b/atdn_vslam_amd/csrc/capi.hip
@@ -32,6 +32,7 @@
 
 extern template TileChoice conv_sf_dispatch<EpiBias<ACT_NONE>>(const ConvShape&, float, EpiBias<ACT_NONE>, hipStream_t);
 extern template TileChoice conv_sf_dispatch<SfBias<ACT_NONE>>(const ConvShape&, float, SfBias<ACT_NONE>, hipStream_t);
+extern template TileChoice conv_sf_dispatch<EpiBiasStats>(const ConvShape&, float, EpiBiasStats, hipStream_t);
 
 static thread_local std::string g_last_error;
 void set_last_error(const std::string& msg) { g_last_error = msg; }
@@ -789,6 +790,59 @@
   ATDN_API_END
 }
 
+int atdn_conv3x3_stats_residual(const float* y_raw, const float* y_mean, const float* y_rstd, const float* shortcut,
+                                const float* x_mean, const float* x_rstd, int x_relu, int nimg, int H, int W, int C,
+                                const float* weight_host, const float* bias_host, int Cout, int mode, float* o_sf, float* dst,
+                                float* part_sum, float* part_m2, float* part_cnt, long part_groups_cap, int* groups_per_img,
+                                void* stream) {
+  ATDN_API_BEGIN
+  ATDN_CHECK(y_raw && y_mean && y_rstd && shortcut && weight_host && o_sf && dst && part_sum && part_m2 && part_cnt && groups_per_img,
+             "null argument");
+  ATDN_CHECK(nimg >= 1 && H >= 1 && W >= 1 && C % 32 == 0 && Cout % 32 == 0, "bad geometry (C and Cout must be multiples of 32)");
+  ATDN_CHECK((x_mean != nullptr) == (x_rstd != nullptr), "the raw shortcut takes both its mean and its rstd");
+  ATDN_CHECK(mode >= 0 && mode <= 2, "mode: 0 separate pass, 1 residual-on-load, 2 residual-on-load at the layer's block width");
+  StateDict sd;
+  const int64_t ws[4] = {Cout, C, 3, 3};
+  sd.put("c.weight", weight_host, ws, 4);
+  std::vector<float> zb(Cout, 0.f);
+  const int64_t bs[1] = {Cout};
+  sd.put("c.bias", bias_host ? bias_host : zb.data(), bs, 1);
+  WeightArena A;
+  PackedConv L = pack_conv_sf(A, sd, {"c"});
+  A.upload();
+  resolve(A, L);
+  hipStream_t st = (hipStream_t)stream;
+  const long rows = (long)nimg * H * W;
+  DeviceBuf xsf;
+  if (!x_mean) {
+    xsf.alloc(rows * C);
+    launch_to_sf(shortcut, xsf.p, rows, C, st);
+  }
+  ConvShape s;
+  s.ld0 = C; s.sb0 = (long)H * W * C; s.C0 = L.C; s.H = H; s.W = W;
+  s.KH = 3; s.KW = 3; s.stride = 1; s.padH = 1; s.padW = 1;
+  s.w = L.w; s.ldw = L.ldw; s.N = Cout; s.nimg = nimg; s.wfrag16 = L.wf16;
+  if (mode == 0) {
+    launch_in_apply_sf(y_raw, o_sf, y_mean, y_rstd, x_mean ? nullptr : xsf.p, x_mean ? shortcut : nullptr, x_mean, x_rstd, nimg,
+                       (long)H * W, C, st, x_relu != 0);
+    s.src0 = o_sf;
+  } else {
+    s.src0 = y_raw; s.in_mean = y_mean; s.in_rstd = y_rstd;
+    if (x_mean) { s.res_raw = shortcut; s.res_mean = x_mean; s.res_rstd = x_rstd; s.res_relu = x_relu != 0; }
+    else s.res_sf = xsf.p;
+    s.res_dst = o_sf;
+    s.tile_form = mode == 2 ? 1 : 0;
+  }
+  const long groups_max = (long)cdiv(W, 16) * std::max(cdiv(H, 8) * 4, cdiv(H, 12) * 6);
+  ATDN_CHECK(groups_max <= part_groups_cap, "statistics buffers too small for this geometry");
+  EpiBiasStats ep{L.b, dst, (long)H * W * Cout, Cout, part_sum, part_m2, 0, part_cnt};
+  const TileChoice t = conv_sf_dispatch(s, L.wscale, ep, st);
+  ATDN_CHECK(t.counted && t.groups_per_img <= part_groups_cap, "the convolution left the halo-patch path");
+  *groups_per_img = t.groups_per_img;
+  ATDN_HIP(hipStreamSynchronize(st));
+  ATDN_API_END
+}
+
 int atdn_conv2d_nhwc_sf(const float* src, int nimg, int H, int W, int Cin, const float* weight_host,
                         const float* bias_host, int Cout, int KH, int KW, int stride, int padH, int padW, float* dst,
                         void* stream) {
diff --git a/atdn_vslam_amd/csrc/conv_mfma.h b/atdn_vslam_amd/csrc/conv_mfma.h
--- a/atdn_vslam_amd/csrc/conv_mfma.h
+++ b/atdn_vslam_amd/csrc/conv_mfma.h
@@ -238,6 +238,9 @@
   int N = 0;
   int nimg = 1;
   const float* in_mean = nullptr; const float* in_rstd = nullptr;
+  const float* res_sf = nullptr; const float* res_raw = nullptr; const float* res_mean = nullptr; const float* res_rstd = nullptr;
+  bool res_relu = false;
+  float* res_dst = nullptr;
   int tile_form = 0;
 };
 
diff --git a/atdn_vslam_amd/csrc/conv_sf.h b/atdn_vslam_amd/csrc/conv_sf.h
--- a/atdn_vslam_amd/csrc/conv_sf.h
+++ b/atdn_vslam_amd/csrc/conv_sf.h
@@ -250,5 +250,6 @@
 TileChoice conv_sf_dispatch(const ConvShape& s, float wscale, Epi ep, hipStream_t st);
 template <class Epi>
 void conv_sf_dispatch_pair(const ConvShape& s0, float wscale0, Epi ep0, const ConvShape& s1, float wscale1, Epi ep1, hipStream_t st);
-
-}
+bool conv_sf_res_on_load_fits(const ConvShape& s);
+
+}
diff --git a/atdn_vslam_amd/csrc/conv_sf6.h b/atdn_vslam_amd/csrc/conv_sf6.h
--- a/atdn_vslam_amd/csrc/conv_sf6.h
+++ b/atdn_vslam_amd/csrc/conv_sf6.h
@@ -1,6 +1,7 @@
 #pragma once
 #include <type_traits>
 #include "conv_sf.h"
+#include "in_residual.h"
 
 namespace atdn {
 
@@ -15,6 +16,7 @@
   const float* w; int N;
   float wscale;
   const float* in_mean; const float* in_rstd;
+  const float* res; const float* res_mean; const float* res_rstd; float* res_dst; int res_relu;
 };
 
 inline bool conv_halo_eligible(const ConvShape& s) {
@@ -45,9 +47,10 @@
 #endif
 
 template <int TH, int TW, int BN, int WM, int WN, int KH, int KW, class Epi, bool FAST = false, bool NORM = false, int ABL = 0,
-          bool RUN = false>
+          bool RUN = false, int RES = 0>
 __device__ __forceinline__ void conv_sf6_body(const Conv2Geom& g, const Epi& ep, const int bidx) {
   static_assert(ABL == 0 || !NORM, "ablation builds exist for the plain patch loader");
+  static_assert(RES == 0 || (NORM && KH == 3 && KW == 3 && !RUN && Epi::kStats), "residual-on-load rides on the normalise-on-load loader");
   static_assert(!RUN || (((KH == 1 && KW == 5) || (KH == 5 && KW == 1)) && TH == 8 && BN == 128 && WM == 1 && WN == 4 && !NORM &&
                          ABL == 0 && !Epi::kStats && !epi_flowhead<Epi>::value),
                 "run tiles: separable passes on the 8 x 16 x 128 block, plain loader, epilogues without statistics");
@@ -106,6 +109,7 @@
   const int s = tid & 7, r0 = !NORM ? tid >> 3 : ((tid >> 6) << 3) + 2 * (jrow & 1) + ((jrow >> 1) & 1) + 4 * (jrow >> 2);
   static_assert(PSZ / 16 <= 4096, "LDS offset field");
   unsigned pmeta[NP];
+  [[maybe_unused]] unsigned owned = 0;
 #pragma unroll
   for (int k = 0; k < NP; ++k) {
     const int prow = r0 + RSTEP * k;
@@ -126,6 +130,9 @@
       if ((unsigned)iy < (unsigned)g.H && (unsigned)ix < (unsigned)g.W) off = (unsigned)(iy * g.W + ix) + 1u;
     }
     pmeta[k] = (off << 12) | (unsigned)((py * RS + px * ROWB + 16 * s) >> 4);
+    if constexpr (RES != 0) {
+      if (off != 0 && (unsigned)(py - g.padH) < (unsigned)TH && (unsigned)(px - g.padW) < (unsigned)TW) owned |= 1u << k;
+    }
     if (prow >= PROWS) pmeta[k] = pmeta[0];
   }
   const float* s0 = g.src0 + (long)img * g.sb0;
@@ -151,13 +158,63 @@
     nmu = *reinterpret_cast<const float4*>(g.in_mean + (long)img * g.C0 + (c << 5) + 4 * s);
     nrs = *reinterpret_cast<const float4*>(g.in_rstd + (long)img * g.C0 + (c << 5) + 4 * s);
   };
+  float4 xr[RES != 0 ? NP : 1];
+  float4 xmu = make_float4(0.f, 0.f, 0.f, 0.f), xrs = make_float4(1.f, 1.f, 1.f, 1.f);
+  [[maybe_unused]] const unsigned obytes = 4u * (unsigned)(g.H * g.W) * (unsigned)g.ld0;
+#if defined(__HIP_DEVICE_COMPILE__)
+  const int rbytes = RES != 0 ? (int)obytes : 0;
+  const __amdgpu_buffer_rsrc_t orsrc = __builtin_amdgcn_make_buffer_rsrc(RES != 0 ? g.res_dst + (long)img * g.sb0 : nullptr, 0, rbytes, 0x00020000);
+  const __amdgpu_buffer_rsrc_t yrsrc = __builtin_amdgcn_make_buffer_rsrc(RES != 0 ? const_cast<float*>(s0) : nullptr, 0, rbytes, 0x00020000);
+  const __amdgpu_buffer_rsrc_t xrsrc =
+      __builtin_amdgcn_make_buffer_rsrc(RES != 0 ? const_cast<float*>(g.res + (long)img * g.sb0) : nullptr, 0, rbytes, 0x00020000);
+#endif
+  constexpr int RL = BN == 128 ? 1 : 3;
+  auto fetch_res_row = [&](int c, int k, bool live) {
+#if defined(__HIP_DEVICE_COMPILE__)
+    if constexpr (RES != 0) {
+      typedef unsigned u32x4 __attribute__((ext_vector_type(4)));
+      typedef unsigned u32x2 __attribute__((ext_vector_type(2)));
+      const unsigned pix = pmeta[k] >> 12;
+      const unsigned bo = (live && pix != 0) ? 4u * (pix - 1u) * (unsigned)g.ld0 : obytes;
+      const u32x4 yv = __builtin_amdgcn_raw_buffer_load_b128(yrsrc, (int)(bo + 16u * (unsigned)s), c << 7, 0);
+      pr[k] = make_float4(__uint_as_float(yv[0]), __uint_as_float(yv[1]), __uint_as_float(yv[2]), __uint_as_float(yv[3]));
+      if constexpr (RES == 2) {
+        const u32x4 xv = __builtin_amdgcn_raw_buffer_load_b128(xrsrc, (int)(bo + 16u * (unsigned)s), c << 7, 0);
+        xr[k] = make_float4(__uint_as_float(xv[0]), __uint_as_float(xv[1]), __uint_as_float(xv[2]), __uint_as_float(xv[3]));
+      } else {
+        const u32x2 h = __builtin_amdgcn_raw_buffer_load_b64(xrsrc, (int)(bo + 8u * (unsigned)s), c << 7, 0);
+        const u32x2 l = __builtin_amdgcn_raw_buffer_load_b64(xrsrc, (int)(bo + 64u + 8u * (unsigned)s), c << 7, 0);
+        xr[k] = make_float4(__uint_as_float(h[0]), __uint_as_float(h[1]), __uint_as_float(l[0]), __uint_as_float(l[1]));
+      }
+    }
+#endif
+  };
+  auto fetch_res_stats = [&](int c) {
+    fetch_norm(c);
+    if constexpr (RES == 2) {
+      xmu = *reinterpret_cast<const float4*>(g.res_mean + (long)img * g.C0 + (c << 5) + 4 * s);
+      xrs = *reinterpret_cast<const float4*>(g.res_rstd + (long)img * g.C0 + (c << 5) + 4 * s);
+    }
+  };
   bool norm_sat = false;
-  auto store_row_norm = [&](int buf, int k, float4 mu, float4 rs) {
+  auto store_row_norm = [&](int buf, int k, float4 mu, float4 rs, int cst = 0, bool wr = false) {
     const float hi = (pmeta[k] >> 12) != 0 ? 65504.f : 0.f;
     float4 v = pr[k];
-    v.x = (v.x - mu.x) * rs.x; v.y = (v.y - mu.y) * rs.y; v.z = (v.z - mu.z) * rs.z; v.w = (v.w - mu.w) * rs.w;
+    if constexpr (RES != 0) {
+      float4 r;
+      if constexpr (RES == 2) {
+        r = in_shortcut_raw4(xr[k], xmu, xrs, g.res_relu != 0);
+      } else {
+        const unsigned h0 = __float_as_uint(xr[k].x), h1 = __float_as_uint(xr[k].y), l0 = __float_as_uint(xr[k].z), l1 = __float_as_uint(xr[k].w);
+        r = make_float4(sf_join_lo_(h0, l0), sf_join_hi_(h0, l0), sf_join_lo_(h1, l1), sf_join_hi_(h1, l1));
+      }
+      v = in_residual_add4(r, in_norm_relu4(v, mu, rs));
+    } else {
+      v.x = (v.x - mu.x) * rs.x; v.y = (v.y - mu.y) * rs.y; v.z = (v.z - mu.z) * rs.z; v.w = (v.w - mu.w) * rs.w;
+    }
     const float m = fmaxf(fmaxf(v.x, v.y), fmaxf(v.z, v.w));
-    norm_sat |= !(m <= 65504.f);
+    if constexpr (RES != 0) norm_sat |= !(m <= 65504.f) & (wr && (pmeta[k] >> 12) != 0);
+    else norm_sat |= !(m <= 65504.f);
     v.x = __builtin_amdgcn_fmed3f(v.x, 0.f, hi); v.y = __builtin_amdgcn_fmed3f(v.y, 0.f, hi);
     v.z = __builtin_amdgcn_fmed3f(v.z, 0.f, hi); v.w = __builtin_amdgcn_fmed3f(v.w, 0.f, hi);
     const unsigned h0 = sf_cvt_pk_(v.x, v.y), h1 = sf_cvt_pk_(v.z, v.w);
@@ -165,6 +222,14 @@
     char* px = Pbytes + buf * PSZ + (((pmeta[k] & 0xFFFu) - (unsigned)s) << 4);
     *reinterpret_cast<uint2*>(px + 8 * s) = make_uint2(h0, h1);
     *reinterpret_cast<uint2*>(px + 64 + 8 * s) = make_uint2(l0, l1);
+#if defined(__HIP_DEVICE_COMPILE__)
+    if constexpr (RES != 0) {
+      typedef unsigned u32x2 __attribute__((ext_vector_type(2)));
+      const unsigned vo = (wr && ((owned >> k) & 1u)) ? 4u * ((pmeta[k] >> 12) - 1u) * (unsigned)g.ld0 + 8u * (unsigned)s : obytes;
+      __builtin_amdgcn_raw_buffer_store_b64(u32x2{h0, h1}, orsrc, (int)vo, cst << 7, 0);
+      __builtin_amdgcn_raw_buffer_store_b64(u32x2{l0, l1}, orsrc, (int)(vo + 64u), cst << 7, 0);
+    }
+#endif
   };
 
   const int wm = wave / WN, wn = wave % WN;
@@ -215,14 +280,20 @@
         if constexpr (!FAST) f.lo[j][cb] = *reinterpret_cast<const f16x8*>(wrow[j][cb] + (long)q * 512 + 256);
       }
     };
-    fetch_patch(0);
-    if constexpr (NORM) fetch_norm(0);
+    if constexpr (RES != 0) {
+      fetch_res_stats(0);
+#pragma unroll
+      for (int k = 0; k < NP; ++k) fetch_res_row(0, k, true);
+    } else {
+      fetch_patch(0);
+      if constexpr (NORM) fetch_norm(0);
+    }
 #pragma unroll
     for (int st = 0; st < RT - 1; ++st) { load_w(wr[st], 0, st, 0); load_w(wr[st], 0, st, 1); }
     if constexpr ((ABL & 1) != 0) { load_w(wr[RT - 1], 0, RT - 1, 0); load_w(wr[RT - 1], 0, RT - 1, 1); }
     if constexpr (NORM) {
 #pragma unroll
-      for (int k = 0; k < NP; ++k) store_row_norm(0, k, nmu, nrs);
+      for (int k = 0; k < NP; ++k) store_row_norm(0, k, nmu, nrs, 0, true);
     } else {
       store_patch(0);
     }
@@ -267,6 +338,7 @@
     constexpr int NMF = (FAST ? 1 : 3) * TM * TN * 2;
     constexpr int NH = 2 * NTAP;
     static_assert(!NORM || NH - 1 - NP >= 1, "normalise-on-load spreads its NP patch rows over the half-steps of a chunk");
+    static_assert(RES == 0 || NH - 1 - NP - RL >= 0, "residual-on-load requests a patch row RL half-steps before it is written");
     read_a(0, 0);
     if constexpr (KH != 3 || !Epi::kStats) __builtin_amdgcn_s_setprio(2);
     for (int c0 = 0; c0 < nck; c0 += CU) {
@@ -280,28 +352,37 @@
           const int tap = hs >> 1, half = hs & 1;
           const int st = cu * NTAP + tap;
           __builtin_amdgcn_sched_barrier(0);
-          if (!(ABL & 2) && hs == 0) { fetch_patch(cn); if constexpr (NORM) fetch_norm(cn); }
+          constexpr int RF0 = NH - 1 - NP - RL;
+          if constexpr (RES != 0) {
+            if (hs == RF0) fetch_res_stats(cn);
+            if (hs >= RF0 && hs < RF0 + NP) fetch_res_row(cn, hs - RF0, c + 1 < nck);
+          } else {
+            if (!(ABL & 2) && hs == 0) { fetch_patch(cn); if constexpr (NORM) fetch_norm(cn); }
+          }
           if (!(ABL & 1)) {
             if (RT == 2) { if (half == 0) { load_w(wr[(st + 1) % RT], c0, st + 1, 0); load_w(wr[(st + 1) % RT], c0, st + 1, 1); } }
             else load_w(wr[(st + RT - 1) % RT], c0, st + RT - 1, half);
           }
           if (!(ABL & 4) && hs + 1 < NH) read_a((hs + 1) & 1, (hs + 1) >> 1);
           if constexpr (NORM) {
-            if (hs >= NH - 1 - NP && hs <= NH - 2) store_row_norm((c + 1) & 1, hs - (NH - 1 - NP), nmu, nrs);
+            if (hs >= NH - 1 - NP && hs <= NH - 2) store_row_norm((c + 1) & 1, hs - (NH - 1 - NP), nmu, nrs, cn, c + 1 < nck);
           } else {
             if (!(ABL & 2) && hs == NH - 2) store_patch((c + 1) & 1);
           }
           if (live) mfma_half(half, wr[st % RT]);
           {
             constexpr int nds = 2 * TM;
-            const int nvm = (RT == 2 ? (half == 0 ? 4 * TN : 0) : 2 * TN) + (hs == 0 ? NP : 0);
+            const int nvm = (RT == 2 ? (half == 0 ? 4 * TN : 0) : 2 * TN) +
+                            (RES == 0 ? (hs == 0 ? NP : 0) : (hs >= RF0 && hs < RF0 + NP) ? (RES == 1 ? 3 : 2) : 0);
             const int ndw = NORM ? ((hs >= NH - 1 - NP && hs <= NH - 2) ? 2 : 0) : ((hs == NH - 2) ? NP : 0);
+            const int nvw = RES != 0 ? ndw : 0;
 #pragma unroll
             for (int k = 0; k < NMF; ++k) {
               __builtin_amdgcn_sched_group_barrier(0x008, 1, 0);
               if (hs + 1 < NH && k < nds) __builtin_amdgcn_sched_group_barrier(0x100, 1, 0);
               else if (k - ((hs + 1 < NH) ? nds : 0) < nvm) __builtin_amdgcn_sched_group_barrier(0x020, 1, 0);
               else if (k - ((hs + 1 < NH) ? nds : 0) - nvm < ndw) __builtin_amdgcn_sched_group_barrier(0x200, 1, 0);
+              else if (k - ((hs + 1 < NH) ? nds : 0) - nvm - ndw < nvw) __builtin_amdgcn_sched_group_barrier(0x040, 1, 0);
             }
           }
         }
@@ -657,6 +738,11 @@
   conv_sf6_body<TH, TW, BN, WM, WN, KH, KW, Epi, FAST, NORM, ABL>(g, ep, (int)blockIdx.x);
 }
 
+template <int TH, int TW, int BN, int WM, int WN, class Epi, int RES>
+__global__ __launch_bounds__(WM * WN * 64, 1) void conv_sf6_res_kernel(const Conv2Geom g, const Epi ep) {
+  conv_sf6_body<TH, TW, BN, WM, WN, 3, 3, Epi, false, true, 0, false, RES>(g, ep, (int)blockIdx.x);
+}
+
 template <int KH, int KW, class Epi, bool FAST = false>
 __global__ __launch_bounds__(256, 1) void conv_sf6_run_kernel(const Conv2Geom g, const Epi ep) {
   conv_sf6_body<8, 16, 128, 1, 4, KH, KW, Epi, FAST, false, 0, true>(g, ep, (int)blockIdx.x);
@@ -671,6 +757,7 @@
   g.nimg = s ? b.nimg : a.nimg; g.ntile_n = s ? b.ntile_n : a.ntile_n;
   g.w = s ? b.w : a.w; g.N = s ? b.N : a.N; g.wscale = s ? b.wscale : a.wscale;
   g.in_mean = nullptr; g.in_rstd = nullptr;
+  g.res = nullptr; g.res_mean = nullptr; g.res_rstd = nullptr; g.res_dst = nullptr; g.res_relu = 0;
   return g;
 }
 template <int TH, int TW, int BN, int WM, int WN, int KH, int KW, class Epi, bool FAST = false>
@@ -706,16 +793,37 @@
   ATDN_CHECK(NORM == (s.in_mean != nullptr) && (!NORM || (s.in_rstd && s.C1 == 0 && s.ld0 == s.C0)),
              "normalise-on-load: one dense fp32 source with its mean / rstd");
   ATDN_CHECK(g.w != nullptr, "missing weight copy for this kernel");
+  ATDN_CHECK(!s.res_dst || NORM, "residual-on-load is a mode of the normalise-on-load loader");
   return g;
 }
 
-template <int TH, int BN, int WM, int WN, int KH, int KW, class Epi, bool FAST = false, bool NORM = false, int ABL = 0>
+inline int conv_sf6_res_mode(const ConvShape& s) { return !s.res_dst ? 0 : s.res_sf ? 1 : 2; }
+
+template <int TH, int BN, int WM, int WN, int KH, int KW, class Epi, bool FAST = false, bool NORM = false, int ABL = 0, int RES = 0>
 inline void launch_conv_sf6(const ConvShape& s, float wscale, Epi ep, hipStream_t st) {
   constexpr int TW = 16;
-  const Conv2Geom g = conv_sf6_geom<TH, BN, WM, WN, KH, KW, Epi, FAST, NORM, ABL>(s, wscale);
+  Conv2Geom g = conv_sf6_geom<TH, BN, WM, WN, KH, KW, Epi, FAST, NORM, ABL>(s, wscale);
+  ATDN_CHECK(conv_sf6_res_mode(s) == RES, "residual-on-load operands do not match the instantiation");
+  if constexpr (RES != 0) {
+    ATDN_CHECK((s.res_sf != nullptr) != (s.res_raw != nullptr) && (!s.res_raw || (s.res_mean && s.res_rstd)),
+               "residual-on-load: one shortcut, sf or raw with its mean / rstd");
+    ATDN_CHECK(g.ntile_n == 1, "residual-on-load needs one channel tile per pixel tile: this plan keeps the separate pass");
+    ATDN_CHECK(g.Ho == g.H && g.Wo == g.W, "residual-on-load: the tiles of a 'same' convolution partition its input");
+    ATDN_CHECK(4L * g.H * g.W * s.ld0 + 128 < (1L << 32), "residual-on-load: the image's slice must fit a buffer descriptor");
+    const float* srcs[] = {s.src0, s.res_sf ? s.res_sf : s.res_raw};
+    for (const float* r : srcs)
+      ATDN_CHECK(r + (long)s.nimg * s.sb0 <= s.res_dst || s.res_dst + (long)s.nimg * s.sb0 <= r, "residual-on-load: the block output overlaps an operand");
+    g.res = s.res_sf ? s.res_sf : s.res_raw; g.res_mean = s.res_mean; g.res_rstd = s.res_rstd; g.res_dst = s.res_dst;
+    g.res_relu = s.res_relu ? 1 : 0;
+  }
   set_groups(ep, g.tiles_x * g.tiles_y * (TH * TW / 32));
   const int nblk = g.nimg * g.tiles_x * g.tiles_y * g.ntile_n;
-  hipLaunchKernelGGL((conv_sf6_kernel<TH, TW, BN, WM, WN, KH, KW, Epi, FAST, NORM, ABL>), dim3(nblk), dim3(WM * WN * 64), 0, st, g, ep);
+  if constexpr (RES != 0) {
+    static_assert(KH == 3 && KW == 3 && !FAST && NORM && ABL == 0, "residual-on-load: the normalise-on-load 3x3 kernels");
+    hipLaunchKernelGGL((conv_sf6_res_kernel<TH, TW, BN, WM, WN, Epi, RES>), dim3(nblk), dim3(WM * WN * 64), 0, st, g, ep);
+  } else {
+    hipLaunchKernelGGL((conv_sf6_kernel<TH, TW, BN, WM, WN, KH, KW, Epi, FAST, NORM, ABL>), dim3(nblk), dim3(WM * WN * 64), 0, st, g, ep);
+  }
   ATDN_HIP(hipGetLastError());
 }
 
@@ -774,11 +882,13 @@
     for (int c : {128, 256})
       if (cdiv(s.N, c) * c <= best) { best = cdiv(s.N, c) * c; bn = c; }
   }
+  const int bn_layer = bn;
   while (bn > 64 && bn != 96 && tiles * cdiv(s.N, bn) < 300) bn /= 2;
   if (!k3) bn = std::min(bn, 128);
   const bool fits12 = k3 && (bn == 64 || bn == 96) && cdiv(Ho, 12) * 12 * 100 <= cdiv(Ho, 8) * 8 * 103;
   if (s.in_mean) {
     if (!Epi::kStats || !k3 || fast || bn == 32 || bn == 256) return none;
+    if (s.tile_form == 1) return {(bn_layer == 64 || bn_layer == 96) && cdiv(Ho, 12) * 12 * 100 <= cdiv(Ho, 8) * 8 * 103 ? 12 : 8, bn_layer, false};
     return {fits12 ? 12 : 8, bn, false};
   }
   const bool run_ok = !k3 && plain && conv_sf6_run_eligible<KH, KW>(s);
@@ -794,8 +904,13 @@
 template <int TH, int BN, int WM, int WN, int KH, int KW, class Epi, bool FAST>
 inline void conv_sf6_launch_tile(const ConvShape& s, float wscale, const Epi& ep, hipStream_t st) {
   if (s.in_mean) {
-    if constexpr (Epi::kStats && KH == 3 && !FAST && TH >= 8 && (BN == 64 || BN == 96 || BN == 128))
-      return launch_conv_sf6<TH, BN, WM, WN, KH, KW, Epi, false, true>(s, wscale, ep, st);
+    if constexpr (Epi::kStats && KH == 3 && !FAST && TH >= 8 && (BN == 64 || BN == 96 || BN == 128)) {
+      switch (conv_sf6_res_mode(s)) {
+        case 0: return launch_conv_sf6<TH, BN, WM, WN, KH, KW, Epi, false, true>(s, wscale, ep, st);
+        case 1: return launch_conv_sf6<TH, BN, WM, WN, KH, KW, Epi, false, true, 0, 1>(s, wscale, ep, st);
+        default: return launch_conv_sf6<TH, BN, WM, WN, KH, KW, Epi, false, true, 0, 2>(s, wscale, ep, st);
+      }
+    }
     ATDN_CHECK(false, "no normalise-on-load kernel for this tile");
   }
   launch_conv_sf6<TH, BN, WM, WN, KH, KW, Epi, FAST, false>(s, wscale, ep, st);
diff --git a/atdn_vslam_amd/csrc/conv_sf_dispatch_impl.h b/atdn_vslam_amd/csrc/conv_sf_dispatch_impl.h
--- a/atdn_vslam_amd/csrc/conv_sf_dispatch_impl.h
+++ b/atdn_vslam_amd/csrc/conv_sf_dispatch_impl.h
@@ -13,7 +13,7 @@
     int bn = 0, th = 8;
     if (conv_sf6_try(s, wscale, ep, st, &bn, &th, sf_fast_mode())) return TileChoice{th * 16, bn, cdiv(Wo, 16) * cdiv(Ho, th) * (th / 2), true};
   }
-  ATDN_CHECK(s.in_mean == nullptr, "normalise-on-load is served by the halo-patch statistics kernels only");
+  ATDN_CHECK(s.in_mean == nullptr && s.res_dst == nullptr, "normalise-on-load is served by the halo-patch statistics kernels only");
   TileChoice t = choose_tile(s.nimg, Ho * Wo, s.N);
   t.groups_per_img = cdiv(Ho * Wo, t.BM) * (t.BM / 32);
   set_groups(ep, t.groups_per_img);
diff --git a/atdn_vslam_amd/csrc/conv_sf_inst_b.hip b/atdn_vslam_amd/csrc/conv_sf_inst_b.hip
--- a/atdn_vslam_amd/csrc/conv_sf_inst_b.hip
+++ b/atdn_vslam_amd/csrc/conv_sf_inst_b.hip
@@ -3,4 +3,11 @@
 ATDN_INSTANTIATE_CONV_SF(EpiBiasStats)
 ATDN_INSTANTIATE_CONV_SF(SfBiasReluAddRelu)
 ATDN_INSTANTIATE_CONV_SF(SfContextSplit)
+
+bool conv_sf_res_on_load_fits(const ConvShape& s) {
+  if (!s.in_mean || !conv_halo_eligible(s) || s.KH != 3 || s.KW != 3 || !conv_sf6_operands_ok(s)) return false;
+  if (s.padH != 1 || s.padW != 1) return false;
+  const Sf6Plan p = conv_sf6_plan<3, 3, EpiBiasStats>(s, sf_fast_mode());
+  return p.th != 0 && cdiv(s.N, p.bn) == 1;
 }
+}
diff --git a/atdn_vslam_amd/csrc/gma.hip b/atdn_vslam_amd/csrc/gma.hip
--- a/atdn_vslam_amd/csrc/gma.hip
+++ b/atdn_vslam_amd/csrc/gma.hip
@@ -566,10 +566,25 @@
   int h = conv_out(H, 7, 2, 3), w = conv_out(W, 7, 2, 3);
   DeviceBuf* eb = bufs ? bufs : enc_;
   float* X = eb[0].p; float* R = eb[1].p; float* Y = eb[2].p; float* O = eb[3].p;
-  auto stats_sf = [&](const PackedConv& L, const float* src, int ld, int ih, int iw, int stride, int pad, float* dst,
-                      int slot, int in_slot = -1) {
+  struct ResidualOnLoad {
+    const float* y = nullptr; int y_slot = 0;
+    const float* x = nullptr; int x_slot = 0; bool x_relu = false;
+    float* spare = nullptr;
+  } rol;
+  auto fold_width = [](int co) { return co == 64 || co == 96 || co == 128; };
+  auto stats_shape = [&](const PackedConv& L, const float* src, int ld, int ih, int iw, int stride, int pad, int in_slot) {
     ConvShape s = conv_shape(L, src, ld, (long)ih * iw * ld, nimg, ih, iw, stride, pad, pad);
     if (in_slot >= 0) { s.in_mean = mean_[in_slot].p; s.in_rstd = rstd_[in_slot].p; }
+    return s;
+  };
+  auto stats_sf = [&](const PackedConv& L, const float* src, int ld, int ih, int iw, int stride, int pad, float* dst,
+                      int slot, int in_slot = -1, float* res_dst = nullptr) {
+    ConvShape s = stats_shape(L, src, ld, ih, iw, stride, pad, in_slot);
+    if (res_dst) {
+      ATDN_CHECK(in_slot != slot && rol.x_slot != slot && dst != src && dst != rol.x && dst != res_dst,
+                 "residual-on-load: the convolution would write what it reads");
+      s.res_raw = rol.x; s.res_mean = mean_[rol.x_slot].p; s.res_rstd = rstd_[rol.x_slot].p; s.res_relu = rol.x_relu; s.res_dst = res_dst;
+    }
     const int oh = conv_out(ih, L.KH, stride, pad), ow = conv_out(iw, L.KW, stride, pad);
     EpiBiasStats ep{L.b, dst, (long)oh * ow * L.N, L.N, psum_.p, pm2_.p, 0, pcnt_.p};
     TileChoice t = conv_sf_dispatch(s, L.wscale, ep, st);
@@ -613,13 +628,28 @@
     if (instance && norm_on_load_) {
       const bool raw_in = stem_raw && bi == 0;
       ATDN_CHECK(!raw_in || !Bk.has_ds, "the block behind the stem has no downsample branch");
-      stats_sf(Bk.c1, X, c, h, w, stride, 1, R, 0, raw_in ? 2 : -1);
-      stats_sf(Bk.c2, R, co, oh, ow, 1, 1, Y, 1, 0);
+      float* C1 = R;
+      int c1_slot = 0;
+      if (rol.y) {
+        ATDN_CHECK(!Bk.has_ds && stride == 1 && c == co, "residual-on-load feeds the second block of a layer");
+        if (rol.x == R) C1 = rol.spare;
+        while (c1_slot == rol.y_slot || c1_slot == rol.x_slot) ++c1_slot;
+        stats_sf(Bk.c1, rol.y, c, h, w, 1, 1, C1, c1_slot, rol.y_slot, X);
+        rol = ResidualOnLoad{};
+      } else {
+        stats_sf(Bk.c1, X, c, h, w, stride, 1, C1, c1_slot, raw_in ? 2 : -1);
+      }
+      stats_sf(Bk.c2, C1, co, oh, ow, 1, 1, Y, 1, c1_slot);
+      bool fold = false;
+      if (bi % 2 == 0 && bi + 1 < 6 && (raw_in || Bk.has_ds) && !E.blk[bi + 1].has_ds && fold_width(co))
+        fold = conv_sf_res_on_load_fits(stats_shape(E.blk[bi + 1].c1, Y, co, oh, ow, 1, 1, 1));
       if (Bk.has_ds) {
         stats_sf(Bk.ds, X, c, h, w, 2, 0, R, 0);
-        launch_in_apply_sf(Y, O, mean_[1].p, rstd_[1].p, nullptr, R, mean_[0].p, rstd_[0].p, nimg, ohw, co, st);
+        if (fold) { rol.y = Y; rol.y_slot = 1; rol.x = R; rol.x_slot = 0; rol.x_relu = false; rol.spare = X; }
+        else launch_in_apply_sf(Y, O, mean_[1].p, rstd_[1].p, nullptr, R, mean_[0].p, rstd_[0].p, nimg, ohw, co, st);
       } else if (raw_in) {
-        launch_in_apply_sf(Y, O, mean_[1].p, rstd_[1].p, nullptr, X, mean_[2].p, rstd_[2].p, nimg, ohw, co, st, true);
+        if (fold) { rol.y = Y; rol.y_slot = 1; rol.x = X; rol.x_slot = 2; rol.x_relu = true; rol.spare = R; }
+        else launch_in_apply_sf(Y, O, mean_[1].p, rstd_[1].p, nullptr, X, mean_[2].p, rstd_[2].p, nimg, ohw, co, st, true);
       } else {
         launch_in_apply_sf(Y, O, mean_[1].p, rstd_[1].p, X, nullptr, nullptr, nullptr, nimg, ohw, co, st);
       }
diff --git a/atdn_vslam_amd/csrc/in_residual.h b/atdn_vslam_amd/csrc/in_residual.h
--- /dev/null
+++ b/atdn_vslam_amd/csrc/in_residual.h
@@ -0,0 +1,31 @@
+#pragma once
+#include "common.h"
+
+namespace atdn {
+
+__device__ __forceinline__ float4 in_norm_relu4(float4 v, const float4 mu, const float4 rs) {
+#pragma clang fp contract(off)
+  v.x = fmaxf((v.x - mu.x) * rs.x, 0.f);
+  v.y = fmaxf((v.y - mu.y) * rs.y, 0.f);
+  v.z = fmaxf((v.z - mu.z) * rs.z, 0.f);
+  v.w = fmaxf((v.w - mu.w) * rs.w, 0.f);
+  return v;
+}
+
+__device__ __forceinline__ float4 in_shortcut_raw4(float4 r, const float4 mu, const float4 rs, const bool relu) {
+#pragma clang fp contract(off)
+  r.x = (r.x - mu.x) * rs.x; r.y = (r.y - mu.y) * rs.y;
+  r.z = (r.z - mu.z) * rs.z; r.w = (r.w - mu.w) * rs.w;
+  r.x = relu ? fmaxf(r.x, 0.f) : r.x; r.y = relu ? fmaxf(r.y, 0.f) : r.y;
+  r.z = relu ? fmaxf(r.z, 0.f) : r.z; r.w = relu ? fmaxf(r.w, 0.f) : r.w;
+  return r;
+}
+
+__device__ __forceinline__ float4 in_residual_add4(const float4 r, float4 v) {
+#pragma clang fp contract(off)
+  v.x = fmaxf(r.x + v.x, 0.f); v.y = fmaxf(r.y + v.y, 0.f);
+  v.z = fmaxf(r.z + v.z, 0.f); v.w = fmaxf(r.w + v.w, 0.f);
+  return v;
+}
+
+}
diff --git a/atdn_vslam_amd/csrc/kernels.hip b/atdn_vslam_amd/csrc/kernels.hip
--- a/atdn_vslam_amd/csrc/kernels.hip
+++ b/atdn_vslam_amd/csrc/kernels.hip
@@ -524,6 +524,7 @@
 }
 
 #include "sf.h"
+#include "in_residual.h"
 #include <mutex>
 #include <vector>
 namespace atdn {
@@ -671,27 +672,18 @@
     const int c = (int)((i * 4) % C);
     const float* mu = mean + img * C + c;
     const float* rs = rstd + img * C + c;
-    float4 v = x[i];
-    v.x = fmaxf((v.x - mu[0]) * rs[0], 0.f);
-    v.y = fmaxf((v.y - mu[1]) * rs[1], 0.f);
-    v.z = fmaxf((v.z - mu[2]) * rs[2], 0.f);
-    v.w = fmaxf((v.w - mu[3]) * rs[3], 0.f);
+    float4 v = in_norm_relu4(x[i], make_float4(mu[0], mu[1], mu[2], mu[3]), make_float4(rs[0], rs[1], rs[2], rs[3]));
     if (res || res_raw) {
       float4 r;
       if (res) {
         r = sf_load4(res, i);
       } else {
-        r = res_raw[i];
         const float* m2 = rmean + img * C + c;
         const float* r2 = rrstd + img * C + c;
-        r.x = (r.x - m2[0]) * r2[0]; r.y = (r.y - m2[1]) * r2[1];
-        r.z = (r.z - m2[2]) * r2[2]; r.w = (r.w - m2[3]) * r2[3];
-        if (res_relu) {
-          r.x = fmaxf(r.x, 0.f); r.y = fmaxf(r.y, 0.f); r.z = fmaxf(r.z, 0.f); r.w = fmaxf(r.w, 0.f);
-        }
+        r = in_shortcut_raw4(res_raw[i], make_float4(m2[0], m2[1], m2[2], m2[3]), make_float4(r2[0], r2[1], r2[2], r2[3]),
+                             res_relu != 0);
       }
-      v.x = fmaxf(r.x + v.x, 0.f); v.y = fmaxf(r.y + v.y, 0.f);
-      v.z = fmaxf(r.z + v.z, 0.f); v.w = fmaxf(r.w + v.w, 0.f);
+      v = in_residual_add4(r, v);
     }
     sf_store4(y, i, v);
   }
diff --git a/include/atdn_hip.h b/include/atdn_hip.h
--- a/include/atdn_hip.h
+++ b/include/atdn_hip.h
@@ -290,6 +290,13 @@
                             const float* bias_host, int Cout, int KH, int KW, int stride, int padH, int padW, int sf_store,
                             float* dst, void* stream);
 
+
+int atdn_conv3x3_stats_residual(const float* y_raw, const float* y_mean, const float* y_rstd, const float* shortcut,
+                                const float* x_mean, const float* x_rstd, int x_relu, int nimg, int H, int W, int C,
+                                const float* weight_host, const float* bias_host, int Cout, int mode, float* o_sf, float* dst,
+                                float* part_sum, float* part_m2, float* part_cnt, long part_groups_cap, int* groups_per_img,
+                                void* stream);
+
 #ifdef __cplusplus
 }
 #endif
```

After: 449.3 frame-pairs/s, median of 6. About the same (+0.4%).
